# mrvollger/rustybam

Measured on AMD Instinct MI355X. Metric: CIGAR-ops/s, liftover over 100 kb sliding windows (whole pass, inputs resident in HBM), higher is better.
Workload: dtype u32

## Files before the change

### include/rustybam_amd.h

```cpp
#ifndef RUSTYBAM_AMD_H
#define RUSTYBAM_AMD_H

#include <stddef.h>
#include <stdint.h>

#ifdef __cplusplus
extern "C" {
#endif

#define RB_ABI_VERSION 1

enum rb_op { RB_OP_M = 0, RB_OP_I = 1, RB_OP_D = 2, RB_OP_N = 3, RB_OP_S = 4, RB_OP_H = 5, RB_OP_P = 6, RB_OP_EQ = 7, RB_OP_X = 8,
             RB_OP_CONT = 14  };

typedef enum rb_error {
    RB_OK = 0,
    RB_E_INVALID = -1,
    RB_E_NO_DEVICE = -2,
    RB_E_HIP = -3,
    RB_E_CAPACITY = -4,
    RB_E_NOMEM = -5
} rb_error;

typedef enum rb_status {
    RB_ST_OK = 0,
    RB_ST_NONE_INDEL = 1,
    RB_ST_NONE_NOMATCH = 2,
    RB_ST_NONE_EMPTY = 3,
    RB_ST_NONE_INVERTED = 4,
    RB_ST_NONE_INTEGRITY = 5,
    RB_ST_PANIC_NOTFOUND = 16,
    RB_ST_PANIC_EMPTY_CIGAR = 17,
    RB_ST_PANIC_INTEGRITY_T = 18,
    RB_ST_PANIC_INTEGRITY_Q = 19,
    RB_ST_PANIC_ALL_INDEL = 20,
    RB_ST_PANIC_ASSERT = 21,
    RB_ST_PANIC_OVERFLOW = 22
} rb_status;

enum { RB_BSEARCH_MODERN = 0 , RB_BSEARCH_LEGACY = 1 , RB_LIFT_EARLY_EXIT = 16,
       RB_LIFT_DESCRIPTORS = 32,
       RB_LIFT_FUSED_SCAN = 64,
       RB_BREAK_ONE_WALK = 128,
       RB_LIFT_OP_STARTS = 1 << 20,
       RB_LIFT_QBED = 1 << 21 };

enum {
    RB_F_REGULAR = 1u << 0,
    RB_F_STRIPPED = 1u << 1,
    RB_F_HAS_M = 1u << 2,
    RB_F_PROVISIONAL = 1u << 3,
    RB_F_ENDS_NOT_MATCH = 1u << 4
};
enum {
    RB_HIT_INSIDE = 1u << 0,
    RB_HIT_GENERIC = 1u << 1,
    RB_HIT_DESCRIPTOR = 1u << 2
};

typedef struct rb_reduce_row {
    uint64_t t_bases, q_bases;
    uint32_t nmatch, aln_len;
    uint32_t equal, diff, ins, del, matches;
    uint32_t ins_events, del_events;
    float id_by_all, id_by_events, id_by_matches;
    uint32_t status;
    uint32_t flags;
} rb_reduce_row;

typedef struct rb_norm_row {
    uint64_t t_st, t_en, q_st, q_en;
    uint32_t first_op, n_ops;
    uint32_t lead_ops, trail_ops;
    uint32_t nmatch, aln_len;
    uint32_t status;
    uint32_t flags;
} rb_norm_row;

typedef struct rb_hit_row {
    uint32_t rec, win;
    uint16_t status, flags;
    uint32_t out_n;
    uint64_t t_st, t_en, q_st, q_en;
    uint32_t nmatch, aln_len;
    uint64_t out_off;
} rb_hit_row;

typedef struct rb_pair_row {
    uint64_t split_idx;
    int32_t split_score;
    uint32_t status;
    uint64_t t_st[2], t_en[2], q_st[2], q_en[2];
    uint32_t nmatch[2], aln_len[2];
    uint64_t out_off[2];
    uint32_t out_n[2];
    uint64_t _pad;
} rb_pair_row;

typedef struct rb_counters {
    uint64_t n_hits;
    uint64_t out_ops_needed;
    uint64_t out_ops_used;
    uint64_t n_generic;
    uint32_t overflow;
    uint32_t phase[5];
    uint32_t brk_scratch_short;
    uint32_t redo_two_walk;
} rb_counters;

enum { RB_TEXT_OK = 0, RB_TEXT_BAD = 1 , RB_TEXT_TOO_LONG = 2 ,
       RB_TEXT_UNUSUAL = 3  };

typedef struct rb_batch_view {
    uint64_t n_rec, n_ops;
    const uint32_t *ops;
    const uint64_t *op_off;
    const uint64_t *t_st, *t_en, *q_st, *q_en;
    const uint8_t *strand;
    const uint32_t *contig;
} rb_batch_view;

typedef struct rb_windows_view {
    uint64_t n_win;
    const uint32_t *contig;
    const uint64_t *st, *en;
} rb_windows_view;

typedef struct rb_ctx rb_ctx;
typedef struct rb_plan rb_plan;

int rb_abi_version(void);
int rb_device_count(void);
int rb_ctx_create(int device, void *hip_stream, rb_ctx **out);
void rb_ctx_destroy(rb_ctx *ctx);
const char *rb_ctx_last_error(const rb_ctx *ctx);
int rb_ctx_sync(rb_ctx *ctx);
void *rb_ctx_stream(rb_ctx *ctx);
int rb_ctx_set_timing(rb_ctx *ctx, int enabled);
int rb_ctx_get_timing(rb_ctx *ctx, double *ms_out, int cap, int *n_out);

int rb_dev_alloc(rb_ctx *ctx, size_t bytes, void **dev_ptr);
int rb_dev_free(rb_ctx *ctx, void *dev_ptr);
int rb_dev_alloc_mode(rb_ctx *ctx, const void *dev_ptr);
int rb_dev_release(rb_ctx *ctx, void *dev_ptr);
int rb_dev_cache_trim(rb_ctx *ctx, uint64_t keep_bytes);
int rb_dev_alloc_stats(rb_ctx *ctx, uint64_t out[5]);
int rb_dev_upload(rb_ctx *ctx, void *dev_dst, const void *host_src, size_t bytes);
int rb_dev_download(rb_ctx *ctx, void *host_dst, const void *dev_src, size_t bytes);
int rb_dev_memset(rb_ctx *ctx, void *dev_dst, int value, size_t bytes);

int rb_dev_scan_records(rb_ctx *ctx, const rb_batch_view *batch, rb_reduce_row *reduce_rows, rb_norm_row *norm_rows);
int rb_ctx_scan_route(rb_ctx *ctx, uint64_t out[2]);

int rb_plan_create(rb_ctx *ctx, uint64_t n_rec, const uint64_t *op_off_host, const uint32_t *contig_host,
                   uint64_t n_win, const uint32_t *w_contig_host, const uint64_t *w_st_host, const uint64_t *w_en_host,
                   rb_plan **out);
void rb_plan_destroy(rb_plan *plan);
int64_t rb_plan_tiles_host(uint64_t n_rec, const uint64_t *op_off_host, uint64_t short_max, uint32_t *sched_out, uint32_t *tiles_out,
                           uint64_t tiles_cap, uint64_t *n_long_out);
size_t rb_plan_workspace_bytes(const rb_plan *plan, uint64_t rows_cap);
size_t rb_plan_diag_stamps_offset(const rb_plan *plan, uint64_t rows_cap);
uint64_t rb_plan_out_capacity(const rb_plan *plan, int for_break);

int rb_dev_liftover(rb_ctx *ctx, const rb_plan *plan, const rb_batch_view *batch, const rb_norm_row *norm_rows,
                    int bsearch_policy, void *workspace, rb_hit_row *rows, uint64_t rows_cap, uint32_t *out_ops,
                    uint64_t out_cap, rb_counters *counters);

size_t rb_largest_scratch_bytes(uint64_t n_keys);
int rb_dev_largest(rb_ctx *ctx, const rb_hit_row *rows, uint64_t n_rows, const uint32_t *win_key, const uint32_t *rec_key,
                   uint64_t n_keys, uint64_t *sel, uint64_t *out, void *scratch);

int rb_dev_stats_rows(rb_ctx *ctx, const rb_batch_view *batch, const rb_hit_row *rows, uint64_t n_rows, const uint32_t *out_ops,
                      rb_reduce_row *stats );

typedef struct rb_pieces_info {
    uint64_t n_pieces, n_ops;
    uint32_t overflow;
    uint32_t declined;
    uint64_t _reserved[5];
} rb_pieces_info;
size_t rb_rows_to_batch_scratch_bytes(uint64_t n_rows);
void rb_rows_to_batch_shape(uint32_t out[3]);
int rb_dev_rows_to_batch(rb_ctx *ctx, const rb_batch_view *src, const rb_hit_row *rows, uint64_t n_rows, const uint32_t *out_ops,
                         uint64_t pieces_cap, uint64_t ops_cap, uint32_t *new_ops, uint64_t *new_op_off ,
                         uint64_t *t_st, uint64_t *t_en, uint64_t *q_st, uint64_t *q_en, uint8_t *strand, uint32_t *contig,
                         uint32_t *parent , rb_pieces_info *info, void *scratch);

enum { RB_PAIRS_ORIENT = 1, RB_PAIRS_FILTER = 2 };
enum { RB_PAIRS_DECL_PANIC = 1, RB_PAIRS_DECL_KEY = 2, RB_PAIRS_DECL_WRAP = 4, RB_PAIRS_DECL_ZERO_SPAN = 8 };
typedef struct rb_pairs_info {
    uint64_t n_kept, n_flipped_rows;
    uint32_t overflow;
    uint32_t declined;
    uint64_t _reserved[5];
} rb_pairs_info;
size_t rb_pairs_scratch_bytes(uint64_t n_keys, uint64_t n_rows);
void rb_pairs_shape(uint32_t out[2]);
int rb_dev_pairs_rows(rb_ctx *ctx, const rb_hit_row *rows, uint64_t n_rows, const uint32_t *rec_key, const uint64_t *rec_q_len,
                      const uint8_t *strand , uint64_t n_rec, uint64_t n_keys, uint32_t mode, uint64_t paired_len,
                      uint64_t min_aln, uint64_t min_query, rb_hit_row *rows_out, uint64_t rows_cap, uint8_t *key_flip ,
                      rb_pairs_info *info, void *scratch);
int rb_host_pairs_rows(const rb_hit_row *rows, uint64_t n_rows, const uint32_t *rec_key, const uint64_t *rec_q_len, const uint8_t *strand,
                       uint64_t n_rec, uint64_t n_keys, uint32_t mode, uint64_t paired_len, uint64_t min_aln, uint64_t min_query,
                       rb_hit_row *rows_out, uint64_t rows_cap, uint8_t *key_flip, rb_pairs_info *info);

size_t rb_pairs_records_scratch_bytes(uint64_t n_keys, uint64_t n_rec);
void rb_pairs_records_shape(uint32_t out[2]);
int rb_dev_pairs_records(rb_ctx *ctx, const uint64_t *t_st, const uint64_t *t_en, const uint64_t *q_st, const uint64_t *q_en,
                         const uint8_t *strand, const uint32_t *rec_key, const uint64_t *rec_q_len ,
                         uint64_t n_rec, uint64_t n_keys, uint32_t mode ,
                         uint64_t paired_len, uint64_t min_aln, uint64_t min_query,
                         uint32_t *kept , uint64_t kept_cap, uint64_t *q_st_out, uint64_t *q_en_out ,
                         uint8_t *key_flip , uint64_t *key_order , rb_pairs_info *info, void *scratch);
int rb_host_pairs_records(const uint64_t *t_st, const uint64_t *t_en, const uint64_t *q_st, const uint64_t *q_en, const uint8_t *strand,
                          const uint32_t *rec_key, const uint64_t *rec_q_len, uint64_t n_rec, uint64_t n_keys, uint32_t mode, uint64_t paired_len,
                          uint64_t min_aln, uint64_t min_query, uint32_t *kept, uint64_t kept_cap, uint64_t *q_st_out, uint64_t *q_en_out,
                          uint8_t *key_flip, uint64_t *key_order, rb_pairs_info *info);

int rb_dev_break(rb_ctx *ctx, const rb_plan *plan, const rb_batch_view *batch, const rb_norm_row *norm_rows,
                 uint32_t max_size, int bsearch_policy, void *workspace, rb_hit_row *rows, uint64_t rows_cap,
                 uint32_t *out_ops, uint64_t out_cap, rb_counters *counters);

int rb_dev_swap(rb_ctx *ctx, const rb_batch_view *batch, uint32_t *out_ops);

enum { RB_TRIM_IN_PLACE = 256 };
int rb_dev_overlap_split(rb_ctx *ctx, const rb_batch_view *batch, const rb_norm_row *norm_rows, uint64_t n_pairs,
                         const uint32_t *left, const uint32_t *right, const uint64_t *pair_out_off, int match_score,
                         int diff_score, int indel_score, int bsearch_policy, rb_pair_row *rows, uint32_t *out_ops);

int rb_dev_trim_reserve(rb_ctx *ctx, uint64_t n_pairs);

int rb_dev_apply_pairs(rb_ctx *ctx, uint64_t n_pairs, const uint32_t *left, const uint32_t *right, const rb_pair_row *rows,
                       uint64_t *op_off, rb_norm_row *norm_rows);

typedef struct rb_trim_pass {
    uint64_t n_pairs, n_deferred, ops_end;
    uint32_t bad_status, _pad;
    uint64_t _reserved[4];
} rb_trim_pass;
size_t rb_trim_select_scratch_bytes(uint64_t n_groups);
int rb_dev_trim_select(rb_ctx *ctx, uint64_t n_rec, uint64_t n_groups, const uint32_t *order, const uint64_t *grp_off,
                       const rb_norm_row *norm_rows, uint64_t out_base, uint8_t *contained, uint32_t *left, uint32_t *right,
                       uint64_t *pair_out_off, rb_trim_pass *pass, void *scratch);
int rb_dev_trim_check(rb_ctx *ctx, uint64_t n_pairs, const rb_pair_row *rows, rb_trim_pass *pass);
int rb_dev_gather_records(rb_ctx *ctx, uint64_t n_rec, const uint32_t *ops, const uint64_t *op_off, const rb_norm_row *norm_rows,
                          uint64_t *new_op_off, uint32_t *new_ops, void *scratch);

int rb_host_scan_records(rb_ctx *ctx, uint64_t n_rec, const uint32_t *ops, const uint64_t *op_off,
                         const uint64_t *t_st, const uint64_t *t_en, const uint64_t *q_st, const uint64_t *q_en,
                         const uint8_t *strand, rb_reduce_row *reduce_rows, rb_norm_row *norm_rows);
int rb_host_liftover(rb_ctx *ctx, uint64_t n_rec, const uint32_t *ops, const uint64_t *op_off, const uint64_t *t_st,
                     const uint64_t *t_en, const uint64_t *q_st, const uint64_t *q_en, const uint8_t *strand,
                     const uint32_t *contig, uint64_t n_win, const uint32_t *w_contig, const uint64_t *w_st,
                     const uint64_t *w_en, int bsearch_policy, rb_norm_row *norm_rows_out ,
                     rb_hit_row **rows, uint64_t *n_rows, uint32_t **out_ops, uint64_t *n_out, rb_counters *counters);
int rb_host_break(rb_ctx *ctx, uint64_t n_rec, const uint32_t *ops, const uint64_t *op_off, const uint64_t *t_st,
                  const uint64_t *t_en, const uint64_t *q_st, const uint64_t *q_en, const uint8_t *strand,
                  uint32_t max_size, int bsearch_policy, rb_norm_row *norm_rows_out, rb_hit_row **rows,
                  uint64_t *n_rows, uint32_t **out_ops, uint64_t *n_out, rb_counters *counters);
int rb_host_swap(rb_ctx *ctx, uint64_t n_rec, const uint32_t *ops, const uint64_t *op_off, const uint8_t *strand,
                 uint32_t *out_ops);
int rb_host_overlap_split(rb_ctx *ctx, uint64_t n_rec, const uint32_t *ops, const uint64_t *op_off, const uint64_t *t_st,
                          const uint64_t *t_en, const uint64_t *q_st, const uint64_t *q_en, const uint8_t *strand,
                          uint64_t n_pairs, const uint32_t *left, const uint32_t *right, int match_score, int diff_score,
                          int indel_score, int bsearch_policy, rb_pair_row *rows, uint32_t **out_ops, uint64_t *n_out);
void rb_host_free(void *p);

size_t rb_text_scratch_bytes(uint64_t n);
int rb_dev_parse_cigars(rb_ctx *ctx, const uint8_t *text, const uint64_t *text_off, const uint64_t *text_end, uint64_t n_rec,
                        uint64_t *op_off, uint32_t *ops, uint64_t ops_cap, uint8_t *status, void *scratch);
int rb_dev_format_cigars(rb_ctx *ctx, const uint32_t *ops, const uint32_t *ops_alt, uint64_t n_items, const uint64_t *first,
                         const uint32_t *count, const uint32_t *first_len, const uint32_t *last_len, uint64_t *text_off, uint8_t *text,
                         uint64_t text_cap, void *scratch);
int rb_host_parse_cigars(rb_ctx *ctx, const uint8_t *text, const uint64_t *text_off, const uint64_t *text_end, uint64_t n_rec,
                         uint64_t *op_off, uint32_t **ops, uint8_t *status);
int rb_host_format_cigars(rb_ctx *ctx, const uint32_t *ops, uint64_t n_ops, uint64_t n_items, const uint64_t *first, const uint32_t *count,
                          const uint32_t *first_len, const uint32_t *last_len, uint64_t *text_off, uint8_t **text);
int rb_host_liftover_text(rb_ctx *ctx, uint64_t n_rec, const uint8_t *text, uint64_t text_bytes, const uint64_t *cig_off,
                          const uint64_t *cig_end, const uint64_t *t_st, const uint64_t *t_en, const uint64_t *q_st, const uint64_t *q_en,
                          const uint8_t *strand, const uint32_t *contig, uint64_t n_win, const uint32_t *w_contig, const uint64_t *w_st,
                          const uint64_t *w_en, int bsearch_policy, uint8_t *cig_status, rb_reduce_row *reduce_out, rb_norm_row *norm_out,
                          rb_hit_row **rows, uint64_t *n_rows, uint64_t **row_text_off, uint8_t **row_text, rb_counters *counters);
int rb_host_liftover_largest_text(rb_ctx *ctx, uint64_t n_rec, const uint8_t *text, uint64_t text_bytes, const uint64_t *cig_off,
                                  const uint64_t *cig_end, const uint64_t *t_st, const uint64_t *t_en, const uint64_t *q_st, const uint64_t *q_en,
                                  const uint8_t *strand, const uint32_t *contig, uint64_t n_win, const uint32_t *w_contig, const uint64_t *w_st,
                                  const uint64_t *w_en, int bsearch_policy, uint8_t *cig_status, rb_reduce_row *reduce_out, rb_norm_row *norm_out,
                                  rb_hit_row **rows, uint64_t *n_rows, uint64_t **row_text_off, uint8_t **row_text, rb_counters *counters,
                                  const uint32_t *win_key, uint64_t n_keys, uint32_t inside_key, int *declined);
int rb_host_break_text(rb_ctx *ctx, uint64_t n_rec, const uint8_t *text, uint64_t text_bytes, const uint64_t *cig_off,
                       const uint64_t *cig_end, const uint64_t *t_st, const uint64_t *t_en, const uint64_t *q_st, const uint64_t *q_en,
                       const uint8_t *strand, uint32_t max_size, int bsearch_policy, uint8_t *cig_status, rb_reduce_row *reduce_out,
                       rb_norm_row *norm_out, rb_hit_row **rows, uint64_t *n_rows, uint64_t **row_text_off, uint8_t **row_text,
                       rb_counters *counters);
int rb_host_liftover_stats_text(rb_ctx *ctx, uint64_t n_rec, const uint8_t *text, uint64_t text_bytes, const uint64_t *cig_off,
                                const uint64_t *cig_end, const uint64_t *t_st, const uint64_t *t_en, const uint64_t *q_st, const uint64_t *q_en,
                                const uint8_t *strand, const uint32_t *contig, uint64_t n_win, const uint32_t *w_contig, const uint64_t *w_st,
                                const uint64_t *w_en, int bsearch_policy, uint8_t *cig_status, rb_reduce_row *reduce_out, rb_norm_row *norm_out,
                                rb_hit_row **rows, uint64_t *n_rows, rb_reduce_row **stats, rb_counters *counters);
int rb_host_break_stats_text(rb_ctx *ctx, uint64_t n_rec, const uint8_t *text, uint64_t text_bytes, const uint64_t *cig_off,
                             const uint64_t *cig_end, const uint64_t *t_st, const uint64_t *t_en, const uint64_t *q_st, const uint64_t *q_en,
                             const uint8_t *strand, uint32_t max_size, int bsearch_policy, uint8_t *cig_status, rb_reduce_row *reduce_out,
                             rb_norm_row *norm_out, rb_hit_row **rows, uint64_t *n_rows, rb_reduce_row **stats, rb_counters *counters);
int rb_host_break_pairs_text(rb_ctx *ctx, uint64_t n_rec, const uint8_t *text, uint64_t text_bytes, const uint64_t *cig_off,
                             const uint64_t *cig_end, const uint64_t *t_st, const uint64_t *t_en, const uint64_t *q_st, const uint64_t *q_en,
                             const uint8_t *strand, uint32_t max_size, int bsearch_policy, uint8_t *cig_status, rb_reduce_row *reduce_out,
                             rb_norm_row *norm_out, rb_hit_row **rows, uint64_t *n_rows, uint64_t **row_text_off, uint8_t **row_text,
                             rb_counters *counters, const uint32_t *rec_key, const uint64_t *rec_q_len, uint64_t n_keys, uint32_t mode,
                             uint64_t paired_len, uint64_t min_aln, uint64_t min_query, uint8_t *key_flip, int *declined);
int rb_host_break_pairs_stats_text(rb_ctx *ctx, uint64_t n_rec, const uint8_t *text, uint64_t text_bytes, const uint64_t *cig_off,
                                   const uint64_t *cig_end, const uint64_t *t_st, const uint64_t *t_en, const uint64_t *q_st, const uint64_t *q_en,
                                   const uint8_t *strand, uint32_t max_size, int bsearch_policy, uint8_t *cig_status, rb_reduce_row *reduce_out,
                                   rb_norm_row *norm_out, rb_hit_row **rows, uint64_t *n_rows, rb_reduce_row **stats, rb_counters *counters,
// ... 90 lines not shown
```

### rustybam_amd/csrc/capi.hip

```cpp
#include <hip/hip_runtime.h>
#include <sys/mman.h>

#include <algorithm>
#include <cstdarg>
#include <cstdio>
#include <cstdlib>
#include <cstring>
#include <ctime>
#include <numeric>
#include <string>
#include <thread>
#include <vector>
#include <chrono>
#include <map>
#include <mutex>

#include "../../include/rustybam_amd.h"
#include "rb_lift.h"
#include "rb_trim.h"
#include "rb_launch.h"

#ifndef RB_SCAN_ROWS_MEAN_MAX
#define RB_SCAN_ROWS_MEAN_MAX 1536
#endif
#ifndef RB_SHORT_MAX_DEFAULT
#define RB_SHORT_MAX_DEFAULT 2048
#endif

#define RB_MAX_ARENA 256

#define RB_TIMING_RING 256
__global__ __launch_bounds__(256) void rb_k_fill_bytes(uint8_t *dst, uint32_t v4, size_t n) {
    const uintptr_t a = (uintptr_t)dst;
    const size_t head = n < 16 ? n : (size_t)((16 - (a & 15)) & 15);
    const size_t body = (n - head) / 16;
    const size_t tail0 = head + body * 16;
    const size_t i = (size_t)blockIdx.x * blockDim.x + threadIdx.x, stride = (size_t)gridDim.x * blockDim.x;
    for (size_t k = i; k < body; k += stride) *reinterpret_cast<uint4 *>(dst + head + k * 16) = make_uint4(v4, v4, v4, v4);
    if (i < head) dst[i] = (uint8_t)v4;
    if (i < n - tail0) dst[tail0 + i] = (uint8_t)v4;
}
extern "C" hipError_t rb_fill_async(void *dst, int value, size_t bytes, hipStream_t stream) {
    if (!bytes) return hipSuccess;
    const uint32_t b = (uint32_t)value & 255u, v4 = b | (b << 8) | (b << 16) | (b << 24);
    const size_t groups = bytes / 16 + 1;
    const unsigned blocks = (unsigned)std::min<size_t>((groups + 255) / 256, 65536);
    hipLaunchKernelGGL(rb_k_fill_bytes, dim3(blocks ? blocks : 1), dim3(256), 0, stream, (uint8_t *)dst, v4, bytes);
    return hipGetLastError();
}

struct rb_ctx {
    int device = -1;
    hipStream_t stream = nullptr;
    bool own_stream = false;
    std::string err;
    bool timing = false;
    std::vector<hipEvent_t> ev_a, ev_b;
    uint64_t timed_calls = 0;
    hipStream_t side = nullptr;
    hipEvent_t ev_fork = nullptr, ev_join = nullptr;
    void *trim_scratch = nullptr;
    uint32_t trim_scratch_blocks = 0;
    void *trim_pend = nullptr;
    uint64_t trim_pend_cap = 0;
    void *scan_list = nullptr;
    uint64_t scan_list_cap = 0;
    uint64_t scan_rows_n = 0;
    void *pin[2] = {nullptr, nullptr};
    hipEvent_t pin_ev[2] = {nullptr, nullptr};
    bool pin_busy[2] = {false, false};
    unsigned pin_next = 0;
    uint64_t alloc_fallbacks = 0;
    struct cached_buf { void *p; size_t bytes; bool placed; };
    std::vector<cached_buf> cache;
    size_t cache_bytes = 0;
};
#define RB_PIN_CHUNK ((size_t)32 << 20)
#define RB_PIN_MIN ((size_t)8 << 20)

struct rb_plan {
    rb_ctx *ctx = nullptr;
    uint64_t n_rec = 0, n_win = 0, n_ops = 0;
    uint32_t n_contig = 0;
    uint32_t depth = 0;
    uint32_t *sched = nullptr, *slot_of = nullptr, *canon_pos = nullptr, *w_orig = nullptr, *ident = nullptr;
    uint64_t *w_st = nullptr, *w_en = nullptr, *wo_st = nullptr, *wo_en = nullptr, *cw_off = nullptr;
    uint8_t *cw_mono = nullptr;
    uint32_t *tiles = nullptr;
    uint32_t n_tiles = 0, stream_end = 0;
};

static int fail(rb_ctx *ctx, int code, const char *fmt, ...) {
    if (ctx) {
        char buf[512];
        va_list ap;
        va_start(ap, fmt);
        vsnprintf(buf, sizeof buf, fmt, ap);
        va_end(ap);
        ctx->err = buf;
    }
    return code;
}
#define HIPCHK(ctx, call)                                                                             \
    do {                                                                                              \
        hipError_t e_ = (call);                                                                       \
        if (e_ != hipSuccess) return fail((ctx), RB_E_HIP, "%s: %s", #call, hipGetErrorString(e_)); \
    } while (0)

extern "C" int rb_abi_version(void) { return RB_ABI_VERSION; }

extern "C" int rb_device_count(void) {
    int n = 0;
    if (hipGetDeviceCount(&n) != hipSuccess) return 0;
    return n;
}

extern "C" int rb_ctx_create(int device, void *hip_stream, rb_ctx **out) {
    if (!out) return RB_E_INVALID;
    *out = nullptr;
    int n = 0;
    if (hipGetDeviceCount(&n) != hipSuccess || n <= 0 || device < 0 || device >= n) return RB_E_NO_DEVICE;
    hipDeviceProp_t prop;
    if (hipGetDeviceProperties(&prop, device) != hipSuccess) return RB_E_NO_DEVICE;
    if (strncmp(prop.gcnArchName, "gfx950", 6) != 0) {
        fprintf(stderr, "rustybam_amd: device %d is %s; this library only carries gfx950 (MI355X) code objects\n", device, prop.gcnArchName);
        return RB_E_NO_DEVICE;
    }
    if (hipSetDevice(device) != hipSuccess) return RB_E_NO_DEVICE;
    rb_ctx *c = new rb_ctx();
    c->device = device;
    if (hip_stream) {
        c->stream = (hipStream_t)hip_stream;
    } else {
        if (hipStreamCreateWithFlags(&c->stream, hipStreamNonBlocking) != hipSuccess) {
            delete c;
            return RB_E_HIP;
        }
        c->own_stream = true;
    }
    int prio_least = 0, prio_greatest = 0;
    if (hipDeviceGetStreamPriorityRange(&prio_least, &prio_greatest) != hipSuccess ||
        hipStreamCreateWithPriority(&c->side, hipStreamNonBlocking, prio_least) != hipSuccess ||
        hipEventCreateWithFlags(&c->ev_fork, hipEventDisableTiming) != hipSuccess ||
        hipEventCreateWithFlags(&c->ev_join, hipEventDisableTiming) != hipSuccess) {
        (void)hipGetLastError();
        rb_ctx_destroy(c);
        return RB_E_HIP;
    }
    *out = c;
    return RB_OK;
}
extern "C" void rb_ctx_destroy(rb_ctx *ctx) {
    if (!ctx) return;
    if (ctx->side) {
        (void)hipStreamSynchronize(ctx->side);
        hipStreamDestroy(ctx->side);
    }
    if (ctx->ev_fork) hipEventDestroy(ctx->ev_fork);
    if (ctx->ev_join) hipEventDestroy(ctx->ev_join);
    for (auto e : ctx->ev_a) hipEventDestroy(e);
    for (auto e : ctx->ev_b) hipEventDestroy(e);
    for (int k = 0; k < 2; k++) {
        if (ctx->pin[k]) hipHostFree(ctx->pin[k]);
        if (ctx->pin_ev[k]) hipEventDestroy(ctx->pin_ev[k]);
    }
    if (ctx->trim_scratch) hipFree(ctx->trim_scratch);
    if (ctx->trim_pend) hipFree(ctx->trim_pend);
    if (ctx->scan_list) hipFree(ctx->scan_list);
    (void)rb_dev_cache_trim(ctx, 0);
    if (ctx->own_stream) hipStreamDestroy(ctx->stream);
    delete ctx;
}
extern "C" const char *rb_ctx_last_error(const rb_ctx *ctx) { return ctx ? ctx->err.c_str() : "no context"; }
extern "C" int rb_ctx_sync(rb_ctx *ctx) {
    if (!ctx) return RB_E_INVALID;
    HIPCHK(ctx, hipStreamSynchronize(ctx->stream));
    return RB_OK;
}
extern "C" void *rb_ctx_stream(rb_ctx *ctx) { return ctx ? (void *)ctx->stream : nullptr; }

extern "C" int rb_ctx_set_timing(rb_ctx *ctx, int enabled) {
    if (!ctx) return RB_E_INVALID;
    if (enabled && ctx->ev_a.empty()) {
        ctx->ev_a.resize(RB_TIMING_RING);
        ctx->ev_b.resize(RB_TIMING_RING);
        for (int i = 0; i < RB_TIMING_RING; i++) {
            HIPCHK(ctx, hipEventCreate(&ctx->ev_a[i]));
            HIPCHK(ctx, hipEventCreate(&ctx->ev_b[i]));
        }
    }
    ctx->timing = enabled != 0;
    ctx->timed_calls = 0;
    return RB_OK;
}
extern "C" int rb_ctx_get_timing(rb_ctx *ctx, double *ms_out, int cap, int *n_out) {
    if (!ctx || !ms_out || !n_out) return RB_E_INVALID;
    HIPCHK(ctx, hipStreamSynchronize(ctx->stream));
    const uint64_t have = ctx->timed_calls < RB_TIMING_RING ? ctx->timed_calls : RB_TIMING_RING;
    int n = 0;
    for (uint64_t k = 0; k < have && n < cap; k++) {
        const uint64_t call = ctx->timed_calls - have + k;
        const size_t slot = (size_t)(call % RB_TIMING_RING);
        float ms = 0;
        HIPCHK(ctx, hipEventElapsedTime(&ms, ctx->ev_a[slot], ctx->ev_b[slot]));
        ms_out[n++] = ms;
    }
    *n_out = n;
    return RB_OK;
}

struct rb_vmm_alloc {
    size_t bytes, chunk;
    std::vector<hipMemGenericAllocationHandle_t> handles;
    bool placed = false;
};
static std::map<void *, rb_vmm_alloc> g_vmm;
static std::mutex g_vmm_mu;
static size_t g_va_live = 0, g_va_retired = 0;
static std::map<void *, size_t> g_asked;
static size_t rb_va_cap() {
    const char *e = getenv("RB_ALLOC_VA_CAP_GB");
    return (size_t)(e ? strtoull(e, nullptr, 10) : 32768ull) << 30;
}
static int rb_free_vmm(void *p, int device, hipError_t *err) {
    std::lock_guard<std::mutex> lk(g_vmm_mu);
    auto it = g_vmm.find(p);
    if (it == g_vmm.end()) return 0;
    hipError_t first = hipSuccess;
    auto note = [&](hipError_t e) {
        if (e != hipSuccess && first == hipSuccess) first = e;
    };
    note(hipSetDevice(device));
    note(hipDeviceSynchronize());
    const size_t chunk = it->second.chunk, n = it->second.handles.size();
    for (size_t k = 0; k < n; k++) note(hipMemUnmap((char *)p + k * chunk, chunk));
    for (auto &h : it->second.handles) note(hipMemRelease(h));
    g_va_live -= it->second.bytes;
    g_va_retired += it->second.bytes;
// ... 236 lines not shown
    if (!pin_ready(ctx)) {
        HIPCHK(ctx, hipStreamSynchronize(ctx->stream));
        HIPCHK(ctx, hipMemcpy(host_dst, dev_src, bytes, hipMemcpyDeviceToHost));
        return RB_OK;
    }
    size_t prev_off = 0, prev_n = 0;
    int prev_slot = -1;
    for (size_t off = 0, k = 0; off < bytes; off += RB_PIN_CHUNK, k++) {
        const int slot = (int)(k & 1);
        const size_t n = std::min(RB_PIN_CHUNK, bytes - off);
        if (ctx->pin_busy[slot]) HIPCHK(ctx, hipEventSynchronize(ctx->pin_ev[slot]));
        HIPCHK(ctx, hipMemcpyAsync(ctx->pin[slot], (const char *)dev_src + off, n, hipMemcpyDeviceToHost, ctx->stream));
        HIPCHK(ctx, hipEventRecord(ctx->pin_ev[slot], ctx->stream));
        ctx->pin_busy[slot] = true;
        if (prev_slot >= 0) {
            HIPCHK(ctx, hipEventSynchronize(ctx->pin_ev[prev_slot]));
            par_memcpy((char *)host_dst + prev_off, ctx->pin[prev_slot], prev_n);
            ctx->pin_busy[prev_slot] = false;
        }
        prev_off = off, prev_n = n, prev_slot = slot;
    }
    if (prev_slot >= 0) {
        HIPCHK(ctx, hipEventSynchronize(ctx->pin_ev[prev_slot]));
        par_memcpy((char *)host_dst + prev_off, ctx->pin[prev_slot], prev_n);
        ctx->pin_busy[prev_slot] = false;
    }
    HIPCHK(ctx, hipStreamSynchronize(ctx->stream));
    return RB_OK;
}
extern "C" int rb_dev_memset(rb_ctx *ctx, void *dev_dst, int value, size_t bytes) {
    if (!ctx) return RB_E_INVALID;
    if (bytes) HIPCHK(ctx, rb_fill_async(dev_dst, value, bytes, ctx->stream));
    return RB_OK;
}

extern "C" int rb_dev_scan_records(rb_ctx *ctx, const rb_batch_view *b, rb_reduce_row *reduce_rows, rb_norm_row *norm_rows) {
    if (!ctx || !b) return RB_E_INVALID;
    if (((uintptr_t)b->ops & 15u) != 0) return fail(ctx, RB_E_INVALID, "ops must be 16-byte aligned");
    rb_scan_params p;
    p.n_rec = b->n_rec;
    p.ops = b->ops;
    p.op_off = b->op_off;
    p.t_st = b->t_st;
    p.t_en = b->t_en;
    p.q_st = b->q_st;
    p.q_en = b->q_en;
    p.strand = b->strand;
    p.reduce_rows = reduce_rows;
    p.norm_rows = norm_rows;
    p.list = nullptr;
    p.n_list = nullptr;
    ctx->scan_rows_n = 0;
    if (b->n_rec >= 64 && b->n_ops / b->n_rec <= RB_SCAN_ROWS_MEAN_MAX) {
        if (ctx->scan_list_cap < b->n_rec) {
            HIPCHK(ctx, hipStreamSynchronize(ctx->stream));
            if (ctx->scan_list) hipFree(ctx->scan_list);
            ctx->scan_list = nullptr, ctx->scan_list_cap = 0;
            const uint64_t cap = b->n_rec + b->n_rec / 4 + 1024;
            if (hipMalloc(&ctx->scan_list, 256 + cap * 4) == hipSuccess) ctx->scan_list_cap = cap;
            else (void)hipGetLastError();
        }
        if (ctx->scan_list) {
            HIPCHK(ctx, rb_fill_async(ctx->scan_list, 0, 8, ctx->stream));
            HIPCHK(ctx, rb_launch_scan_rows(&p, ctx->scan_list, ctx->stream));
            ctx->scan_rows_n = b->n_rec;
            return RB_OK;
        }
    }
    HIPCHK(ctx, rb_launch_scan_records(&p, ctx->stream));
    return RB_OK;
}

extern "C" int rb_ctx_scan_route(rb_ctx *ctx, uint64_t out[2]) {
    if (!ctx || !out) return RB_E_INVALID;
    out[0] = out[1] = 0;
    if (!ctx->scan_rows_n) return RB_OK;
    unsigned long long n_listed = 0;
    HIPCHK(ctx, hipSetDevice(ctx->device));
    HIPCHK(ctx, hipMemcpyAsync(&n_listed, ctx->scan_list, sizeof n_listed, hipMemcpyDeviceToHost, ctx->stream));
    HIPCHK(ctx, hipStreamSynchronize(ctx->stream));
    out[0] = ctx->scan_rows_n - n_listed;
    out[1] = n_listed;
    return RB_OK;
}

template <typename T>
static int upload_vec(rb_ctx *ctx, const std::vector<T> &v, T **dev) {
    int rc = rb_dev_alloc(ctx, v.size() * sizeof(T) + 16, (void **)dev);
    if (rc) return rc;
    if (!v.empty()) {
        rc = rb_dev_upload(ctx, *dev, v.data(), v.size() * sizeof(T));
        if (rc) return rc;
    }
    return RB_OK;
}

static void rb_cut_tiles(uint64_t n_rec, const uint64_t *op_off, uint64_t short_max, std::vector<uint32_t> &sched, std::vector<uint32_t> &tiles,
                         uint64_t *n_long_out) {
    tiles.clear();
    *n_long_out = 0;
    short_max = std::min<uint64_t>(short_max, rb_tile_max_ops());
    if (short_max < 8 || !n_rec) return;
    const uint64_t max_ops = rb_tile_max_ops(), max_rec = rb_tile_max_records();
    std::vector<uint32_t> t2;
    uint64_t first = 0, cnt = 0, ops = 0, n_long = 0, n_tiled = 0;
    bool tiny = false;
    auto close = [&]() {
        if (cnt) t2.push_back((uint32_t)first | (tiny ? 0x80000000u : 0u)), t2.push_back((uint32_t)cnt), n_tiled += tiny ? 0 : cnt;
        cnt = 0, ops = 0;
    };
    for (uint64_t r = 0; r < n_rec; r++) {
        const uint64_t n = op_off[r + 1] - op_off[r];
        if (n > short_max) {
            close();
            n_long++;
            continue;
        }
        const bool t = n < 8;
        if (cnt && (t != tiny || cnt >= max_rec || (!t && ops + n > max_ops))) close();
        if (!cnt) first = r, tiny = t;
        cnt++, ops += n;
    }
    close();
    if (n_tiled == 0) return;
    std::vector<uint32_t> s2(n_rec);
    uint64_t a = 0, b = n_long;
    for (uint64_t w = 0; w < n_rec; w++)
        if (op_off[(uint64_t)sched[w] + 1] - op_off[sched[w]] > short_max) s2[a++] = sched[w];
    std::vector<uint32_t> slot_short(n_rec, 0);
    for (uint64_t r = 0; r < n_rec; r++)
        if (op_off[r + 1] - op_off[r] <= short_max) slot_short[r] = (uint32_t)b, s2[b++] = (uint32_t)r;
    sched.swap(s2);
    tiles.reserve(t2.size() / 2 * 3);
    for (size_t t = 0; t + 1 < t2.size(); t += 2) tiles.push_back(t2[t]), tiles.push_back(t2[t + 1]), tiles.push_back(slot_short[t2[t] & 0x7FFFFFFFu]);
    *n_long_out = n_long;
}
extern "C" int64_t rb_plan_tiles_host(uint64_t n_rec, const uint64_t *op_off, uint64_t short_max, uint32_t *sched_out, uint32_t *tiles_out,
                                      uint64_t tiles_cap, uint64_t *n_long_out) {
    if (n_rec && (!op_off || !sched_out)) return -1;
    if (n_rec >= 0xFFFFFFFFull) return -1;
    std::vector<uint32_t> sched(n_rec), tiles;
    std::iota(sched.begin(), sched.end(), 0u);
    std::stable_sort(sched.begin(), sched.end(), [&](uint32_t x, uint32_t y) { return op_off[(uint64_t)x + 1] - op_off[x] > op_off[(uint64_t)y + 1] - op_off[y]; });
    uint64_t n_long = 0;
    rb_cut_tiles(n_rec, op_off, short_max ? short_max : RB_SHORT_MAX_DEFAULT, sched, tiles, &n_long);
    for (uint64_t i = 0; i < n_rec; i++) sched_out[i] = sched[i];
    const uint64_t nt = tiles.size() / 3;
    for (uint64_t t = 0; t < nt && t < tiles_cap && tiles_out; t++)
        for (int k = 0; k < 3; k++) tiles_out[3 * t + k] = tiles[3 * t + k];
    if (n_long_out) *n_long_out = tiles.empty() ? n_rec : n_long;
    return (int64_t)nt;
}

extern "C" int rb_plan_create(rb_ctx *ctx, uint64_t n_rec, const uint64_t *op_off, const uint32_t *contig, uint64_t n_win,
                              const uint32_t *w_contig, const uint64_t *w_st, const uint64_t *w_en, rb_plan **out) {
    if (!ctx || !out || (n_rec && (!op_off || !contig))) return RB_E_INVALID;
    if (n_rec >= 0xFFFFFFFFull || n_win >= 0xFFFFFFFFull) return fail(ctx, RB_E_INVALID, "too many records/windows for one batch");
    HIPCHK(ctx, hipSetDevice(ctx->device));
    rb_plan *pl = new rb_plan();
    pl->ctx = ctx;
    pl->n_rec = n_rec;
    pl->n_win = n_win;
    uint32_t maxc = 0;
    for (uint64_t i = 0; i < n_rec; i++) maxc = std::max(maxc, contig[i]);
    for (uint64_t i = 0; i < n_win; i++) maxc = std::max(maxc, w_contig[i]);
    const uint32_t n_contig = (n_rec || n_win) ? maxc + 1 : 0;
    pl->n_contig = n_contig;
    std::vector<uint32_t> canon_pos(n_rec);
    {
        std::vector<uint64_t> rank(n_contig, UINT64_MAX);
        uint64_t nr = 0;
        for (uint64_t i = 0; i < n_rec; i++)
            if (rank[contig[i]] == UINT64_MAX) rank[contig[i]] = nr++;
        std::vector<uint64_t> start(nr + 1, 0);
        for (uint64_t i = 0; i < n_rec; i++) start[rank[contig[i]] + 1]++;
        for (uint64_t k = 0; k < nr; k++) start[k + 1] += start[k];
        for (uint64_t i = 0; i < n_rec; i++) canon_pos[i] = (uint32_t)start[rank[contig[i]]]++;
    }
    std::vector<uint32_t> sched(n_rec), ident(n_rec);
    std::iota(ident.begin(), ident.end(), 0u);
    {
        uint64_t max_len = 0;
        std::vector<uint64_t> key(n_rec);
        for (uint64_t i = 0; i < n_rec; i++) key[i] = op_off[i + 1] - op_off[i], max_len = std::max(max_len, key[i]);
        int passes = 0;
        while (passes < 4 && (max_len >> (16 * passes)) != 0) passes++;
        std::vector<uint32_t> a(ident), b(n_rec);
        std::vector<uint64_t> cnt(65537);
        for (int ps = 0; ps < passes; ps++) {
            std::fill(cnt.begin(), cnt.end(), 0);
            const int sh = 16 * ps;
            for (uint64_t i = 0; i < n_rec; i++) cnt[(0xFFFFu - (uint32_t)((key[i] >> sh) & 0xFFFFu)) + 1]++;
            for (int k = 0; k < 65536; k++) cnt[k + 1] += cnt[k];
            for (uint64_t i = 0; i < n_rec; i++) {
                const uint32_t r = a[i];
                b[cnt[0xFFFFu - (uint32_t)((key[r] >> sh) & 0xFFFFu)]++] = r;
            }
            a.swap(b);
        }
        sched = a;
    }
    std::vector<uint64_t> cw_off(n_contig + 1, 0), g_st(n_win), g_en(n_win), o_st(n_win), o_en(n_win);
    std::vector<uint32_t> g_orig(n_win);
    std::vector<uint8_t> mono(n_contig ? n_contig : 1, 1);
    for (uint64_t i = 0; i < n_win; i++) cw_off[w_contig[i] + 1]++;
    for (uint32_t c = 0; c < n_contig; c++) cw_off[c + 1] += cw_off[c];
    {
        std::vector<uint64_t> cur(cw_off.begin(), cw_off.end() - (n_contig ? 1 : 0));
        for (uint64_t i = 0; i < n_win; i++) {
            const uint64_t d = cur[w_contig[i]]++;
            g_st[d] = w_st[i];
            g_en[d] = w_en[i];
            g_orig[d] = (uint32_t)i;
            o_st[i] = w_st[i];
            o_en[i] = w_en[i];
        }
    }
    for (uint32_t c = 0; c < n_contig; c++)
        for (uint64_t i = cw_off[c] + 1; i < cw_off[c + 1]; i++)
            if (g_st[i] < g_st[i - 1] || g_en[i] < g_en[i - 1]) mono[c] = 0;
    pl->n_ops = n_rec ? op_off[n_rec] : 0;
    for (uint32_t c = 0; c < n_contig; c++) {
        if (!mono[c]) continue;
        uint64_t lo = cw_off[c];
        for (uint64_t i = cw_off[c]; i < cw_off[c + 1]; i++) {
            while (lo < i && g_en[lo] < g_st[i]) lo++;
            pl->depth = std::max<uint32_t>(pl->depth, (uint32_t)std::min<uint64_t>(i - lo + 1, 1u << 20));
        }
    }
    std::vector<uint32_t> tiles;
    pl->stream_end = (uint32_t)n_rec;
    {
        const char *e = getenv("RB_TILE");
        const bool on = !(e && !strcmp(e, "0"));
        uint64_t short_max = RB_SHORT_MAX_DEFAULT;
        if (const char *m = getenv("RB_SHORT_MAX")) short_max = strtoull(m, nullptr, 10);
        if (on && n_rec) {
            uint64_t n_long = 0;
            rb_cut_tiles(n_rec, op_off, short_max, sched, tiles, &n_long);
            if (!tiles.empty()) pl->stream_end = (uint32_t)n_long;
        }
        pl->n_tiles = (uint32_t)(tiles.size() / 3);
    }
    int rc = RB_OK;
    std::vector<uint32_t> slot_of(n_rec);
    for (uint64_t w = 0; w < n_rec; w++) slot_of[sched[w]] = (uint32_t)w;
    if (!rc) rc = upload_vec(ctx, sched, &pl->sched);
    if (!rc) rc = upload_vec(ctx, slot_of, &pl->slot_of);
    if (!rc) rc = upload_vec(ctx, ident, &pl->ident);
    if (!rc) rc = upload_vec(ctx, canon_pos, &pl->canon_pos);
    if (!rc) rc = upload_vec(ctx, g_st, &pl->w_st);
    if (!rc) rc = upload_vec(ctx, g_en, &pl->w_en);
    if (!rc) rc = upload_vec(ctx, g_orig, &pl->w_orig);
    if (!rc) rc = upload_vec(ctx, o_st, &pl->wo_st);
    if (!rc) rc = upload_vec(ctx, o_en, &pl->wo_en);
    if (!rc) rc = upload_vec(ctx, cw_off, &pl->cw_off);
    if (!rc) rc = upload_vec(ctx, mono, &pl->cw_mono);
    if (!rc && pl->n_tiles) rc = upload_vec(ctx, tiles, &pl->tiles);
    if (!rc && hipStreamSynchronize(ctx->stream) != hipSuccess) rc = fail(ctx, RB_E_HIP, "plan upload: %s", hipGetErrorString(hipGetLastError()));
    if (rc) {
        rb_plan_destroy(pl);
        return rc;
    }
    *out = pl;
    return RB_OK;
}
extern "C" void rb_plan_destroy(rb_plan *pl) {
    if (!pl) return;
    void *ptrs[] = {pl->sched, pl->slot_of, pl->ident, pl->canon_pos, pl->w_st, pl->w_en, pl->w_orig, pl->wo_st, pl->wo_en, pl->cw_off, pl->cw_mono, pl->tiles};
    for (void *q : ptrs)
        if (q) (void)rb_dev_free(pl->ctx, q);
    delete pl;
}

struct ws_layout {
    size_t hit_off, win_lo, block_sums, arena, pend_count, pend_list, jobs, gen_list, x_st, x_en, bp_tmp, bp_off, bp_cur, brk_rows, copy_count, copy_list, decl_count, decl_list, gen_cp, diag_stamps, fb_count, fb_list, starts_bad, total;
};
static bool rb_no_gen_cp() {
    static const bool v = getenv("RB_DEBUG_NO_GEN_CP") != nullptr;
    return v;
}
static ws_layout ws_of(uint64_t n_rec, uint64_t rows_cap, uint64_t n_ops) {
    ws_layout w;
    size_t o = 0;
    auto take = [&](size_t bytes) {
        size_t at = o;
        o += (bytes + 255) & ~(size_t)255;
        return at;
    };
    w.hit_off = take((n_rec + 2) * 8);
    w.win_lo = take((n_rec + 2) * 4);
    w.block_sums = take(rb_scan_block_sums_count(n_rec) * 8);
    w.arena = take((size_t)RB_MAX_ARENA * RB_ARENA_STRIDE * 8);
    w.pend_count = take(256);
    w.pend_list = take((n_rec + 1) * 4);
    w.jobs = take((n_rec + 1) * sizeof(rb_job));
    w.gen_list = take((rows_cap + 1) * 4);
    w.x_st = take((rows_cap + 1) * 8);
    w.x_en = take((rows_cap + 1) * 8);
    w.bp_tmp = take((rows_cap + 1) * 8);
    w.bp_off = take((n_rec + 1) * 8);
    w.bp_cur = take((size_t)RB_MAX_ARENA * 128);
    w.brk_rows = take((rows_cap + 1) * sizeof(rb_hit_row));
    w.copy_count = take(256);
    w.copy_list = take((rows_cap + 1) * 16);
    w.decl_count = take(256);
    w.decl_list = take((n_rec + 1) * 4);
    w.gen_cp = take(rb_no_gen_cp() ? 256 : (size_t)(n_ops / RB_GCP + n_rec + 2) * sizeof(uint4));
    w.diag_stamps = take((n_rec + 1) * 4);
    w.fb_count = take(256);
    w.fb_list = take((n_rec + 1) * 4);
    w.starts_bad = take(256);
    w.total = o;
    return w;
}
extern "C" size_t rb_plan_workspace_bytes(const rb_plan *plan, uint64_t rows_cap) {
    if (!plan) return 0;
    return ws_of(plan->n_rec, rows_cap, plan->n_ops).total;
}
extern "C" size_t rb_plan_diag_stamps_offset(const rb_plan *plan, uint64_t rows_cap) {
    if (!plan) return 0;
    return ws_of(plan->n_rec, rows_cap, plan->n_ops).diag_stamps;
}

static uint64_t slot_stride_of(uint64_t n_ops, uint64_t n_rec) { return ((n_ops + 31) & ~(uint64_t)31) + 32 * n_rec + 64; }
extern "C" uint64_t rb_plan_out_capacity(const rb_plan *plan, int for_break) {
    if (!plan) return 0;
    const uint64_t slots = for_break ? std::min<uint32_t>(2u, RB_MS) : std::min<uint32_t>(plan->depth, RB_MS);
    return slots * slot_stride_of(plan->n_ops, plan->n_rec) + plan->n_ops / 16 + 32 * plan->n_rec + (1u << 20);
}

static uint32_t pick_arenas(uint64_t n_rec) {
    uint64_t a = n_rec / 256;
    if (a < 1) a = 1;
    if (a > RB_MAX_ARENA) a = RB_MAX_ARENA;
    return (uint32_t)a;
}

static int lift_common(rb_ctx *ctx, const rb_plan *plan, const rb_batch_view *b, const rb_norm_row *norm, int policy,
                       void *workspace, rb_hit_row *rows, uint64_t rows_cap, uint32_t *out_ops, uint64_t out_cap,
                       rb_counters *counters, bool is_break, uint32_t max_size) {
    if (!ctx || !plan || !b || !norm || !workspace || !counters) return RB_E_INVALID;
    if (b->n_rec != plan->n_rec) return fail(ctx, RB_E_INVALID, "plan was built for %llu records, batch has %llu", (unsigned long long)plan->n_rec, (unsigned long long)b->n_rec);
    if (((uintptr_t)b->ops & 15u) || ((uintptr_t)out_ops & 15u)) return fail(ctx, RB_E_INVALID, "ops/out_ops must be 16-byte aligned");
    if (rows_cap >= 0xFFFFFFFFull) return fail(ctx, RB_E_INVALID, "rows_cap too large");
    if ((uintptr_t)workspace & 255u) return fail(ctx, RB_E_INVALID, "workspace must be 256-byte aligned");
    const ws_layout w = ws_of(plan->n_rec, rows_cap, plan->n_ops);
    char *ws = (char *)workspace;
    rb_lift_params p;
    memset(&p, 0, sizeof p);
    p.n_rec = b->n_rec;
    p.ops = b->ops;
    p.op_off = b->op_off;
    p.contig = b->contig;
    p.strand = b->strand;
    p.norm = norm;
    p.sched = plan->sched;
    p.slot_of = plan->slot_of;
    p.canon_pos = is_break ? plan->ident : plan->canon_pos;
    p.w_st = plan->w_st;
    p.w_en = plan->w_en;
    p.w_orig = plan->w_orig;
    p.wo_st = plan->wo_st;
    p.wo_en = plan->wo_en;
    p.cw_off = plan->cw_off;
    p.cw_mono = plan->cw_mono;
    p.n_contig = plan->n_contig;
    p.hit_off = (uint64_t *)(ws + w.hit_off);
    p.win_lo = (uint32_t *)(ws + w.win_lo);
    p.rows = rows;
    p.rows_cap = rows_cap;
    p.out_ops = out_ops;
    p.out_cap = out_cap;
    p.arena_cur = (unsigned long long *)(ws + w.arena);
    p.n_arena = pick_arenas(b->n_rec);
    p.desc_mode = (policy & RB_LIFT_DESCRIPTORS) ? 1 : 0;
    p.slot_stride = slot_stride_of(b->n_ops, b->n_rec);
    const uint32_t want = p.desc_mode ? 0u : std::min<uint32_t>(is_break ? 2u : plan->depth, RB_MS);
    const uint64_t min_arena = 1024ull * p.n_arena;
    uint32_t n_slots = want;
    while (n_slots && (uint64_t)n_slots * p.slot_stride + min_arena > out_cap) n_slots--;
    if (getenv("RB_DEBUG_SLOTS")) n_slots = std::min<uint32_t>(n_slots, (uint32_t)atoi(getenv("RB_DEBUG_SLOTS")));
    p.n_slots = n_slots;
    p.needed_base = p.desc_mode ? 4 * rows_cap : (uint64_t)want * p.slot_stride;
    p.arena_origin = p.desc_mode ? 4 * rows_cap : (uint64_t)n_slots * p.slot_stride;
    if (p.desc_mode && out_cap < p.arena_origin + 1024) return fail(ctx, RB_E_CAPACITY, "descriptor mode needs out_cap >= 4 * rows_cap + 1024");
    p.arena_size = out_cap > p.arena_origin ? ((out_cap - p.arena_origin) / p.n_arena) & ~(uint64_t)3 : 0;
    p.copy_list = (uint4 *)(ws + w.copy_list);
    p.gj_a = (rb_gja *)(ws + w.brk_rows), p.gj_b = (uint4 *)(ws + w.copy_list), p.gj_c = (uint2 *)(ws + w.bp_tmp);
    p.copy_count = (unsigned long long *)(ws + w.copy_count);
    p.gen_list = (uint32_t *)(ws + w.gen_list);
    p.gen_cp = rb_no_gen_cp() ? nullptr : (uint4 *)(ws + w.gen_cp);
    p.diag_stamps = (uint32_t *)(ws + w.diag_stamps);
    p.jobs = (rb_job *)(ws + w.jobs);
    p.fused = (policy & RB_LIFT_FUSED_SCAN) ? 1 : 0;
    p.op_starts = (policy & RB_LIFT_OP_STARTS) ? 1 : 0;
    if (p.op_starts && p.fused) return fail(ctx, RB_E_INVALID, "RB_LIFT_OP_STARTS takes finished norm_rows: not together with RB_LIFT_FUSED_SCAN");
    if (p.op_starts && (policy & RB_LIFT_DESCRIPTORS)) return fail(ctx, RB_E_INVALID, "RB_LIFT_OP_STARTS with RB_LIFT_DESCRIPTORS: a descriptor indexes the record's ORIGINAL cigar, which a batch cut in place no longer is");
    if (p.op_starts && b->n_ops > plan->n_ops) return fail(ctx, RB_E_INVALID, "RB_LIFT_OP_STARTS: batch->n_ops exceeds the plan's op count (gather the batch first)");
    if (p.op_starts && b->n_rec) {
        unsigned long long *bad = (unsigned long long *)(ws + w.starts_bad), first_bad = 0;
        HIPCHK(ctx, rb_fill_async(bad, 0xFF, 8, ctx->stream));
        HIPCHK(ctx, rb_launch_starts_check(b->op_off, norm, b->n_rec, b->n_ops, bad, ctx->stream));
        HIPCHK(ctx, hipMemcpyAsync(&first_bad, bad, 8, hipMemcpyDeviceToHost, ctx->stream));
        HIPCHK(ctx, hipStreamSynchronize(ctx->stream));
        if (first_bad != ~0ull)
            return fail(ctx, RB_E_INVALID, "RB_LIFT_OP_STARTS: record %llu lies outside the batch's %llu ops (a pass moved it: gather the batch first)",
                        first_bad, (unsigned long long)b->n_ops);
    }
    p.norm_w = const_cast<rb_norm_row *>(norm);
    p.pend_list = (uint32_t *)(ws + w.pend_list);
    p.pend_count = (unsigned long long *)(ws + w.pend_count);
    const bool use_tiles = plan->n_tiles != 0 && ((policy >> 8) & 0xFFF) == 0;
    p.tile_first = use_tiles ? plan->tiles : nullptr;
    p.n_tiles = use_tiles ? plan->n_tiles : 0;
    p.fb_list = (uint32_t *)(ws + w.fb_list);
    p.fb_count = (unsigned long long *)(ws + w.fb_count);
    const uint32_t stream_end = use_tiles ? plan->stream_end : (uint32_t)b->n_rec;
    rb_scan_params sp;
    memset(&sp, 0, sizeof sp);
    if (p.fused) {
        sp.n_rec = b->n_rec;
        sp.ops = b->ops;
        sp.op_off = b->op_off;
        sp.t_st = b->t_st, sp.t_en = b->t_en, sp.q_st = b->q_st, sp.q_en = b->q_en;
        sp.strand = b->strand;
        sp.norm_rows = p.norm_w;
        HIPCHK(ctx, rb_fill_async(p.pend_count, 0, 8, ctx->stream));
        HIPCHK(ctx, rb_launch_peek_norm(&sp, ctx->stream));
    }
    p.counters = counters;
    p.policy = policy & 1;
    p.early_exit = (policy & RB_LIFT_EARLY_EXIT) ? 1 : 0;
    p.debug_skip = (policy >> 8) & 0xFFF;
    uint64_t *block_sums = (uint64_t *)(ws + w.block_sums);
    HIPCHK(ctx, rb_fill_async(counters, 0, sizeof(rb_counters), ctx->stream));
    HIPCHK(ctx, rb_fill_async(p.copy_count, 0, 8, ctx->stream));
    HIPCHK(ctx, rb_fill_async(p.arena_cur, 0, (size_t)RB_MAX_ARENA * RB_ARENA_STRIDE * 8, ctx->stream));
    if (b->n_rec == 0) return RB_OK;
    const bool one_walk = is_break && (policy & RB_BREAK_ONE_WALK) && !p.desc_mode;
    if (one_walk) {
        p.brk_mode = 1, p.brk_max = max_size;
        p.rows_final = rows;
        p.rows = (rb_hit_row *)(ws + w.brk_rows);
        p.brk_off = (uint64_t *)(ws + w.bp_off);
        p.brk_cursor = (unsigned long long *)(ws + w.bp_cur);
        p.brk_n_arena = pick_arenas(b->n_rec);
        p.brk_arena_cap = rows_cap / p.brk_n_arena;
        p.brk_decl_list = (uint32_t *)(ws + w.decl_list);
        p.brk_decl_count = (unsigned long long *)(ws + w.decl_count);
        HIPCHK(ctx, rb_fill_async(p.brk_decl_count, 0, 8, ctx->stream));
        HIPCHK(ctx, rb_fill_async(p.brk_cursor, 0, (size_t)RB_MAX_ARENA * 128, ctx->stream));
        HIPCHK(ctx, rb_fill_async(p.hit_off, 0, (size_t)(b->n_rec + 2) * 8, ctx->stream));
        HIPCHK(ctx, rb_fill_async(p.brk_off, 0xFF, (size_t)(b->n_rec + 1) * 8, ctx->stream));
        HIPCHK(ctx, rb_launch_make_jobs(&p, ctx->stream));
        const size_t slot1 = (size_t)(ctx->timed_calls % RB_TIMING_RING);
        if (ctx->timing) HIPCHK(ctx, hipEventRecord(ctx->ev_a[slot1], ctx->stream));
        p.wave0 = 0;
        p.wave_end = stream_end;
        HIPCHK(ctx, rb_launch_liftover_stream(&p, ctx->stream));
        if (use_tiles) {
            HIPCHK(ctx, rb_fill_async(p.fb_count, 0, 8, ctx->stream));
            HIPCHK(ctx, rb_launch_liftover_tiles(&p, ctx->stream));
            HIPCHK(ctx, rb_launch_liftover_stream_list(&p, ctx->stream));
        }
        if (p.fused) {
            sp.list = p.pend_list;
            sp.n_list = (const uint64_t *)p.pend_count;
            HIPCHK(ctx, rb_launch_scan_records(&sp, ctx->stream));
        }
        if (ctx->timing) {
            HIPCHK(ctx, hipEventRecord(ctx->ev_b[slot1], ctx->stream));
            ctx->timed_calls++;
        }
        rb_break_params bp;
        memset(&bp, 0, sizeof bp);
        bp.n_rec = b->n_rec, bp.ops = b->ops, bp.op_off = b->op_off, bp.norm = norm, bp.sched = plan->sched, bp.hit_off = p.hit_off;
        bp.x_st = (uint64_t *)(ws + w.x_st), bp.x_en = (uint64_t *)(ws + w.x_en);
        bp.rows_cap = rows_cap, bp.max_size = max_size;
        bp.list = p.brk_decl_list, bp.n_list = p.brk_decl_count;
        bp.fill = 0;
        HIPCHK(ctx, rb_launch_break_list_declined(&p, ctx->stream));
        HIPCHK(ctx, rb_launch_break_pieces(&bp, ctx->stream));
        HIPCHK(ctx, rb_launch_count_and_scan(&p, block_sums, false, ctx->stream));
        bp.fill = 1;
        HIPCHK(ctx, rb_launch_break_pieces(&bp, ctx->stream));
        HIPCHK(ctx, rb_launch_break_gather(&p, ctx->stream));
        rb_lift_params pg = p;
        pg.rows = rows, pg.x_st = bp.x_st, pg.x_en = bp.x_en;
        HIPCHK(ctx, rb_launch_break_declined(&pg, ctx->stream));
        return RB_OK;
    }
    if (is_break) {
        rb_break_params bp;
        memset(&bp, 0, sizeof bp);
        bp.n_rec = b->n_rec;
        bp.ops = b->ops;
        bp.op_off = b->op_off;
        bp.norm = norm;
        bp.sched = plan->sched;
        bp.hit_off = p.hit_off;
        bp.x_st = (uint64_t *)(ws + w.x_st);
        bp.x_en = (uint64_t *)(ws + w.x_en);
        bp.rows_cap = rows_cap;
        bp.max_size = max_size;
        bp.tmp = (uint2 *)(ws + w.bp_tmp);
        bp.tmp_off = (uint64_t *)(ws + w.bp_off);
        bp.tmp_cursor = (unsigned long long *)(ws + w.bp_cur);
        bp.n_arena = pick_arenas(b->n_rec);
        bp.arena_cap = rows_cap / bp.n_arena;
        HIPCHK(ctx, rb_fill_async(bp.tmp_cursor, 0, (size_t)RB_MAX_ARENA * 128, ctx->stream));
        bp.fill = 2, bp.redo_only = 0;
        HIPCHK(ctx, rb_launch_break_pieces(&bp, ctx->stream));
        HIPCHK(ctx, rb_launch_count_and_scan(&p, block_sums, false, ctx->stream));
        HIPCHK(ctx, rb_launch_break_place(&bp, ctx->stream));
        bp.fill = 1, bp.redo_only = 1;
        HIPCHK(ctx, rb_launch_break_pieces(&bp, ctx->stream));
        p.x_st = bp.x_st;
        p.x_en = bp.x_en;
    } else {
        HIPCHK(ctx, rb_launch_count_and_scan(&p, block_sums, true, ctx->stream));
    }
    const char *tb = getenv("RB_TILE_BESIDE");
    const bool beside = use_tiles && !is_break && stream_end != 0 && !(tb && atoi(tb) == 0);
    if (use_tiles && !is_break) HIPCHK(ctx, rb_fill_async(p.fb_count, 0, 8, ctx->stream));
    HIPCHK(ctx, rb_launch_make_jobs(&p, ctx->stream));
    const size_t slot = (size_t)(ctx->timed_calls % RB_TIMING_RING);
    if (beside) HIPCHK(ctx, hipEventRecord(ctx->ev_fork, ctx->stream));
    if (ctx->timing) HIPCHK(ctx, hipEventRecord(ctx->ev_a[slot], ctx->stream));
    p.wave0 = 0;
    p.wave_end = stream_end;
    if (beside) {
        hipError_t e = hipStreamWaitEvent(ctx->side, ctx->ev_fork, 0);
        const char *what = "hipStreamWaitEvent(fork)";
        if (e == hipSuccess) e = rb_launch_liftover_tiles(&p, ctx->side), what = "rb_launch_liftover_tiles";
        if (e == hipSuccess) e = rb_launch_liftover_stream_list(&p, ctx->side), what = "rb_launch_liftover_stream_list";
        if (e == hipSuccess) e = hipEventRecord(ctx->ev_join, ctx->side), what = "hipEventRecord(join)";
        if (e == hipSuccess) e = rb_launch_liftover_stream(&p, ctx->stream), what = "rb_launch_liftover_stream";
        if (e == hipSuccess) e = hipStreamWaitEvent(ctx->stream, ctx->ev_join, 0), what = "hipStreamWaitEvent(join)";
        if (e != hipSuccess) {
            (void)hipStreamSynchronize(ctx->side);
            return fail(ctx, RB_E_HIP, "%s: %s", what, hipGetErrorString(e));
        }
    } else {
        HIPCHK(ctx, rb_launch_liftover_stream(&p, ctx->stream));
        if (use_tiles) {
            if (is_break) HIPCHK(ctx, rb_fill_async(p.fb_count, 0, 8, ctx->stream));
            HIPCHK(ctx, rb_launch_liftover_tiles(&p, ctx->stream));
            HIPCHK(ctx, rb_launch_liftover_stream_list(&p, ctx->stream));
        }
    }
    if (p.fused) {
        sp.list = p.pend_list;
        sp.n_list = (const uint64_t *)p.pend_count;
        HIPCHK(ctx, rb_launch_scan_records(&sp, ctx->stream));
    }
    if (ctx->timing) {
        HIPCHK(ctx, hipEventRecord(ctx->ev_b[slot], ctx->stream));
        ctx->timed_calls++;
    }
    HIPCHK(ctx, rb_launch_liftover_tail(&p, ctx->stream));
    return RB_OK;
}

extern "C" int rb_dev_liftover(rb_ctx *ctx, const rb_plan *plan, const rb_batch_view *batch, const rb_norm_row *norm_rows,
                               int bsearch_policy, void *workspace, rb_hit_row *rows, uint64_t rows_cap, uint32_t *out_ops,
                               uint64_t out_cap, rb_counters *counters) {
    return lift_common(ctx, plan, batch, norm_rows, bsearch_policy, workspace, rows, rows_cap, out_ops, out_cap, counters, false, 0);
}
extern "C" int rb_dev_break(rb_ctx *ctx, const rb_plan *plan, const rb_batch_view *batch, const rb_norm_row *norm_rows,
                            uint32_t max_size, int bsearch_policy, void *workspace, rb_hit_row *rows, uint64_t rows_cap,
                            uint32_t *out_ops, uint64_t out_cap, rb_counters *counters) {
    return lift_common(ctx, plan, batch, norm_rows, bsearch_policy, workspace, rows, rows_cap, out_ops, out_cap, counters, true, max_size);
}

extern "C" int rb_dev_swap(rb_ctx *ctx, const rb_batch_view *b, uint32_t *out_ops) {
    if (!ctx || !b || !out_ops) return RB_E_INVALID;
    rb_swap_params p;
    p.n_rec = b->n_rec;
    p.ops = b->ops;
    p.op_off = b->op_off;
    p.strand = b->strand;
    p.out_ops = out_ops;
    if (out_ops == b->ops) {
        HIPCHK(ctx, rb_launch_swap_inplace(&p, ctx->stream));
        return RB_OK;
    }
    if (out_ops < b->ops + b->n_ops && b->ops < out_ops + b->n_ops)
        return fail(ctx, RB_E_INVALID, "rb_dev_swap: out_ops overlaps the batch's ops without being equal to them (in place: out_ops == batch->ops)");
    HIPCHK(ctx, rb_launch_swap(&p, ctx->stream));
    return RB_OK;
}

static int trim_pend_reserve(rb_ctx *ctx, uint64_t n_pairs) {
    if (ctx->trim_pend && ctx->trim_pend_cap >= n_pairs) return RB_OK;
    HIPCHK(ctx, hipStreamSynchronize(ctx->stream));
    if (ctx->trim_pend) hipFree(ctx->trim_pend);
    ctx->trim_pend = nullptr, ctx->trim_pend_cap = 0;
    const uint64_t cap = n_pairs + n_pairs / 4 + 1024;
    const hipError_t e = hipMalloc(&ctx->trim_pend, 256 + cap * 4);
    if (e != hipSuccess) {
        ctx->trim_pend = nullptr, (void)hipGetLastError();
        return fail(ctx, RB_E_NOMEM, "hipMalloc(list of %llu pending pairs): %s", (unsigned long long)cap, hipGetErrorString(e));
    }
    ctx->trim_pend_cap = cap;
    return RB_OK;
}
extern "C" int rb_dev_trim_reserve(rb_ctx *ctx, uint64_t n_pairs) {
    if (!ctx) return RB_E_INVALID;
    HIPCHK(ctx, hipSetDevice(ctx->device));
    return trim_pend_reserve(ctx, n_pairs);
}

extern "C" int rb_dev_overlap_split(rb_ctx *ctx, const rb_batch_view *b, const rb_norm_row *norm, uint64_t n_pairs, const uint32_t *left,
                                    const uint32_t *right, const uint64_t *pair_out_off, int match_score, int diff_score,
                                    int indel_score, int policy, rb_pair_row *rows, uint32_t *out_ops) {
    if (!ctx || !b || !norm || (n_pairs && (!left || !right || !pair_out_off || !rows || !out_ops))) return RB_E_INVALID;
    rb_trim_params p;
    p.n_pairs = n_pairs;
    p.ops = b->ops;
    p.op_off = b->op_off;
    p.strand = b->strand;
    p.norm = norm;
    p.left = left;
    p.right = right;
    p.pair_out_off = pair_out_off;
    p.match_score = match_score;
    p.diff_score = diff_score;
    p.indel_score = indel_score;
    p.policy = policy & 1;
    p.rows = rows;
    p.out_ops = out_ops;
    p.list_declined = 0;
    p.in_place = (policy & RB_TRIM_IN_PLACE) ? 1 : 0;
    if (p.in_place && out_ops != b->ops) return fail(ctx, RB_E_INVALID, "RB_TRIM_IN_PLACE: out_ops must be the batch's own ops array");
    if (!ctx->trim_scratch) {
        const uint32_t blocks = 48;
        if (hipMalloc(&ctx->trim_scratch, rb_trim_scratch_bytes(blocks)) == hipSuccess) ctx->trim_scratch_blocks = blocks;
        else ctx->trim_scratch = nullptr, (void)hipGetLastError();
    }
    p.scratch = (uint32_t *)ctx->trim_scratch;
    p.scratch_blocks = ctx->trim_scratch_blocks;
    {
        const int rc = trim_pend_reserve(ctx, n_pairs);
        if (rc) return rc;
    }
    p.pend = (unsigned long long *)ctx->trim_pend;
    p.pend_list = (uint32_t *)((char *)ctx->trim_pend + 256);
    HIPCHK(ctx, rb_fill_async(p.pend, 0, 8, ctx->stream));
    HIPCHK(ctx, rb_launch_overlap_split(&p, ctx->stream));
    return RB_OK;
}

extern "C" size_t rb_trim_select_scratch_bytes(uint64_t n_groups) {
    return 2 * (((n_groups + 2) * 8 + 255) & ~(size_t)255) + ((2 * n_groups * 4 + 255) & ~(size_t)255) + (rb_scan_block_sums_count(n_groups) + 4) * 8 + 256;
}
extern "C" int rb_dev_trim_select(rb_ctx *ctx, uint64_t n_rec, uint64_t n_groups, const uint32_t *order, const uint64_t *grp_off,
                                  const rb_norm_row *norm_rows, uint64_t out_base, uint8_t *contained, uint32_t *left, uint32_t *right,
                                  uint64_t *pair_out_off, rb_trim_pass *pass, void *scratch) {
    if (!ctx || !pass || (n_groups && (!order || !grp_off || !norm_rows || !contained || !left || !right || !pair_out_off || !scratch))) return RB_E_INVALID;
    (void)n_rec;
    HIPCHK(ctx, hipSetDevice(ctx->device));
    rb_tsel_params p;
    memset(&p, 0, sizeof p);
    char *sc = (char *)scratch;
    p.n_groups = n_groups, p.order = order, p.grp_off = grp_off, p.norm = norm_rows, p.contained = contained;
    p.slot = (uint64_t *)sc;
    sc += ((n_groups + 2) * 8 + 255) & ~(size_t)255;
    p.has = (uint64_t *)sc;
    sc += ((n_groups + 2) * 8 + 255) & ~(size_t)255;
    p.cand = (uint32_t *)sc;
    sc += (2 * n_groups * 4 + 255) & ~(size_t)255;
    p.out_base = out_base, p.left = left, p.right = right, p.pair_out_off = pair_out_off, p.pass = pass;
    HIPCHK(ctx, rb_launch_trim_select(&p, (uint64_t *)sc, ctx->stream));
    return RB_OK;
}
extern "C" int rb_dev_trim_check(rb_ctx *ctx, uint64_t n_pairs, const rb_pair_row *rows, rb_trim_pass *pass) {
    if (!ctx || !pass || (n_pairs && !rows)) return RB_E_INVALID;
    HIPCHK(ctx, hipSetDevice(ctx->device));
    HIPCHK(ctx, rb_launch_trim_check(rows, n_pairs, pass, ctx->stream));
    return RB_OK;
}
extern "C" int rb_dev_apply_pairs(rb_ctx *ctx, uint64_t n_pairs, const uint32_t *left, const uint32_t *right, const rb_pair_row *rows,
                                  uint64_t *op_off, rb_norm_row *norm_rows) {
    if (!ctx || (n_pairs && (!left || !right || !rows || !op_off || !norm_rows))) return RB_E_INVALID;
    rb_apply_params p{n_pairs, left, right, rows, op_off, norm_rows};
    HIPCHK(ctx, rb_launch_apply_pairs(&p, ctx->stream));
    return RB_OK;
}
extern "C" int rb_dev_gather_records(rb_ctx *ctx, uint64_t n_rec, const uint32_t *ops, const uint64_t *op_off, const rb_norm_row *norm_rows,
                                     uint64_t *new_op_off, uint32_t *new_ops, void *scratch) {
    if (!ctx || !new_op_off || !scratch || (n_rec && (!ops || !op_off || !norm_rows))) return RB_E_INVALID;
    rb_gather_params p{n_rec, ops, op_off, norm_rows, new_op_off, new_ops, 0};
    HIPCHK(ctx, rb_fill_async(new_op_off + n_rec, 0, 8, ctx->stream));
    if (n_rec == 0) return RB_OK;
    HIPCHK(ctx, rb_launch_gather_records(&p, ctx->stream));
    HIPCHK(ctx, rb_launch_exclusive_scan(new_op_off, n_rec, (uint64_t *)scratch, nullptr, ctx->stream));
    if (new_ops) {
        p.fill = 1;
        HIPCHK(ctx, rb_launch_gather_records(&p, ctx->stream));
// ... 1732 lines not shown
```

### rustybam_amd/csrc/k_liftover.hip

```cpp
#include "rb_lift.h"
#include "rb_launch.h"
#include <type_traits>
#include <algorithm>

__global__ __launch_bounds__(256) void rb_k_count_hits(rb_lift_params p) {
    const uint64_t r = (uint64_t)blockIdx.x * blockDim.x + threadIdx.x;
    if (r >= p.n_rec) return;
    uint64_t cnt = 0;
    const rb_norm_row *nr = &p.norm[r];
    const uint32_t c = p.contig[r];
    if (nr->status == RB_ST_OK && c < p.n_contig) {
        const uint64_t ws = p.cw_off[c], we = p.cw_off[c + 1];
        const uint64_t t_st = nr->t_st, t_en = nr->t_en;
        if (p.cw_mono[c]) {
            const uint64_t lo = rb_lower_en_gt(p.w_en, ws, we, t_st);
            const uint64_t hi = rb_lower_st_ge(p.w_st, ws, we, t_en);
            cnt = hi > lo ? hi - lo : 0;
            p.win_lo[r] = (uint32_t)lo;
        } else {
            for (uint64_t i = ws; i < we; i++) cnt += (t_en > p.w_st[i] && t_st < p.w_en[i]) ? 1 : 0;
        }
    }
    p.hit_off[p.canon_pos[r]] = cnt;
}

#define RB_SCAN_PER_BLOCK 2048
__global__ __launch_bounds__(256) void rb_k_scan_partial(const uint64_t *v, uint64_t n, uint64_t *block_sums) {
    __shared__ uint64_t sh[4];
    const uint64_t base = (uint64_t)blockIdx.x * RB_SCAN_PER_BLOCK;
    uint64_t s = 0;
    for (int k = 0; k < RB_SCAN_PER_BLOCK / 256; k++) {
        uint64_t i = base + (uint64_t)k * 256 + threadIdx.x;
        if (i < n) s += v[i];
    }
    s = rb_wave_sum_u64(s);
    if ((threadIdx.x & 63) == 0) sh[threadIdx.x >> 6] = s;
    __syncthreads();
    if (threadIdx.x == 0) block_sums[blockIdx.x] = sh[0] + sh[1] + sh[2] + sh[3];
}
__global__ __launch_bounds__(256) void rb_k_scan_top(uint64_t *block_sums, uint64_t n_blocks) {
    __shared__ uint64_t sh[256];
    __shared__ uint64_t carry;
    if (threadIdx.x == 0) carry = 0;
    __syncthreads();
    for (uint64_t b = 0; b < n_blocks; b += 256) {
        uint64_t i = b + threadIdx.x;
        uint64_t x = i < n_blocks ? block_sums[i] : 0;
        sh[threadIdx.x] = x;
        __syncthreads();
        for (int off = 1; off < 256; off <<= 1) {
            uint64_t y = threadIdx.x >= (unsigned)off ? sh[threadIdx.x - off] : 0;
            __syncthreads();
            sh[threadIdx.x] += y;
            __syncthreads();
        }
        uint64_t incl = sh[threadIdx.x];
        if (i < n_blocks) block_sums[i] = carry + incl - x;
        __syncthreads();
        if (threadIdx.x == 255) carry += incl;
        __syncthreads();
    }
    if (threadIdx.x == 0) block_sums[n_blocks] = carry;
}
__global__ __launch_bounds__(256) void rb_k_scan_apply(uint64_t *v, uint64_t n, const uint64_t *block_sums, uint64_t *total_out) {
    __shared__ uint64_t sh[256];
    const uint64_t base = (uint64_t)blockIdx.x * RB_SCAN_PER_BLOCK;
    uint64_t x[RB_SCAN_PER_BLOCK / 256];
    uint64_t s = 0;
    const uint64_t i0 = base + (uint64_t)threadIdx.x * (RB_SCAN_PER_BLOCK / 256);
#pragma unroll
    for (int k = 0; k < RB_SCAN_PER_BLOCK / 256; k++) {
        x[k] = (i0 + k < n) ? v[i0 + k] : 0;
        s += x[k];
    }
    sh[threadIdx.x] = s;
    __syncthreads();
    for (int off = 1; off < 256; off <<= 1) {
        uint64_t y = threadIdx.x >= (unsigned)off ? sh[threadIdx.x - off] : 0;
        __syncthreads();
        sh[threadIdx.x] += y;
        __syncthreads();
    }
    uint64_t run = block_sums[blockIdx.x] + sh[threadIdx.x] - s;
#pragma unroll
    for (int k = 0; k < RB_SCAN_PER_BLOCK / 256; k++) {
        if (i0 + k < n) v[i0 + k] = run;
        run += x[k];
    }
    if (blockIdx.x == gridDim.x - 1 && threadIdx.x == 255) {
        const uint64_t total = block_sums[gridDim.x];
        v[n] = total;
        if (total_out) *total_out = total;
    }
}

__global__ __launch_bounds__(256) void rb_k_make_jobs(rb_lift_params p) {
    const uint64_t r64 = (uint64_t)blockIdx.x * blockDim.x + threadIdx.x;
    if (r64 >= p.n_rec) return;
    const uint32_t r = (uint32_t)r64;
    const uint64_t w = p.slot_of[r];
    const rb_norm_row *nr = &p.norm[r];
    rb_job j;
    j.r = r;
    j.n = nr->n_ops;
    j.rec0 = p.op_off[r] + nr->first_op;
    j.t_st = nr->t_st, j.t_en = nr->t_en, j.q_st = nr->q_st, j.q_en = nr->q_en;
    const uint64_t k = p.canon_pos[r];
    const bool brk = p.brk_mode != 0;
    const uint64_t h0 = brk ? 0ull : p.hit_off[k], nh = brk ? 1ull : p.hit_off[k + 1] - h0;
    const bool explicit_w = brk || p.x_st != nullptr;
    const uint32_t cg = p.contig[r];
    const bool mono = explicit_w || (cg < p.n_contig && p.cw_mono[cg] != 0);
    uint32_t f = 0;
    const bool provisional = (nr->flags & RB_F_PROVISIONAL) != 0;
    if (nr->status == RB_ST_OK && (nh != 0 || provisional)) {
        if (h0 + nh > p.rows_cap) f |= RB_JOB_ROWS_OVERFLOW;
        else f |= RB_JOB_VALID;
    }
    if ((nr->flags & RB_F_REGULAR) || (provisional && !(nr->flags & RB_F_ENDS_NOT_MATCH))) f |= RB_JOB_REGULAR;
    if (p.strand[r] == (uint8_t)'-') f |= RB_JOB_MINUS;
    if (mono) f |= RB_JOB_MONO;
    j.flags = f;
    j.h0 = (uint32_t)h0;
    j.nh = (uint32_t)nh;
    j.lo = (explicit_w || !mono || !(f & RB_JOB_VALID) || nh == 0) ? 0u : p.win_lo[r];
    p.jobs[w] = j;
}

#define RB_RING_BASE 88
#define RB_RING_TOP_N 103
#define RB_SPILL_ROOM 4
#define RB_WPE 4, 5
#include "rb_stream.h"
#define RB_STREAM_KERNEL(NAME, BRK, DIAG, ROOM)                                                                                   \
    __global__ __launch_bounds__(256) __attribute__((amdgpu_waves_per_eu(RB_WPE), amdgpu_num_vgpr(RB_RING_BASE - (ROOM)))) void NAME(rb_lift_params p_) { \
        (void)p_;                                 \
        rb_stream_record<BRK, DIAG>();                                                                                            \
    }
RB_STREAM_KERNEL(rb_k_liftover_stream, false, false, RB_SPILL_ROOM)
RB_STREAM_KERNEL(rb_k_liftover_stream_diag, false, true, 5)

__global__ __launch_bounds__(256) void rb_k_copy_clips(rb_lift_params p) {
    const uint64_t n_copy = *p.copy_count;
    const int lane = rb_lane();
    for (uint64_t e = (uint64_t)blockIdx.x * 4u + (threadIdx.x >> 6); e < n_copy; e += (uint64_t)gridDim.x * 4u) {
        const uint4 d = p.copy_list[e];
        rb_hit_row *row = &p.rows[d.x];
        const uint32_t rec = row->rec, n = row->out_n;
        const uint32_t *src = p.ops + p.op_off[rec] + p.norm[rec].first_op + d.y;
        const uint32_t padded = (n + 3u) & ~3u;
        const uint32_t arena = (uint32_t)(e % p.n_arena);
        unsigned long long b0 = 0;
        if (lane == 0) b0 = atomicAdd(&p.arena_cur[(uint64_t)arena * RB_ARENA_STRIDE], (unsigned long long)padded);
        b0 = rb_first64(b0);
        if (b0 + padded > p.arena_size) {
            if (lane == 0) p.counters->overflow = 1;
            continue;
        }
        const uint64_t off = p.arena_origin + (uint64_t)arena * p.arena_size + b0;
        uint32_t *dst = p.out_ops + off;
        for (uint32_t k = (uint32_t)lane; k < n; k += 64u) {
            uint32_t w = src[k];
            const uint32_t len0 = rb_len(w);
            uint32_t len = len0;
            if (n == 1u && d.z && d.w) len = d.z + d.w - len0;
            else {
                if (k == 0 && d.z) len = d.z;
                if (k == n - 1u && d.w) len = d.w;
            }
            dst[k] = (len << 4) | rb_opc(w);
        }
        if (lane == 0) row->out_off = off;
    }
}

struct rb_gwalk {
    const uint32_t *ops;
    uint32_t n;
};

__device__ uint64_t rb_legacy_probe(uint64_t N, uint64_t klo, uint64_t khi) {
    uint64_t size = N, left = 0, right = N;
    while (left < right) {
        const uint64_t mid = left + size / 2;
        if (mid < klo)
            left = mid + 1;
        else if (mid > khi)
            right = mid;
        else
            return mid;
        size = right - left;
    }
    return klo;
}

__device__ uint64_t rb_unit_tpos(const uint32_t *ops, uint32_t n, uint64_t t_st, uint64_t unit) {
    int64_t tpos = (int64_t)t_st - 1;
    uint64_t U = 0;
    for (uint32_t i = 0; i < n; i++) {
        const uint32_t opc = rb_wopc(ops, i), len = rb_wlen(ops, i);
        const bool isref = opc <= 8 && rb_in(RB_REF_MASK, opc);
        if (unit < U + len) return (uint64_t)(isref ? tpos + (int64_t)(unit - U) + 1 : tpos);
        U += len;
        if (isref) tpos += len;
    }
    return ~0ull;
}
__device__ bool rb_bsearch_units(const uint32_t *ops, uint32_t n, uint64_t t_st, uint64_t N, uint64_t key, int policy, uint64_t *idx) {
    auto cmp = [&](uint64_t mid) -> int {
        const uint64_t v = rb_unit_tpos(ops, n, t_st, mid);
        return v < key ? -1 : (v > key ? 1 : 0);
    };
    if (policy != RB_BSEARCH_LEGACY) {
        uint64_t size = N;
        if (size == 0) return false;
        uint64_t base = 0;
        while (size > 1) {
            const uint64_t half = size / 2, mid = base + half;
            base = cmp(mid) > 0 ? base : mid;
            size -= half;
        }
        *idx = base;
        return cmp(base) == 0;
    }
    uint64_t size = N, left = 0, right = N;
    while (left < right) {
        const uint64_t mid = left + size / 2;
        const int c = cmp(mid);
        if (c < 0) left = mid + 1;
        else if (c > 0) right = mid;
        else {
            *idx = mid;
            return true;
        }
        size = right - left;
    }
    return false;
}

__device__ void rb_generic_serial_hit(const rb_lift_params &p, const uint64_t g) {
    for (int once = 0; once < 1; once++) {
        const uint64_t hrow = p.gen_list[g];
        rb_hit_row *row = &p.rows[hrow];
        const uint32_t r = row->rec, win = row->win;
        const rb_norm_row *nr = &p.norm[r];
        if (nr->status != RB_ST_OK) {
            row->status = (uint16_t)nr->status;
            row->out_n = 0;
            row->out_off = 0;
            row->t_st = row->t_en = row->q_st = row->q_en = 0;
            row->nmatch = row->aln_len = 0;
            continue;
        }
        const uint64_t t_st = nr->t_st, t_en = nr->t_en, q_st = nr->q_st, q_en = nr->q_en;
        const bool minus = p.strand[r] == (uint8_t)'-';
        const uint32_t n = nr->n_ops;
        const uint32_t *ops = p.ops + p.op_off[r] + nr->first_op;
        const uint64_t wst = p.x_st ? p.x_st[hrow] : p.wo_st[win];
        const uint64_t wen = p.x_en ? p.x_en[hrow] : p.wo_en[win];
        rb_hit_row w;
        w.rec = r;
        w.win = win;
        w.flags = RB_HIT_GENERIC;
        w.status = RB_ST_OK;
        w.out_n = 0;
        w.out_off = 0;
        w.t_st = w.t_en = w.q_st = w.q_en = 0;
        w.nmatch = w.aln_len = 0;
        const uint32_t arena = (uint32_t)(g % p.n_arena);

        if (t_st > wst && t_en < wen) {
            w.flags |= RB_HIT_INSIDE;
            w.t_st = t_st;
            w.t_en = t_en;
            w.q_st = q_st;
            w.q_en = q_en;
            w.nmatch = nr->nmatch;
            w.aln_len = nr->aln_len;
            w.out_n = n;
            const uint32_t padded = (n + 3u) & ~3u;
            const unsigned long long b0 = atomicAdd(&p.arena_cur[(uint64_t)arena * RB_ARENA_STRIDE], (unsigned long long)padded);
            if (b0 + padded <= p.arena_size) {
                w.out_off = p.arena_origin + (uint64_t)arena * p.arena_size + b0;
                for (uint32_t i = 0; i < n; i++) p.out_ops[w.out_off + i] = ops[i];
            } else {
                p.counters->overflow = 1;
            }
            *row = w;
            continue;
        }
        const int64_t ps = (int64_t)(wst > t_st ? wst : t_st);
        const int64_t pe = (int64_t)(wen < t_en ? wen : t_en) - 1;
        uint64_t N = 0;
        uint64_t s_lo = 0, s_hi = 0, e_lo = 0, e_hi = 0;
        bool s_found = false, e_found = false;
        {
            int64_t tpos = (int64_t)t_st - 1;
            for (uint32_t i = 0; i < n; i++) {
                const uint32_t opc = rb_wopc(ops, i), len = rb_wlen(ops, i);
                if (len == 0) continue;
                if (opc <= 8 && rb_in(RB_REF_MASK, opc)) {
                    if (ps > tpos && ps <= tpos + (int64_t)len) {
                        const uint64_t u = N + (uint64_t)(ps - tpos - 1);
                        if (!s_found) { s_found = true; s_lo = u; }
                        s_hi = u;
                    }
                    if (pe > tpos && pe <= tpos + (int64_t)len) {
                        const uint64_t u = N + (uint64_t)(pe - tpos - 1);
                        if (!e_found) { e_found = true; e_lo = u; }
                        e_hi = u;
                    }
                    tpos += len;
                } else {
                    if (ps == tpos && tpos >= 0) {
                        if (!s_found) { s_found = true; s_lo = N; }
                        s_hi = N + len - 1;
                    }
                    if (pe == tpos && tpos >= 0) {
                        if (!e_found) { e_found = true; e_lo = N; }
                        e_hi = N + len - 1;
                    }
                }
                N += len;
            }
        }
        bool wrapped = false;
        if (t_st == 0)
            for (uint32_t i = 0; i < n; i++) {
                if (rb_wlen(ops, i) == 0) continue;
                const uint32_t opc = rb_wopc(ops, i);
                wrapped = !(opc <= 8 && rb_in(RB_REF_MASK, opc));
                break;
            }
        uint64_t ks, ke;
        if (wrapped) {
            if (!rb_bsearch_units(ops, n, t_st, N, (uint64_t)ps, p.policy, &ks) || !rb_bsearch_units(ops, n, t_st, N, (uint64_t)pe, p.policy, &ke)) {
                w.status = RB_ST_PANIC_NOTFOUND;
                *row = w;
                continue;
            }
        } else {
            if (!s_found || !e_found) {
                w.status = RB_ST_PANIC_NOTFOUND;
                *row = w;
                continue;
            }
            ks = p.policy == RB_BSEARCH_LEGACY ? rb_legacy_probe(N, s_lo, s_hi) : s_hi;
            ke = p.policy == RB_BSEARCH_LEGACY ? rb_legacy_probe(N, e_lo, e_hi) : e_hi;
        }
        uint64_t a = N, b = 0;
        uint64_t Ra = 0, Qa = 0, Ma = 0, nRb = 0, nQb = 0, nMb = 0;
        {
            uint64_t U = 0, R = 0, Q = 0, M = 0;
            bool a_set = false;
            for (uint32_t i = 0; i < n; i++) {
                const uint32_t opc = rb_wopc(ops, i), len = rb_wlen(ops, i);
                if (len == 0) continue;
                const bool isref = opc <= 8 && rb_in(RB_REF_MASK, opc), isq = opc <= 8 && rb_in(RB_QRY_MASK, opc);
                const bool ism = opc <= 8 && rb_in(RB_MATCH_MASK, opc);
                if (ism) {
                    if (!a_set && U + len > ks) {
                        a = ks > U ? ks : U;
                        const uint64_t off = a - U;
                        Ra = R + off;
                        Qa = Q + off;
                        Ma = M + off;
                        a_set = true;
                    }
                    if (U <= ke) {
                        b = (U + len - 1) < ke ? (U + len - 1) : ke;
                        const uint64_t off = b - U;
                        nRb = R + off + 1;
                        nQb = Q + off + 1;
                        nMb = M + off + 1;
                    }
                }
                U += len;
                if (isref) R += len;
                if (isq) Q += len;
                if (ism) M += len;
            }
        }
        if (a > b || a >= N) {
            w.status = RB_ST_NONE_INDEL;
            *row = w;
            continue;
        }
        uint32_t out_n = 0;
        {
            uint64_t U = 0;
            uint32_t prev = RB_NULL_OP, run = 0;
            for (uint32_t i = 0; i < n; i++) {
                const uint32_t opc = rb_wopc(ops, i), len = rb_wlen(ops, i);
                if (len == 0) continue;
                const uint64_t u0 = U, u1 = U + len - 1;
                U += len;
                if (u1 < a) continue;
                if (u0 > b) break;
                const uint64_t c0 = u0 > a ? u0 : a, c1 = u1 < b ? u1 : b;
                if (opc != prev) {
                    if (prev != RB_NULL_OP) out_n += 1u + ((run >> RB_LEN_BITS_WORD) ? 1u : 0u);
                    run = 0;
                }
                run += (uint32_t)(c1 - c0 + 1);
                prev = opc;
            }
            if (prev != RB_NULL_OP) out_n += 1u + ((run >> RB_LEN_BITS_WORD) ? 1u : 0u);
        }
        w.t_st = t_st + Ra;
        w.t_en = t_st + nRb;
        if (!minus) {
            w.q_st = q_st + Qa;
            w.q_en = q_st + nQb;
        } else {
            w.q_st = q_en - nQb;
            w.q_en = q_en - Qa;
        }
        w.nmatch = (uint32_t)(nMb - Ma);
        w.aln_len = (uint32_t)(b - a + 1);
        w.out_n = out_n;
        const uint32_t padded = (out_n + 3u) & ~3u;
        const unsigned long long b0 = atomicAdd(&p.arena_cur[(uint64_t)arena * RB_ARENA_STRIDE], (unsigned long long)padded);
        if (b0 + padded > p.arena_size) {
            p.counters->overflow = 1;
            *row = w;
            continue;
        }
        w.out_off = p.arena_origin + (uint64_t)arena * p.arena_size + b0;
        {
            uint64_t U = 0;
            uint32_t prev = RB_NULL_OP, run = 0;
            uint64_t o = w.out_off;
            for (uint32_t i = 0; i < n; i++) {
                const uint32_t opc = rb_wopc(ops, i), len = rb_wlen(ops, i);
                if (len == 0) continue;
                const uint64_t u0 = U, u1 = U + len - 1;
                U += len;
                if (u1 < a) continue;
                if (u0 > b) break;
                const uint64_t c0 = u0 > a ? u0 : a, c1 = u1 < b ? u1 : b;
                const uint32_t piece = (uint32_t)(c1 - c0 + 1);
                if (opc != prev) {
                    if (prev != RB_NULL_OP) o += rb_emit_run(p.out_ops + o, run, prev);
                    prev = opc;
                    run = piece;
                } else {
                    run += piece;
                }
            }
            if (prev != RB_NULL_OP) o += rb_emit_run(p.out_ops + o, run, prev);
        }
        *row = w;
    }
}

__device__ __forceinline__ uint4 *rb_gen_cp_of(const rb_lift_params &p, uint32_t r, uint32_t first_op) {
    return p.gen_cp + ((p.op_off[r] + first_op) / RB_GCP + r);
}
__global__ __launch_bounds__(256) void rb_k_generic_checkpoints(rb_lift_params p) {
    static_assert(RB_GCP == 64u, "one 16-byte load per lane covers four checkpoint intervals: lanes 0, 16, 32, 48 stand at their starts");
    const uint32_t wib = threadIdx.x >> 6;
    const int lane = rb_lane();
    const uint64_t n_gen = p.counters->n_generic;
    for (uint64_t g = (uint64_t)blockIdx.x * 4u + wib; g < n_gen; g += (uint64_t)gridDim.x * 4u) {
        const uint32_t r = p.rows[p.gen_list[g]].rec;
        if (g > 0 && p.rows[p.gen_list[g - 1]].rec == r) continue;
        const rb_norm_row *nr = &p.norm[r];
        if (nr->status != RB_ST_OK) continue;
        const uint32_t n = nr->n_ops;
        if (n <= RB_GCP) continue;
        const uint32_t *ops = p.ops + p.op_off[r] + nr->first_op;
        uint4 *cp = rb_gen_cp_of(p, r, nr->first_op);
        auto load = [&](uint32_t c0) -> uint4 {
            const uint32_t i = c0 + 4u * (uint32_t)lane;
            if (i + 3u < n) return rb_load4_unaligned(ops + i);
            return make_uint4(i < n ? ops[i] : 0u, i + 1u < n ? ops[i + 1u] : 0u, i + 2u < n ? ops[i + 2u] : 0u, 0u);
        };
        uint64_t U = 0;
        uint32_t R = 0, Q = 0, M = 0;
        uint4 nxt = load(0u);
        for (uint32_t c0 = 0; c0 < n; c0 += 256u) {
            const uint4 cur = nxt;
            if (c0 + 256u < n) nxt = load(c0 + 256u);
            const uint32_t w4[4] = {cur.x, cur.y, cur.z, cur.w};
            uint64_t u = 0;
            uint32_t rr = 0, q = 0, m = 0;
#pragma unroll
            for (int k = 0; k < 4; k++) {
                const uint32_t i = c0 + 4u * (uint32_t)lane + (uint32_t)k;
                uint32_t opc = rb_opc(w4[k]), len = rb_len(w4[k]);
                if (opc == RB_OP_CONT && i < n) opc = rb_wopc(ops, i), len = rb_wlen(ops, i);
                const bool okc = opc <= 8u;
                u += len;
                rr += okc && rb_in(RB_REF_MASK, opc) ? len : 0u;
                q += okc && rb_in(RB_QRY_MASK, opc) ? len : 0u;
                m += okc && rb_in(RB_MATCH_MASK, opc) ? len : 0u;
            }
            const uint64_t iu = (uint64_t)rb_wave_scan_incl((uint32_t)u & 0xFFFFFFu) + ((uint64_t)rb_wave_scan_incl((uint32_t)(u >> 24)) << 24);
            const uint32_t ir = rb_wave_scan_incl(rr), iq = rb_wave_scan_incl(q), im = rb_wave_scan_incl(m);
            const bool mine = (lane & 15) == 0 && c0 + 4u * (uint32_t)lane < n;
            const uint64_t Uv = U + iu - u;
            if (__ballot(mine && (Uv >> 32)) != 0ull) {
                if (lane == 0) cp[0] = make_uint4(0xFFFFFFFFu, 0xFFFFFFFFu, 0xFFFFFFFFu, 0xFFFFFFFFu);
                break;
            }
            if (mine) cp[c0 / RB_GCP + ((uint32_t)lane >> 4)] = make_uint4((uint32_t)Uv, R + ir - rr, Q + iq - q, M + im - m);
            U += rb_readlane<uint64_t>(iu, 63), R += rb_readlane<uint32_t>(ir, 63), Q += rb_readlane<uint32_t>(iq, 63), M += rb_readlane<uint32_t>(im, 63);
        }
    }
}
__device__ __forceinline__ uint64_t rb_wave_min_u64(uint64_t v) {
#pragma unroll
    for (int off = 32; off > 0; off >>= 1) {
        const uint64_t o = __shfl_xor(v, off, 64);
        v = o < v ? o : v;
    }
    return v;
}
__device__ __forceinline__ uint64_t rb_wave_max_u64(uint64_t v) {
#pragma unroll
    for (int off = 32; off > 0; off >>= 1) {
        const uint64_t o = __shfl_xor(v, off, 64);
        v = o > v ? o : v;
    }
    return v;
}
__global__ __launch_bounds__(256) void rb_k_generic_jobs(rb_lift_params p) {
    const uint64_t n_gen = p.counters->n_generic;
    for (uint64_t g = (uint64_t)blockIdx.x * 256u + threadIdx.x; g < n_gen; g += (uint64_t)gridDim.x * 256u) {
        const uint32_t hrow = p.gen_list[g];
        const rb_hit_row *row = &p.rows[hrow];
        const uint32_t r = row->rec, win = row->win;
        const rb_norm_row *nr = &p.norm[r];
        rb_gja A;
        A.t_st = nr->t_st, A.t_en = nr->t_en, A.q_st = nr->q_st, A.q_en = nr->q_en;
        A.n = nr->n_ops;
        A.ops_off = p.op_off[r] + nr->first_op;
        A.wst = p.x_st ? p.x_st[hrow] : p.wo_st[win];
        A.wen = p.x_en ? p.x_en[hrow] : p.wo_en[win];
        A.k2 = 0;
        uint32_t k1 = 0, has_cp = 0;
        const uint32_t status = nr->status;
        if (status == RB_ST_OK && !(A.t_st > A.wst && A.t_en < A.wen)) {
            const uint4 *gcp = (p.gen_cp && A.n > RB_GCP) ? rb_gen_cp_of(p, r, nr->first_op) : nullptr;
            if (gcp && gcp[0].x == 0xFFFFFFFFu) gcp = nullptr;
            if (gcp) {
                has_cp = 1;
                const uint32_t ncp = (A.n + RB_GCP - 1u) / RB_GCP;
                auto last_le = [&](uint64_t target) -> uint32_t {
                    uint32_t lo = 0, hi = ncp;
                    while (hi - lo > 1u) {
                        const uint32_t mid = (lo + hi) >> 1;
                        if ((uint64_t)gcp[mid].y <= target) lo = mid; else hi = mid;
                    }
                    return lo;
                };
                const int64_t ps = (int64_t)(A.wst > A.t_st ? A.wst : A.t_st), pe = (int64_t)(A.wen < A.t_en ? A.wen : A.t_en) - 1;
                k1 = last_le((uint64_t)ps - A.t_st);
                const uint32_t k2 = pe >= ps ? last_le((uint64_t)pe - A.t_st) : 0u;
                if (k2 > k1 + 1u) A.k2 = k2;
            }
        }
        p.gj_a[g] = A;
        p.gj_b[g] = make_uint4(hrow, r, win, (status << 16) | (((uint32_t)row->flags & 0xFFu) << 8) | (has_cp << 1) | (p.strand[r] == (uint8_t)'-' ? 1u : 0u));
        p.gj_c[g] = make_uint2(nr->aln_len, k1);
    }
}
#define RB_GW_WPE 4
__global__ __launch_bounds__(256) __attribute__((amdgpu_waves_per_eu(RB_GW_WPE))) void rb_k_liftover_generic_wave(rb_lift_params p) {
    __shared__ uint32_t run_tot_all[4][64], run_opc_all[4][64];
    const uint32_t wib = threadIdx.x >> 6;
    uint32_t *run_tot = run_tot_all[wib], *run_opc = run_opc_all[wib];
    const int lane = rb_lane();
    const uint64_t n_gen = p.counters->n_generic;
    for (uint64_t g = (uint64_t)blockIdx.x * 4u + wib; g < n_gen; g += (uint64_t)gridDim.x * 4u) {
        const rb_gja A_ = p.gj_a[g];
        const uint4 B_ = p.gj_b[g];
        const uint2 C_ = p.gj_c[g];
        const uint64_t hrow = rb_first(B_.x);
        const uint32_t r = rb_first(B_.y), win = rb_first(B_.z), gfl = rb_first(B_.w);
        rb_hit_row *row = &p.rows[hrow];
        rb_hit_row w;
        w.rec = r;
        w.win = win;
        w.flags = RB_HIT_GENERIC;
        w.status = RB_ST_OK;
        w.out_n = 0;
        w.out_off = 0;
        w.t_st = w.t_en = w.q_st = w.q_en = 0;
        w.nmatch = w.aln_len = 0;
        if ((gfl >> 16) != RB_ST_OK) {
            w.status = (uint16_t)(gfl >> 16);
            w.flags = (uint16_t)((gfl >> 8) & 0xFFu);
            if (lane == 0) *row = w;
            continue;
        }
        const uint64_t t_st = rb_first64(A_.t_st), t_en = rb_first64(A_.t_en), q_st = rb_first64(A_.q_st), q_en = rb_first64(A_.q_en);
        const bool minus = (gfl & 1u) != 0u;
        const uint32_t n = rb_first(A_.n);
        const uint64_t ops_off = rb_first64(A_.ops_off);
        const uint32_t *ops = p.ops + ops_off;
        const uint64_t wst = rb_first64(A_.wst), wen = rb_first64(A_.wen);
        const uint32_t rec_units = rb_first(C_.x);
        const uint32_t arena = (uint32_t)(g % p.n_arena);
        auto reserve = [&](uint32_t padded, uint64_t *off) -> bool {
            unsigned long long b0 = 0;
            if (lane == 0) b0 = atomicAdd(&p.arena_cur[(uint64_t)arena * RB_ARENA_STRIDE], (unsigned long long)padded);
            b0 = rb_first64(b0);
            if (b0 + padded > p.arena_size) {
                if (lane == 0) p.counters->overflow = 1;
                return false;
            }
            *off = p.arena_origin + (uint64_t)arena * p.arena_size + b0;
            return true;
        };
        if (t_st > wst && t_en < wen) {
            w.flags |= RB_HIT_INSIDE;
            w.t_st = t_st, w.t_en = t_en, w.q_st = q_st, w.q_en = q_en;
            w.nmatch = p.norm[r].nmatch, w.aln_len = rec_units;
            w.out_n = n;
            uint64_t off;
            if (reserve((n + 3u) & ~3u, &off)) {
                w.out_off = off;
                for (uint32_t i = (uint32_t)lane; i < n; i += 64u) p.out_ops[off + i] = ops[i];
            }
            if (lane == 0) *row = w;
            continue;
        }
        const int64_t ps = (int64_t)(wst > t_st ? wst : t_st);
        const int64_t pe = (int64_t)(wen < t_en ? wen : t_en) - 1;
        uint32_t c_start = 0, c_end1 = 0;
        uint4 cp0 = make_uint4(0u, 0u, 0u, 0u), cp_e1 = cp0;
        bool first_seen = false, wrapped = false;
        const uint4 *gcp = (gfl & 2u) ? p.gen_cp + (ops_off / RB_GCP + r) : nullptr;
        const uint32_t ncp = (n + RB_GCP - 1u) / RB_GCP;
        auto cp_search = [&](int field, uint64_t target) -> uint32_t {
            uint32_t k1 = 0;
            for (uint32_t kb = 0; kb < ncp; kb += 64u) {
                const uint32_t k = kb + (uint32_t)lane;
                const uint4 c = gcp[k < ncp ? k : 0u];
                const uint64_t m = __ballot(k < ncp && (uint64_t)(field ? c.y : c.x) <= target);
                if (!m) break;
                k1 = kb + (uint32_t)__builtin_popcountll(m) - 1u;
                if (m != ~0ull) break;
            }
            return k1;
        };
        if (gcp) {
            const uint32_t k1 = rb_first(C_.y), k2 = rb_first(A_.k2);
            if (k2) c_end1 = k2 * RB_GCP, cp_e1 = gcp[k2];
            if (k1) {
                c_start = k1 * RB_GCP;
                cp0 = gcp[k1];
                if (t_st == 0) {
                    for (uint32_t c0 = 0; c0 < n && !first_seen; c0 += 64u) {
                        const uint32_t i = c0 + (uint32_t)lane;
                        uint32_t opc = RB_NULL_OP, len = 0u;
                        if (i < n) opc = rb_wopc(ops, i), len = rb_wlen(ops, i);
                        const uint64_t m = __ballot(len != 0u);
                        if (m) {
                            first_seen = true;
                            wrapped = !((__ballot(opc <= 8u && rb_in(RB_REF_MASK, opc)) >> __builtin_ctzll(m)) & 1ull);
                        }
                    }
                }
                first_seen = true;
            }
        }
        uint64_t s_lo = ~0ull, s_hi = 0, e_lo = ~0ull, e_hi = 0;
        uint64_t Ub = cp0.x, Rb = cp0.y;
        auto ld = [&](uint32_t c0_) -> uint32_t { return c0_ + (uint32_t)lane < n ? ops[c0_ + (uint32_t)lane] : 0u; };
#define RB_GW_GROUP 1
#define RB_GW_GROUP3 2
        constexpr int RB_GW_GMAX = RB_GW_GROUP > RB_GW_GROUP3 ? RB_GW_GROUP : RB_GW_GROUP3;
        using rb_g12 = std::integral_constant<int, RB_GW_GROUP>;
        using rb_g3 = std::integral_constant<int, RB_GW_GROUP3>;
        uint32_t wc[RB_GW_GMAX], wx[RB_GW_GMAX];
        uint32_t wcb = 0xFFFFFFFFu, wxb = 0xFFFFFFFFu;
        auto win_fill = [&](auto G_, uint32_t base, uint32_t (&dst)[RB_GW_GMAX], auto &&ldf) {
            constexpr int G = decltype(G_)::value;
#pragma unroll
            for (int k = 0; k < G; k++) dst[k] = ldf(base + 64u * (uint32_t)k);
        };
        auto win_take = [&](auto G_, uint32_t c0_, auto &&ldf) -> uint32_t {
            constexpr int G = decltype(G_)::value;
            const uint32_t d = c0_ - wcb;
            if (wcb == 0xFFFFFFFFu || d >= 64u * G || (d & 63u)) {
                if (c0_ == wxb) {
#pragma unroll
                    for (int k = 0; k < G; k++) wc[k] = wx[k];
                } else {
                    win_fill(G_, c0_, wc, ldf);
                }
                wcb = c0_, wxb = c0_ + 64u * G;
                win_fill(G_, wxb, wx, ldf);
            }
            const uint32_t k = (c0_ - wcb) >> 6;
            uint32_t v = wc[0];
#pragma unroll
            for (int q = 1; q < G; q++) v = k == (uint32_t)q ? wc[q] : v;
            return v;
        };
        auto win_reset = [&]() { wcb = wxb = 0xFFFFFFFFu; };
        for (uint32_t c0 = c_start; c0 < n; c0 += 64u) {
            const uint32_t i = c0 + (uint32_t)lane;
            const uint32_t wv = win_take(rb_g12{}, c0, ld);
            uint32_t opc = rb_opc(wv), len = i < n ? rb_len(wv) : 0u;
            if (opc == RB_OP_CONT) opc = rb_wopc(ops, i), len = rb_wlen(ops, i);
            const bool isref = opc <= 8u && rb_in(RB_REF_MASK, opc);
            const uint32_t iu = rb_wave_scan_incl(len), ir = rb_wave_scan_incl(isref ? len : 0u);
            if (!first_seen) {
                const uint64_t m = __ballot(len != 0u);
                if (m) {
                    first_seen = true;
                    wrapped = t_st == 0 && !((__ballot(isref) >> __builtin_ctzll(m)) & 1ull);
                }
            }
            if (len) {
                const uint64_t U = Ub + iu - len;
                const int64_t tpos = (int64_t)t_st - 1 + (int64_t)(Rb + ir - (isref ? len : 0u));
                if (isref) {
                    if (ps > tpos && ps <= tpos + (int64_t)len) {
                        const uint64_t u = U + (uint64_t)(ps - tpos - 1);
// ... 34 lines not shown
        uint32_t ia = 0, ib = 0, len_a = 0, len_b = 0;
        bool a_set = false, b_set = false;
        {
            uint64_t U0 = cp0.x, R0 = cp0.y, Q0 = cp0.z, M0 = cp0.w;
            uint32_t c_end2 = 0;
            uint4 cp_e2 = cp0;
            if (gcp && ke >= ks) {
                const uint32_t k3 = cp_search(0, ke);
                if (k3 * RB_GCP > c_start + RB_GCP) c_end2 = k3 * RB_GCP, cp_e2 = gcp[k3];
            }
          for (int attempt = 0; attempt < 2; attempt++) {
            bool jumped = false;
            if (attempt) U0 = cp0.x, R0 = cp0.y, Q0 = cp0.z, M0 = cp0.w, a_set = false, b_set = false, a = N, b = 0, c_end2 = 0;
            win_reset();
            for (uint32_t c0 = c_start; c0 < n; c0 += 64u) {
                if (a_set && U0 > ke) break;
                const uint32_t i = c0 + (uint32_t)lane;
                const uint32_t wv = win_take(rb_g12{}, c0, ld);
                uint32_t opc = rb_opc(wv), len = i < n ? rb_len(wv) : 0u;
                if (opc == RB_OP_CONT) opc = rb_wopc(ops, i), len = rb_wlen(ops, i);
                const bool okc = opc <= 8u;
                const bool isref = okc && rb_in(RB_REF_MASK, opc), isq = okc && rb_in(RB_QRY_MASK, opc), ism = okc && rb_in(RB_MATCH_MASK, opc);
                const uint32_t iu = rb_wave_scan_incl(len), ir = rb_wave_scan_incl(isref ? len : 0u), iq = rb_wave_scan_incl(isq ? len : 0u),
                               im = rb_wave_scan_incl(ism ? len : 0u);
                const uint64_t U = U0 + iu - len, R = R0 + ir - (isref ? len : 0u), Q = Q0 + iq - (isq ? len : 0u), M = M0 + im - (ism ? len : 0u);
                if (!a_set) {
                    const uint64_t m = __ballot(ism && len != 0u && U + len > ks);
                    if (m) {
                        const int l = __builtin_ctzll(m);
                        const uint64_t Ul = rb_readlane<uint64_t>(U, l);
                        a = ks > Ul ? ks : Ul;
                        const uint64_t off = a - Ul;
                        Ra = rb_readlane<uint64_t>(R, l) + off, Qa = rb_readlane<uint64_t>(Q, l) + off, Ma = rb_readlane<uint64_t>(M, l) + off;
                        Ua_op = Ul, ia = c0 + (uint32_t)l, len_a = rb_readlane<uint32_t>(len, l);
                        a_set = true;
                    }
                }
                {
                    const uint64_t m = __ballot(ism && len != 0u && U <= ke);
                    if (m) {
                        const int l = 63 - __builtin_clzll(m);
                        const uint64_t Ul = rb_readlane<uint64_t>(U, l);
                        const uint32_t ll = rb_readlane<uint32_t>(len, l);
                        b = Ul + ll - 1 < ke ? Ul + ll - 1 : ke;
                        const uint64_t off = b - Ul;
                        nRb = rb_readlane<uint64_t>(R, l) + off + 1, nQb = rb_readlane<uint64_t>(Q, l) + off + 1, nMb = rb_readlane<uint64_t>(M, l) + off + 1;
                        Ub_op = Ul, ib = c0 + (uint32_t)l, len_b = ll;
                        b_set = true;
                    }
                }
                U0 += rb_readlane<uint32_t>(iu, 63), R0 += rb_readlane<uint32_t>(ir, 63), Q0 += rb_readlane<uint32_t>(iq, 63), M0 += rb_readlane<uint32_t>(im, 63);
                if (a_set && c_end2 > c0 + 64u) {
                    c0 = c_end2 - 64u;
                    U0 = cp_e2.x, R0 = cp_e2.y, Q0 = cp_e2.z, M0 = cp_e2.w;
                    c_end2 = 0, jumped = true, b_set = false;
                }
            }
            if (!jumped || b_set) break;
          }
        }
        if (a > b || a >= N || !a_set || !b_set) {
            w.status = RB_ST_NONE_INDEL;
            if (lane == 0) *row = w;
            continue;
        }
        w.t_st = t_st + Ra;
        w.t_en = t_st + nRb;
        if (!minus) w.q_st = q_st + Qa, w.q_en = q_st + nQb;
        else w.q_st = q_en - nQb, w.q_en = q_en - Qa;
        w.nmatch = (uint32_t)(nMb - Ma);
        w.aln_len = (uint32_t)(b - a + 1);
        uint64_t off;
        if (!reserve((ib - ia + 2u + 3u) & ~3u, &off)) {
            if (lane == 0) *row = w;
            continue;
        }
        uint32_t out_pos = 0, c_tot = 0, c_opc = 0;
        bool has_carry = false;
        auto ld3 = [&](uint32_t c0_) -> uint32_t {
            const uint32_t i_ = c0_ + (uint32_t)lane;
            return (i_ >= ia && i_ <= ib) ? ops[i_] : 0u;
        };
        win_reset();
        for (uint32_t c0 = ia & ~63u; c0 <= ib; c0 += 64u) {
            const uint32_t i = c0 + (uint32_t)lane;
            const uint32_t wv = win_take(rb_g3{}, c0, ld3);
            uint32_t opc = rb_opc(wv), len = rb_len(wv);
            if (opc == RB_OP_CONT) opc = rb_wopc(ops, i), len = rb_wlen(ops, i);
            const bool in = i >= ia && i <= ib && len != 0u;
            uint32_t piece = len;
            if (i == ia) piece = ia == ib ? (uint32_t)(b - a + 1) : (uint32_t)(Ua_op + len_a - a);
            else if (i == ib) piece = (uint32_t)(b - Ub_op + 1);
            {
                const bool inr = i >= ia && i <= ib;
                const uint32_t ptype = rb_prev_lane(opc, has_carry ? c_opc : 0xFFu);
                const bool odd = inr && (len == 0u || rb_opc(wv) == RB_OP_CONT || (piece >> RB_LEN_BITS_WORD) != 0u || (ptype == opc && (lane == 0 || i > ia)));
                if (!__ballot(odd)) {
                    if (has_carry) {
                        if (lane == 0) rb_emit_run(p.out_ops + off + out_pos, c_tot, c_opc);
                        out_pos += 1u + ((c_tot >> RB_LEN_BITS_WORD) ? 1u : 0u);
                    }
                    const uint64_t im = __ballot(inr);
                    const uint32_t cnt = (uint32_t)__builtin_popcountll(im), rank = (uint32_t)__builtin_popcountll(im & ((1ull << lane) - 1ull));
                    if (inr && rank + 1u < cnt) p.out_ops[off + out_pos + rank] = (piece << 4) | opc;
                    out_pos += cnt - 1u;
                    const int last = 63 - __builtin_clzll(im);
                    c_tot = rb_readlane<uint32_t>(piece, last), c_opc = rb_readlane<uint32_t>(opc, last);
                    has_carry = true;
                    continue;
                }
            }
            const uint32_t key = in ? ((uint32_t)lane << 5) | 16u | opc : 0u;
            const uint32_t incl = rb_wave_scan_incl_max_u32(key);
            const uint32_t ckey = has_carry ? 16u | c_opc : 0u;
            uint32_t prev = rb_prev_lane(incl, ckey);
            prev = (prev & 16u) ? prev : ckey;
            const bool start = in && !((prev & 16u) && (prev & 15u) == opc);
            const uint64_t sm = __ballot(start);
            const uint32_t nstarts = (uint32_t)__builtin_popcountll(sm);
            const int32_t ridx = (int32_t)__builtin_popcountll(sm & ((2ull << lane) - 1ull)) - 1;
            run_tot[lane] = 0u;
            __builtin_amdgcn_fence(__ATOMIC_RELEASE, "wavefront");
            __builtin_amdgcn_wave_barrier();
            if (in && ridx >= 0) atomicAdd(&run_tot[ridx], piece);
            if (start) run_opc[ridx] = opc;
            c_tot += rb_wave_sum_u32((in && ridx < 0) ? piece : 0u);
            __builtin_amdgcn_fence(__ATOMIC_ACQ_REL, "wavefront");
            __builtin_amdgcn_wave_barrier();
            if (nstarts) {
                if (has_carry) {
                    const uint32_t cw = 1u + ((c_tot >> RB_LEN_BITS_WORD) ? 1u : 0u);
                    if (lane == 0) rb_emit_run(p.out_ops + off + out_pos, c_tot, c_opc);
                    out_pos += cw;
                }
                const bool mine_out = (uint32_t)lane + 1u < nstarts;
                const uint32_t my_tot = mine_out ? run_tot[lane] : 0u;
                const uint32_t my_words = mine_out ? 1u + ((my_tot >> RB_LEN_BITS_WORD) ? 1u : 0u) : 0u;
                const uint32_t wincl = rb_wave_scan_incl(my_words);
                if (mine_out) rb_emit_run(p.out_ops + off + out_pos + (wincl - my_words), my_tot, run_opc[lane]);
                out_pos += rb_readlane<uint32_t>(wincl, 63);
                c_tot = run_tot[nstarts - 1u], c_opc = run_opc[nstarts - 1u];
                has_carry = true;
            }
            __builtin_amdgcn_wave_barrier();
        }
        if (has_carry) {
            if (lane == 0) rb_emit_run(p.out_ops + off + out_pos, c_tot, c_opc);
            out_pos += 1u + ((c_tot >> RB_LEN_BITS_WORD) ? 1u : 0u);
        }
        w.out_n = out_pos;
        w.out_off = off;
        if (lane == 0) *row = w;
    }
}

__global__ __launch_bounds__(64) void rb_k_finish(rb_lift_params p) {
    unsigned long long mx = 0, sum = 0;
    for (uint32_t a = threadIdx.x; a < p.n_arena; a += 64) {
        const unsigned long long c = p.arena_cur[(uint64_t)a * RB_ARENA_STRIDE];
        mx = c > mx ? c : mx;
        sum += c;
    }
    for (int off = 32; off > 0; off >>= 1) {
        const unsigned long long o = __shfl_xor(mx, off, 64);
        mx = o > mx ? o : mx;
        sum += __shfl_xor(sum, off, 64);
    }
    if (threadIdx.x != 0) return;
    p.counters->out_ops_used = p.arena_origin + sum;
    p.counters->out_ops_needed = p.needed_base + (mx + 3ull) / 4ull * 4ull * p.n_arena + 1024ull * p.n_arena;
    if (p.counters->n_hits > p.rows_cap) p.counters->overflow = 1;
    if (p.n_tiles && !p.debug_skip) {
        p.counters->phase[3] = p.n_tiles;
        p.counters->phase[4] = (uint32_t)*p.fb_count;
    }
    if (p.brk_mode && p.counters->brk_scratch_short) {
        p.counters->overflow = 1;
        const uint64_t have = p.counters->n_hits > p.rows_cap ? p.counters->n_hits : p.rows_cap;
        p.counters->n_hits = have + have / 4u + 1024u;
    }
}

__global__ __launch_bounds__(256) void rb_k_break_gather(rb_lift_params p) {
    const uint64_t t = (uint64_t)blockIdx.x * 256u + threadIdx.x;
    const uint64_t r = t >> 2;
    if (r >= p.n_rec) return;
    const uint64_t h0 = p.hit_off[r], n = p.hit_off[r + 1] - h0, src = p.brk_off[r];
    if (src == ~0ull) return;
    const uint32_t part = (uint32_t)(t & 3u);
    const uint4 *from = reinterpret_cast<const uint4 *>(p.rows + src);
    uint4 *to = reinterpret_cast<uint4 *>(p.rows_final + h0);
    for (uint64_t j = 0; j < n; j++)
        if (h0 + j < p.rows_cap) to[4 * j + part] = from[4 * j + part];
}
extern "C" hipError_t rb_launch_break_gather(const rb_lift_params *p, hipStream_t stream) {
    if (p->n_rec == 0) return hipSuccess;
    hipLaunchKernelGGL(rb_k_copy_clips, dim3(2048), dim3(256), 0, stream, *p);
    hipLaunchKernelGGL(rb_k_break_gather, dim3((unsigned)((p->n_rec * 4 + 255) / 256)), dim3(256), 0, stream, *p);
    return hipGetLastError();
}
__global__ __launch_bounds__(256) void rb_k_break_list_declined(rb_lift_params p) {
    const uint64_t r = (uint64_t)blockIdx.x * 256u + threadIdx.x;
    if (r >= p.n_rec || p.brk_off[r] != ~1ull) return;
    p.brk_off[r] = ~0ull;
    p.hit_off[r] = 0;
    p.brk_decl_list[atomicAdd(p.brk_decl_count, 1ull)] = (uint32_t)r;
}
extern "C" hipError_t rb_launch_break_list_declined(const rb_lift_params *p, hipStream_t stream) {
    if (p->n_rec == 0) return hipSuccess;
    hipLaunchKernelGGL(rb_k_break_list_declined, dim3((unsigned)((p->n_rec + 255) / 256)), dim3(256), 0, stream, *p);
    return hipGetLastError();
}
__global__ __launch_bounds__(256) void rb_k_break_declined_rows(rb_lift_params p) {
    const uint64_t n_list = *p.brk_decl_count;
    for (uint64_t i = (uint64_t)blockIdx.x * 256u + threadIdx.x; i < n_list; i += (uint64_t)gridDim.x * 256u) {
        const uint32_t r = p.brk_decl_list[i];
        const uint64_t h0 = p.hit_off[r], n = p.hit_off[r + 1] - h0;
        for (uint64_t j = 0; j < n; j++) {
            const uint64_t h = h0 + j;
            if (h >= p.rows_cap) break;
            rb_hit_row *row = &p.rows[h];
            row->rec = r;
            row->win = (uint32_t)j;
            row->flags = RB_HIT_GENERIC;
            const unsigned long long g = atomicAdd((unsigned long long *)&p.counters->n_generic, 1ull);
            p.gen_list[g] = (uint32_t)h;
        }
    }
}
extern "C" hipError_t rb_launch_break_declined(const rb_lift_params *p, hipStream_t stream) {
    if (p->n_rec == 0) return hipSuccess;
    hipLaunchKernelGGL(rb_k_break_declined_rows, dim3((unsigned)std::min<uint64_t>((p->n_rec + 255) / 256, 256)), dim3(256), 0, stream, *p);
    if (p->gen_cp) hipLaunchKernelGGL(rb_k_generic_checkpoints, dim3(2048), dim3(256), 0, stream, *p);
    hipLaunchKernelGGL(rb_k_generic_jobs, dim3(1024), dim3(256), 0, stream, *p);
    hipLaunchKernelGGL(rb_k_liftover_generic_wave, dim3(2048), dim3(256), 0, stream, *p);
    hipLaunchKernelGGL(rb_k_finish, dim3(1), dim3(64), 0, stream, *p);
    return hipGetLastError();
}
extern "C" hipError_t rb_launch_count_and_scan(const rb_lift_params *p, uint64_t *block_sums, bool do_count, hipStream_t stream) {
    if (p->n_rec == 0) return hipSuccess;
    if (do_count) {
        const unsigned blocks = (unsigned)((p->n_rec + 255) / 256);
        hipLaunchKernelGGL(rb_k_count_hits, dim3(blocks), dim3(256), 0, stream, *p);
    }
    return rb_launch_exclusive_scan(p->hit_off, p->n_rec, block_sums, &p->counters->n_hits, stream);
}
extern "C" hipError_t rb_launch_exclusive_scan(uint64_t *v, uint64_t n, uint64_t *block_sums, uint64_t *total_out, hipStream_t stream) {
    if (n == 0) return hipSuccess;
    const uint64_t nb = (n + RB_SCAN_PER_BLOCK - 1) / RB_SCAN_PER_BLOCK;
    hipLaunchKernelGGL(rb_k_scan_partial, dim3((unsigned)nb), dim3(256), 0, stream, (const uint64_t *)v, n, block_sums);
    hipLaunchKernelGGL(rb_k_scan_top, dim3(1), dim3(256), 0, stream, block_sums, nb);
    hipLaunchKernelGGL(rb_k_scan_apply, dim3((unsigned)nb), dim3(256), 0, stream, v, n, (const uint64_t *)block_sums, total_out);
    return hipGetLastError();
}
extern "C" hipError_t rb_launch_make_jobs(const rb_lift_params *p, hipStream_t stream) {
    if (p->n_rec == 0) return hipSuccess;
    hipLaunchKernelGGL(rb_k_make_jobs, dim3((unsigned)((p->n_rec + 255) / 256)), dim3(256), 0, stream, *p);
    return hipGetLastError();
}

extern "C" hipError_t rb_launch_liftover_stream(const rb_lift_params *p, hipStream_t stream) {
    if (p->n_rec == 0 || p->wave_end <= p->wave0) return hipSuccess;
    const unsigned blocks = (unsigned)(((uint64_t)(p->wave_end - p->wave0) + 3) / 4);
    if (p->debug_skip) {
        if (!p->brk_mode) {
            hipLaunchKernelGGL(rb_k_liftover_stream_diag, dim3(blocks), dim3(256), 0, stream, *p);
            return hipGetLastError();
        }
    }
    if (p->brk_mode) return rb_launch_liftover_stream_brk(p, blocks, stream);
    hipLaunchKernelGGL(rb_k_liftover_stream, dim3(blocks), dim3(256), 0, stream, *p);
    return hipGetLastError();
}
extern "C" hipError_t rb_launch_liftover_tail(const rb_lift_params *p, hipStream_t stream) {
    if (p->n_rec == 0) return hipSuccess;
    hipLaunchKernelGGL(rb_k_copy_clips, dim3(2048), dim3(256), 0, stream, *p);
    if (p->gen_cp) hipLaunchKernelGGL(rb_k_generic_checkpoints, dim3(2048), dim3(256), 0, stream, *p);
    hipLaunchKernelGGL(rb_k_generic_jobs, dim3(1024), dim3(256), 0, stream, *p);
    hipLaunchKernelGGL(rb_k_liftover_generic_wave, dim3(2048), dim3(256), 0, stream, *p);
    hipLaunchKernelGGL(rb_k_finish, dim3(1), dim3(64), 0, stream, *p);
    return hipGetLastError();
}

extern "C" size_t rb_scan_block_sums_count(uint64_t n_rec) { return (size_t)((n_rec + RB_SCAN_PER_BLOCK - 1) / RB_SCAN_PER_BLOCK + 2); }
```

### rustybam_amd/csrc/k_records.hip

```cpp
#include "rb_device.h"
#include "rb_launch.h"
#include "rb_ratio.h"
#include <algorithm>
#include <type_traits>

struct rb_strip {
    uint32_t lead, trail;
    uint64_t dR, dQ;
    uint64_t t_st, t_en, q_st, q_en;
};
__device__ __forceinline__ rb_strip rb_strip_ends(const uint32_t *ops, uint64_t n, uint64_t t_st, uint64_t t_en, uint64_t q_st, uint64_t q_en,
                                                  bool minus) {
    rb_strip o;
    uint64_t lead = 0, rm_st_t = 0, rm_st_q = 0;
    uint32_t prev = RB_NULL_OP;
    o.dR = o.dQ = 0;
    while (lead < n) {
        uint32_t opc, len;
        const uint32_t words = rb_op_fwd(ops, n, lead, &opc, &len);
        if (!rb_in(RB_INDEL_MASK, opc)) break;
        if (opc == RB_OP_D) {
            rm_st_t += len;
            rm_st_q += 1;
            o.dR += len;
        } else {
            rm_st_q += len;
            o.dQ += len;
        }
        if (prev != RB_NULL_OP && prev != opc) {
            rm_st_t += 1;
            rm_st_q -= 1;
        }
        prev = opc;
        lead += words;
    }
    uint64_t trail = 0, rm_en_t = 0, rm_en_q = 0;
    while (trail < n) {
        uint32_t opc, len;
        const uint32_t words = rb_op_bwd(ops, n - 1 - trail, &opc, &len);
        if (!rb_in(RB_INDEL_MASK, opc)) break;
        if (opc == RB_OP_D) {
            rm_en_t += len;
            if (lead + trail < n) o.dR += len;
        } else {
            rm_en_q += len;
            if (lead + trail < n) o.dQ += len;
        }
        trail += words;
    }
    o.lead = (uint32_t)lead;
    o.trail = (uint32_t)trail;
    o.t_st = t_st + rm_st_t, o.t_en = t_en - rm_en_t;
    if (minus) {
        const uint64_t t = rm_st_q;
        rm_st_q = rm_en_q;
        rm_en_q = t;
    }
    o.q_st = q_st + rm_st_q, o.q_en = q_en - rm_en_q;
    return o;
}

__global__ __launch_bounds__(256) void rb_k_peek_norm(rb_scan_params p) {
    const uint64_t r = (uint64_t)blockIdx.x * blockDim.x + threadIdx.x;
    if (r >= p.n_rec) return;
    const uint64_t o0 = p.op_off[r], n = p.op_off[r + 1] - o0;
    rb_norm_row w;
    w.t_st = w.t_en = w.q_st = w.q_en = 0;
    w.first_op = w.n_ops = w.lead_ops = w.trail_ops = w.nmatch = w.aln_len = 0;
    w.flags = RB_F_PROVISIONAL;
    uint32_t st = RB_ST_OK;
    if (n == 0) {
        st = RB_ST_PANIC_EMPTY_CIGAR;
    } else {
        const bool minus = p.strand && p.strand[r] == (uint8_t)'-';
        const rb_strip sp = rb_strip_ends(p.ops + o0, n, p.t_st[r], p.t_en[r], p.q_st[r], p.q_en[r], minus);
        w.lead_ops = sp.lead;
        w.trail_ops = sp.trail;
        if (sp.lead || sp.trail) w.flags |= RB_F_STRIPPED;
        if ((uint64_t)sp.lead + sp.trail > n) {
            st = RB_ST_PANIC_ALL_INDEL;
        } else {
            w.t_st = sp.t_st, w.t_en = sp.t_en, w.q_st = sp.q_st, w.q_en = sp.q_en;
            w.first_op = sp.lead;
            w.n_ops = (uint32_t)(n - sp.lead - sp.trail);
            const uint32_t fo = rb_opc(p.ops[o0 + sp.lead]), lo_ = rb_opc(p.ops[o0 + n - 1 - sp.trail]);
            if (fo > 8u || lo_ > 8u || !rb_in(RB_MATCH_MASK, fo) || !rb_in(RB_MATCH_MASK, lo_)) w.flags |= RB_F_ENDS_NOT_MATCH;
        }
    }
    if (st != RB_ST_OK) w.flags &= ~(uint32_t)RB_F_PROVISIONAL;
    w.status = st;
    p.norm_rows[r] = w;
}

__device__ __forceinline__ void rb_scan_finish(const rb_scan_params &p, const uint64_t r, const uint64_t (&L)[9], const uint32_t ins_events,
                                               const uint32_t del_events, const uint32_t bad, const uint64_t o0, const uint64_t o1, const uint64_t t_st,
                                               const uint64_t t_en, const uint64_t q_st, const uint64_t q_en, const bool minus) {
    const uint64_t n = o1 - o0;
    const uint64_t R = L[RB_OP_M] + L[RB_OP_D] + L[RB_OP_N] + L[RB_OP_EQ] + L[RB_OP_X];
    const uint64_t Q = L[RB_OP_M] + L[RB_OP_I] + L[RB_OP_S] + L[RB_OP_EQ] + L[RB_OP_X];
    const uint64_t M = L[RB_OP_M] + L[RB_OP_EQ] + L[RB_OP_X];
    uint64_t U = 0;
#pragma unroll
    for (int t = 0; t < 9; t++) U += L[t];
    uint32_t flags = 0;
    if (bad == 0 && U <= 0xFFFFFFFFull) flags |= RB_F_REGULAR;
    if (L[RB_OP_M] != 0) flags |= RB_F_HAS_M;

    if (p.reduce_rows) {
        rb_reduce_row w;
        w.t_bases = R;
        w.q_bases = Q;
        w.nmatch = (uint32_t)M;
        w.aln_len = (uint32_t)U;
        w.equal = (uint32_t)L[RB_OP_EQ];
        w.diff = (uint32_t)(L[RB_OP_X] + L[RB_OP_M]);
        w.ins = (uint32_t)L[RB_OP_I];
        w.del = (uint32_t)L[RB_OP_D];
        w.matches = (uint32_t)L[RB_OP_M];
        w.ins_events = ins_events;
        w.del_events = del_events;
        rb_identity_ratios(w);
        uint32_t st = RB_ST_OK;
        if (U > 0xFFFFFFFFull)
            st = RB_ST_PANIC_OVERFLOW;
        else if (t_en < t_st || t_en - t_st != R)
            st = RB_ST_PANIC_INTEGRITY_T;
        else if (q_en < q_st || q_en - q_st != Q)
            st = RB_ST_PANIC_INTEGRITY_Q;
        w.status = st;
        w.flags = flags;
        p.reduce_rows[r] = w;
    }

    if (p.norm_rows) {
        rb_norm_row w;
        w.t_st = w.t_en = w.q_st = w.q_en = 0;
        w.first_op = w.n_ops = w.lead_ops = w.trail_ops = w.nmatch = w.aln_len = 0;
        w.flags = flags;
        uint32_t st = RB_ST_OK;
        if (n == 0) {
            st = RB_ST_PANIC_EMPTY_CIGAR;
        } else {
            const rb_strip sp = rb_strip_ends(p.ops + o0, n, t_st, t_en, q_st, q_en, minus);
            w.lead_ops = sp.lead;
            w.trail_ops = sp.trail;
            if (sp.lead || sp.trail) w.flags |= RB_F_STRIPPED;
            if ((uint64_t)sp.lead + sp.trail > n) {
                st = RB_ST_PANIC_ALL_INDEL;
            } else {
                const uint64_t Rn = R - sp.dR, Qn = Q - sp.dQ, Un = U - sp.dR - sp.dQ;
                if (Un > 0xFFFFFFFFull)
                    st = RB_ST_PANIC_OVERFLOW;
                else if (sp.t_en < sp.t_st || sp.t_en - sp.t_st != Rn)
                    st = RB_ST_PANIC_INTEGRITY_T;
                else if (sp.q_en < sp.q_st || sp.q_en - sp.q_st != Qn)
                    st = RB_ST_PANIC_INTEGRITY_Q;
                if (st == RB_ST_OK) {
                    w.t_st = sp.t_st;
                    w.t_en = sp.t_en;
                    w.q_st = sp.q_st;
                    w.q_en = sp.q_en;
                    w.first_op = sp.lead;
                    w.n_ops = (uint32_t)(n - sp.lead - sp.trail);
                    w.nmatch = (uint32_t)M;
                    w.aln_len = (uint32_t)Un;
                    const uint32_t fo = rb_opc(p.ops[o0 + sp.lead]), lo_ = rb_opc(p.ops[o1 - 1 - sp.trail]);
                    if (!rb_in(RB_MATCH_MASK, fo) || !rb_in(RB_MATCH_MASK, lo_)) w.flags &= ~(uint32_t)RB_F_REGULAR;
                }
            }
        }
        w.status = st;
        p.norm_rows[r] = w;
    }
}

#define RB_LEN_BITS 40

__global__ __launch_bounds__(256) void rb_k_scan_records(rb_scan_params p) {
    __shared__ unsigned long long hist_all[4][9][64];
    const uint64_t wave0 = (uint64_t)blockIdx.x * 4u + (threadIdx.x >> 6);
    const int lane = rb_lane();
    unsigned long long(*hist)[64] = hist_all[threadIdx.x >> 6];
    const uint64_t n_work = p.list ? rb_first64(*p.n_list) : p.n_rec;
    const uint64_t stride = p.list ? (uint64_t)gridDim.x * 4u : n_work + 1;
  for (uint64_t wave = wave0; wave < n_work; wave += stride) {
    const uint64_t r = p.list ? (uint64_t)rb_first(p.list[wave]) : rb_first64(wave);
    const uint64_t o0 = p.op_off[r], o1 = p.op_off[r + 1];
    const uint64_t n = o1 - o0;
#pragma unroll
    for (int t = 0; t < 9; t++) hist[t][lane] = 0ull;
    uint32_t bad = 0;

    const uint64_t g0 = o0 & ~3ull;
    const int32_t head = (int32_t)(o0 - g0);
    const uint32_t n32 = (uint32_t)n;
    const uint32_t n_steps = n ? (uint32_t)((o1 - g0 + 511u) >> 9) : 0u;
    const uint32_t *__restrict__ gbase = p.ops + g0;
    const uint32_t last_off = n ? (uint32_t)(((o1 - 1u) & ~3ull) - g0) : 0u;
    auto load_half = [&](uint32_t stp, uint32_t half) -> uint4 {
        uint32_t off = (stp << 9) + half * 4u + (uint32_t)lane * 8u;
        off = off < last_off ? off : last_off;
        return *reinterpret_cast<const uint4 *>(gbase + off);
    };
    uint32_t carry_w = 0xFu;
    uint32_t v_reg = 0xFFFFFFFFu, v_minlen = 0xFFFFFFFFu, v_adj = 0xFFFFFFFFu, v_big = 0u;
    uint4 pf[2][2];
    if (n_steps) {
#pragma unroll
        for (int q = 0; q < 2; q++) {
            pf[q][0] = load_half((uint32_t)q, 0u);
            pf[q][1] = load_half((uint32_t)q, 1u);
            __builtin_amdgcn_sched_barrier(0);
        }
    }
    const uint32_t my_hist = (uint32_t)lane;
    for (uint32_t st0 = 0; st0 < n_steps; st0 += 2) {
#pragma unroll
        for (int ring = 0; ring < 2; ring++) {
            const uint32_t st = st0 + (uint32_t)ring;
            if (st < n_steps) {
                const uint32_t raw[8] = {pf[ring][0].x, pf[ring][0].y, pf[ring][0].z, pf[ring][0].w,
                                         pf[ring][1].x, pf[ring][1].y, pf[ring][1].z, pf[ring][1].w};
                const int32_t idx0 = (int32_t)(st << 9) + lane * 8 - head;
                auto step = [&](auto edge_c) {
                    constexpr bool edge = decltype(edge_c)::value;
                    uint32_t mylast = raw[7];
                    if (edge && (uint32_t)(idx0 + 7) >= n32) mylast = 0xFu;
                    uint32_t prevw = rb_prev_lane(mylast, carry_w);
                    carry_w = rb_readlane<uint32_t>(mylast, 63);
#pragma unroll
                    for (int q = 0; q < 8; q++) {
                        const bool ok = !edge || (uint32_t)(idx0 + q) < n32;
                        const uint32_t w = raw[q], opc = w & 15u, len = w >> 4;
                        if (ok) {
                            if (opc <= 8u) {
                                __hip_atomic_fetch_add(&hist[opc][my_hist], (unsigned long long)len | (1ull << RB_LEN_BITS), __ATOMIC_RELAXED,
                                                       __HIP_MEMORY_SCOPE_WORKGROUP);
                            } else {
                                v_big |= 8u;
                                const bool cont = opc == RB_OP_CONT && (prevw & 15u) <= 8u;
                                __hip_atomic_fetch_add(&hist[cont ? (prevw & 15u) : (uint32_t)RB_OP_P][my_hist],
                                                       cont ? (unsigned long long)(len & 15u) << RB_LEN_BITS_WORD : (unsigned long long)len, __ATOMIC_RELAXED,
                                                       __HIP_MEMORY_SCOPE_WORKGROUP);
                            }
// ... 169 lines not shown
```

### rustybam_amd/csrc/rb_launch.h

```cpp
#pragma once
#include <hip/hip_runtime.h>
#include <stdint.h>

#include "../../include/rustybam_amd.h"

struct rb_lift_params;
struct rb_trim_params;
struct nf_read;
struct nf_tdesc;

struct rb_scan_params {
    uint64_t n_rec;
    const uint32_t *ops;
    const uint64_t *op_off;
    const uint64_t *t_st, *t_en, *q_st, *q_en;
    const uint8_t *strand;
    rb_reduce_row *reduce_rows;
    rb_norm_row *norm_rows;
    const uint32_t *list;
    const uint64_t *n_list;
};
extern "C" hipError_t rb_launch_scan_records(const rb_scan_params *p, hipStream_t stream);
extern "C" hipError_t rb_launch_scan_rows(const rb_scan_params *p, void *long_buf, hipStream_t stream);
extern "C" hipError_t rb_launch_peek_norm(const rb_scan_params *p, hipStream_t stream);

extern "C" hipError_t rb_launch_count_and_scan(const rb_lift_params *p, uint64_t *block_sums, bool do_count, hipStream_t stream);
extern "C" hipError_t rb_launch_exclusive_scan(uint64_t *v, uint64_t n, uint64_t *block_sums, uint64_t *total_out, hipStream_t stream);
extern "C" size_t rb_scan_block_sums_count(uint64_t n_rec);
extern "C" hipError_t rb_launch_make_jobs(const rb_lift_params *p, hipStream_t stream);
extern "C" hipError_t rb_launch_liftover_stream(const rb_lift_params *p, hipStream_t stream);
extern "C" hipError_t rb_launch_liftover_tail(const rb_lift_params *p, hipStream_t stream);
extern "C" hipError_t rb_launch_liftover_stream_list(const rb_lift_params *p, hipStream_t stream);
extern "C" hipError_t rb_launch_liftover_stream_brk(const rb_lift_params *p, unsigned blocks, hipStream_t stream);
extern "C" hipError_t rb_launch_liftover_tiles(const rb_lift_params *p, hipStream_t stream);
extern "C" uint32_t rb_tile_max_ops(void);
extern "C" uint32_t rb_tile_max_records(void);
extern "C" hipError_t rb_launch_break_gather(const rb_lift_params *p, hipStream_t stream);
extern "C" hipError_t rb_launch_break_declined(const rb_lift_params *p, hipStream_t stream);
extern "C" hipError_t rb_launch_break_list_declined(const rb_lift_params *p, hipStream_t stream);

struct rb_break_params {
    uint64_t n_rec;
    const uint32_t *ops;
    const uint64_t *op_off;
    const rb_norm_row *norm;
    const uint32_t *sched;
    uint64_t *hit_off;
    uint64_t *x_st, *x_en;
    uint64_t rows_cap;
    uint32_t max_size;
    int fill;
    int redo_only;
    uint2 *tmp;
    uint64_t *tmp_off;
    unsigned long long *tmp_cursor;
    uint32_t n_arena;
    uint64_t arena_cap;
    const uint32_t *list;
    const unsigned long long *n_list;
};
struct rb_swap_params {
    uint64_t n_rec;
    const uint32_t *ops;
    const uint64_t *op_off;
    const uint8_t *strand;
    uint32_t *out_ops;
};
struct rb_digest_params {
    const uint32_t *ops;
    const uint64_t *op_off;
    const rb_hit_row *rows;
    uint64_t n_rows;
    const uint32_t *out_ops;
    uint64_t row_base, rec_base;
    unsigned long long *digest;
};
struct rb_compact_params {
    uint64_t n_rows;
    rb_hit_row *rows;
    const uint32_t *src;
    uint64_t *off;
    uint32_t *dst;
    int fill;
};
extern "C" hipError_t rb_launch_break_pieces(const rb_break_params *p, hipStream_t stream);
extern "C" hipError_t rb_launch_break_place(const rb_break_params *p, hipStream_t stream);
extern "C" hipError_t rb_launch_swap(const rb_swap_params *p, hipStream_t stream);
extern "C" hipError_t rb_launch_swap_inplace(const rb_swap_params *p, hipStream_t stream);
extern "C" hipError_t rb_launch_starts_check(const uint64_t *op_off, const rb_norm_row *norm, uint64_t n_rec, uint64_t n_ops, unsigned long long *bad,
                                             hipStream_t stream);
extern "C" hipError_t rb_launch_synth(uint64_t seed, uint64_t first_record, uint64_t n_rec, const uint64_t *op_off, uint32_t *ops, hipStream_t stream);
extern "C" hipError_t rb_launch_digest_rows(const rb_digest_params *p, hipStream_t stream);
extern "C" hipError_t rb_launch_compact_clips(const rb_compact_params *p, hipStream_t stream);
extern "C" hipError_t rb_launch_box_probe(const void *src, void *d0, void *d1, uint64_t n_stretch, uint32_t *stamps, int scatter, hipStream_t stream);

struct rb_parse_params {
    uint64_t n_rec;
    const uint8_t *text;
    const uint64_t *text_off;
    const uint64_t *text_end;
    uint64_t *op_off;
    uint32_t *ops;
    uint64_t ops_cap;
    uint8_t *status;
};
struct rb_format_params {
    uint64_t n_items;
    const uint32_t *ops;
    const uint32_t *ops_alt;
    const uint64_t *first;
    const uint32_t *count;
    const uint32_t *first_len;
    const uint32_t *last_len;
    uint64_t *text_off;
    uint8_t *text;
    uint64_t text_cap;
    int plain_ops;
};
extern "C" hipError_t rb_launch_parse_cigars(const rb_parse_params *p, bool fill, hipStream_t stream);
extern "C" hipError_t rb_launch_format_cigars(const rb_format_params *p, bool fill, hipStream_t stream);

struct rb_apply_params {
    uint64_t n_pairs;
    const uint32_t *left, *right;
    const rb_pair_row *rows;
    uint64_t *op_off;
    rb_norm_row *norm;
};
struct rb_gather_params {
    uint64_t n_rec;
    const uint32_t *ops;
    const uint64_t *op_off;
    const rb_norm_row *norm;
    uint64_t *new_off;
    uint32_t *new_ops;
    int fill;
};
struct rb_tsel_params {
    uint64_t n_groups;
    const uint32_t *order;
    const uint64_t *grp_off;
    const rb_norm_row *norm;
    uint8_t *contained;
    uint64_t *slot;
    uint64_t *has;
    uint32_t *cand;
    uint64_t out_base;
    uint32_t *left, *right;
    uint64_t *pair_out_off;
    rb_trim_pass *pass;
};
extern "C" hipError_t rb_launch_overlap_split(const rb_trim_params *p, hipStream_t stream);
extern "C" hipError_t rb_launch_overlap_split_quad(const rb_trim_params *p, int t, bool from_list, hipStream_t stream);
extern "C" size_t rb_trim_scratch_bytes(uint32_t blocks);
extern "C" hipError_t rb_launch_apply_pairs(const rb_apply_params *p, hipStream_t stream);
extern "C" hipError_t rb_launch_gather_records(const rb_gather_params *p, hipStream_t stream);
extern "C" hipError_t rb_launch_trim_select(const rb_tsel_params *p, uint64_t *block_sums, hipStream_t stream);
extern "C" hipError_t rb_launch_trim_check(const rb_pair_row *rows, uint64_t n_pairs, rb_trim_pass *pass, hipStream_t stream);

struct rb_largest_params {
    const rb_hit_row *rows;
    uint64_t n_rows;
    const uint32_t *win_key;
    const uint32_t *rec_key;
    uint64_t n_keys;
    unsigned long long *best_span;
    unsigned long long *best_row;
    uint64_t *sel;
    unsigned long long *out;
    uint32_t *worst_status;
};
extern "C" hipError_t rb_launch_largest(const rb_largest_params *p, uint64_t *block_sums, hipStream_t stream);
extern "C" hipError_t rb_launch_largest_rec_keys(const rb_norm_row *norm, uint64_t n_rec, uint32_t inside_key, uint32_t *rec_key, hipStream_t stream);
extern "C" hipError_t rb_launch_largest_gather(const rb_hit_row *rows, const uint32_t *out_ops, const uint64_t *sel, uint64_t n_sel, rb_hit_row *sel_rows,
                                               uint32_t *sel_desc, hipStream_t stream);

struct rb_pairs_params {
    const rb_hit_row *rows;
    uint64_t n_rows;
// ... 131 lines not shown
```

### rustybam_amd/csrc/rb_lift.h

```cpp
#pragma once
#include "rb_device.h"
#include <cstdlib>


#define RB_HMAX 32
#define RB_LDS_PER_HIT 6
#define RB_ARENA_STRIDE 16
#define RB_MS 2

struct __attribute__((aligned(64))) rb_job {
    uint64_t rec0;
    uint32_t n;
    uint32_t r;
    uint32_t h0;
    uint32_t flags;
    uint32_t nh;
    uint32_t lo;
    uint64_t t_st, t_en, q_st, q_en;
};
enum { RB_JOB_VALID = 1, RB_JOB_REGULAR = 2, RB_JOB_MINUS = 4, RB_JOB_MONO = 8, RB_JOB_ROWS_OVERFLOW = 16 };

struct rb_lift_params {
    uint64_t n_rec;
    const uint32_t *ops;
    const uint64_t *op_off;
    const uint32_t *contig;
    const uint8_t *strand;
    const rb_norm_row *norm;
    const uint32_t *sched;
    const uint32_t *slot_of;
    const uint32_t *canon_pos;
    const uint64_t *w_st, *w_en;
    const uint32_t *w_orig;
    const uint64_t *wo_st, *wo_en;
    const uint64_t *cw_off;
    const uint8_t *cw_mono;
    uint32_t n_contig;
    const uint64_t *x_st, *x_en;
    uint64_t *hit_off;
    uint32_t *win_lo;
    rb_hit_row *rows;
    uint64_t rows_cap;
    uint32_t *out_ops;
    uint64_t out_cap;
    unsigned long long *arena_cur;
    uint64_t arena_size;
    uint32_t n_arena;
    uint32_t *gen_list;
    rb_counters *counters;
    int policy;
    int early_exit;
    int desc_mode;
    uint64_t arena_origin;
    int debug_skip;
    uint32_t wave0, wave_end;
    rb_job *jobs;
    int fused;
    rb_norm_row *norm_w;
    uint32_t *pend_list;
    unsigned long long *pend_count;
    uint32_t n_slots;
    uint64_t slot_stride;
    uint64_t needed_base;
    uint4 *copy_list;
    unsigned long long *copy_count;
    int brk_mode;
    uint32_t brk_max;
    uint32_t brk_n_arena;
    uint64_t brk_arena_cap;
    unsigned long long *brk_cursor;
    uint64_t *brk_off;
    rb_hit_row *rows_final;
    uint32_t *brk_decl_list;
    unsigned long long *brk_decl_count;
    uint4 *gen_cp;
    uint32_t *diag_stamps;
    struct rb_gja *gj_a;
    uint4 *gj_b;
    uint2 *gj_c;
    const uint32_t *tile_first;
    uint32_t n_tiles;
    uint32_t *fb_list;
    unsigned long long *fb_count;
    int op_starts;
};
#define RB_GCP 64u
struct __attribute__((aligned(64))) rb_gja {
    uint64_t ops_off;
    uint64_t t_st, t_en, q_st, q_en;
    uint64_t wst, wen;
    uint32_t n;
    uint32_t k2;
};

typedef const __attribute__((address_space(4))) rb_lift_params *rb_kparams;
__device__ __forceinline__ rb_kparams rb_kp_here(rb_kparams q) {
    asm volatile("" : "+s"(q));
    return q;
}

__device__ __forceinline__ uint64_t rb_lower_en_gt(const uint64_t *w_en, uint64_t lo, uint64_t hi, uint64_t t_st) {
    while (lo < hi) {
        uint64_t mid = lo + ((hi - lo) >> 1);
        if (w_en[mid] > t_st) hi = mid; else lo = mid + 1;
    }
    return lo;
}
__device__ __forceinline__ uint64_t rb_lower_st_ge(const uint64_t *w_st, uint64_t lo, uint64_t hi, uint64_t t_en) {
    while (lo < hi) {
        uint64_t mid = lo + ((hi - lo) >> 1);
        if (w_st[mid] >= t_en) hi = mid; else lo = mid + 1;
    }
    return lo;
}

enum { RB_S_UNRES = 0, RB_S_OK = 1, RB_S_NONE = 2, RB_S_DEFER = 3 };

__device__ __forceinline__ int rb_ffs64(unsigned long long m) { return __ffsll((long long)m) - 1; }

__device__ inline void rb_defer_record(rb_kparams kp, uint32_t r, const rb_norm_row *nr, uint64_t h0, uint64_t nh,
                                bool explicit_w, bool mono, uint64_t ws, uint64_t we, int lane) {
    asm volatile("" : "+v"(lane));
    const rb_kparams q_ = rb_kp_here(kp);
    struct { const uint64_t *w_st, *w_en; const uint32_t *w_orig; rb_hit_row *rows; uint64_t rows_cap; uint32_t *gen_list; rb_counters *counters; } p =
        {q_->w_st, q_->w_en, q_->w_orig, q_->rows, q_->rows_cap, q_->gen_list, q_->counters};
    if (explicit_w || mono) {
        uint64_t lo = 0;
        if (!explicit_w) lo = rb_lower_en_gt(p.w_en, ws, we, nr->t_st);
        for (uint64_t j = lane; j < nh; j += 64) {
            const uint64_t h = h0 + j;
            if (h < p.rows_cap) {
                rb_hit_row *row = &p.rows[h];
                row->rec = r;
                row->win = explicit_w ? (uint32_t)j : p.w_orig[lo + j];
                row->flags = RB_HIT_GENERIC;
                const unsigned long long g = atomicAdd((unsigned long long *)&p.counters->n_generic, 1ull);
                p.gen_list[g] = (uint32_t)h;
            }
        }
    } else {
        uint64_t done = 0;
        for (uint64_t b = ws; b < we; b += 64) {
            const uint64_t i = b + lane;
            const bool hit = i < we && nr->t_en > p.w_st[i] && nr->t_st < p.w_en[i];
            const unsigned long long ball = __ballot(hit);
            if (hit) {
                const uint64_t j = done + __popcll(ball & ((1ull << lane) - 1ull));
                const uint64_t h = h0 + j;
                if (h < p.rows_cap) {
                    rb_hit_row *row = &p.rows[h];
                    row->rec = r;
                    row->win = p.w_orig[i];
                    row->flags = RB_HIT_GENERIC;
                    const unsigned long long g = atomicAdd((unsigned long long *)&p.counters->n_generic, 1ull);
                    p.gen_list[g] = (uint32_t)h;
                }
            }
            done += __popcll(ball);
        }
    }
}

struct rb_bres {
    uint32_t st;
    uint32_t op, part;
    uint32_t R, Q, U;
};

__device__ __forceinline__ uint32_t rb_part_pack(uint32_t part, uint32_t op_word) { return part | (op_word << 28); }
__device__ __forceinline__ uint32_t rb_part(uint32_t packed) { return packed & 0x0FFFFFFFu; }
__device__ __forceinline__ uint32_t rb_part_word(uint32_t packed) { return (packed << 4) | (packed >> 28); }

#define RB_WALK_MAX 24

__device__ __forceinline__ uint32_t rb_rl(uint32_t v) { return rb_opc(v) == RB_OP_I ? 0u : rb_len(v); }
__device__ __forceinline__ uint32_t rb_ql(uint32_t v) { return (rb_opc(v) == RB_OP_D || rb_opc(v) == RB_OP_N) ? 0u : rb_len(v); }
__device__ __forceinline__ bool rb_ism(uint32_t v) { return rb_in(RB_MATCH_MASK, rb_opc(v)); }

#define RB_CP_OPS 8
__device__ __forceinline__ rb_bres rb_resolve_group(const uint32_t *__restrict__ ops, uint32_t n, int32_t cidx, const uint32_t (&g)[8],
                                                    uint32_t pv, uint32_t cR, uint32_t cQ, uint32_t cU, uint32_t D, bool is_start, int policy) {
    rb_bres o;
    o.st = RB_S_DEFER;
    o.op = o.part = o.R = o.Q = o.U = 0;
    uint32_t np = 0, fR = cR, fQ = cQ, fU = cU, fv = 0;
    {
        uint32_t R = cR, Q = cQ, U = cU;
        bool before = true;
#pragma unroll
        for (int k = 0; k < RB_CP_OPS; k++) {
            const uint32_t v = (uint32_t)(cidx + k) < n ? g[k] : 0u;
            const uint32_t len = rb_len(v);
            R += len & (uint32_t)__builtin_amdgcn_sbfe((int)0xFFFDFFFDu, v, 1u);
            Q += len & (uint32_t)__builtin_amdgcn_sbfe((int)0xFFF3FFF3u, v, 1u);
            U += len;
            const bool pk = R <= D;
            fv = (before && !pk) ? v : fv;
            np += pk ? 1u : 0u;
            fR = pk ? R : fR;
            fQ = pk ? Q : fQ;
            fU = pk ? U : fU;
            pv = pk ? v : pv;
            before = pk;
        }
    }
    if (np >= (uint32_t)RB_CP_OPS) return o;
    const int32_t fi = cidx + (int32_t)np;
    const uint32_t off = D - fR;
    if (is_start) {
        int32_t X;
        if (off > 0) {
            if (rb_ism(fv)) {
                o.st = RB_S_OK, o.op = (uint32_t)fi, o.part = rb_part_pack(rb_len(fv) - (off - 1), fv), o.R = fR + off - 1, o.Q = fQ + off - 1, o.U = fU + off - 1;
                return o;
            }
            X = fi + 1;
        } else {
            if (fi > 0 && rb_ism(pv)) {
                o.st = RB_S_OK, o.op = (uint32_t)(fi - 1), o.part = rb_part_pack(1u, pv), o.R = fR - 1, o.Q = fQ - 1, o.U = fU - 1;
                return o;
            }
            if (policy == RB_BSEARCH_LEGACY && fi > 0 && rb_opc(pv) == RB_OP_I) return o;
            X = fi;
        }
        uint32_t R = fR, Q = fQ, U = fU;
        uint32_t v = fv;
        int32_t i = fi;
#pragma nounroll
        for (int t = 0; t < RB_WALK_MAX; t++) {
            if (i >= X && rb_ism(v)) {
                o.st = RB_S_OK, o.op = (uint32_t)i, o.part = rb_part_pack(rb_len(v), v), o.R = R, o.Q = Q, o.U = U;
                return o;
            }
            R += rb_rl(v);
            Q += rb_ql(v);
            U += rb_len(v);
            i++;
            if ((uint32_t)i >= n) {
                o.st = RB_S_NONE;
                return o;
            }
            v = ops[i];
        }
        return o;
    } else {
        int32_t Y;
        if (off > 0) {
            if (rb_ism(fv)) {
                o.st = RB_S_OK, o.op = (uint32_t)fi, o.part = rb_part_pack(off, fv), o.R = D, o.Q = fQ + off, o.U = fU + off;
                return o;
            }
            Y = fi - 1;
        } else {
            if (fi > 0 && rb_ism(pv)) {
                o.st = RB_S_OK, o.op = (uint32_t)(fi - 1), o.part = rb_part_pack(rb_len(pv), pv), o.R = fR, o.Q = fQ, o.U = fU;
                return o;
            }
            Y = fi - 2;
        }
        uint32_t R = fR, Q = fQ, U = fU;
        int32_t i = fi - 1;
#pragma nounroll
        for (int t = 0; t < RB_WALK_MAX; t++) {
            if (i < 0) {
                o.st = RB_S_NONE;
                return o;
// ... 104 lines not shown
```

Before: 561.3 billion.

## Fuse liftover setup: zeroing, peek-norm, hit count and job creation in one kernel

Replaces several memset fills, the peek-norm kernel, the count-hits kernel and the separate make-jobs kernel with a single setup kernel that zeroes counters, normalises each record, runs both window binary searches interleaved, writes hit counts and pre-builds jobs. The scan's apply pass then patches h0 into the jobs through a new precomputed slot_of_canon table, so make_jobs is skipped on the non-break path. This cuts launch count and redundant passes over records at the price of a more complex setup kernel, an extra plan table, and job fields being written twice.

New measurement: 561.3 billion. No clear change (-0.0%).

```diff
diff --git a/include/rustybam_amd.h b/include/rustybam_amd.h
--- a/include/rustybam_amd.h
+++ b/include/rustybam_amd.h
@@ -158,6 +158,8 @@
 void rb_plan_destroy(rb_plan *plan);
 int64_t rb_plan_tiles_host(uint64_t n_rec, const uint64_t *op_off_host, uint64_t short_max, uint32_t *sched_out, uint32_t *tiles_out,
                            uint64_t tiles_cap, uint64_t *n_long_out);
+int rb_plan_tables_host(uint64_t n_rec, const uint64_t *op_off_host, const uint32_t *contig_host, int identity, uint32_t *slot_of_out,
+                        uint32_t *canon_pos_out, uint32_t *slot_of_canon_out);
 size_t rb_plan_workspace_bytes(const rb_plan *plan, uint64_t rows_cap);
 size_t rb_plan_diag_stamps_offset(const rb_plan *plan, uint64_t rows_cap);
 uint64_t rb_plan_out_capacity(const rb_plan *plan, int for_break);
diff --git a/rustybam_amd/csrc/capi.hip b/rustybam_amd/csrc/capi.hip
--- a/rustybam_amd/csrc/capi.hip
+++ b/rustybam_amd/csrc/capi.hip
@@ -84,6 +84,7 @@
     uint32_t n_contig = 0;
     uint32_t depth = 0;
     uint32_t *sched = nullptr, *slot_of = nullptr, *canon_pos = nullptr, *w_orig = nullptr, *ident = nullptr;
+    uint32_t *slot_of_canon = nullptr;
     uint64_t *w_st = nullptr, *w_en = nullptr, *wo_st = nullptr, *wo_en = nullptr, *cw_off = nullptr;
     uint8_t *cw_mono = nullptr;
     uint32_t *tiles = nullptr;
@@ -626,6 +627,80 @@
     return (int64_t)nt;
 }
 
+struct rb_plan_orders {
+    std::vector<uint32_t> canon_pos, sched, slot_of, slot_of_canon, tiles;
+    uint32_t stream_end = 0;
+};
+static void rb_plan_order(uint64_t n_rec, const uint64_t *op_off, const uint32_t *contig, uint32_t n_contig, rb_plan_orders &o) {
+    std::vector<uint32_t> &canon_pos = o.canon_pos;
+    canon_pos.assign(n_rec, 0);
+    {
+        std::vector<uint64_t> rank(n_contig, UINT64_MAX);
+        uint64_t nr = 0;
+        for (uint64_t i = 0; i < n_rec; i++)
+            if (rank[contig[i]] == UINT64_MAX) rank[contig[i]] = nr++;
+        std::vector<uint64_t> start(nr + 1, 0);
+        for (uint64_t i = 0; i < n_rec; i++) start[rank[contig[i]] + 1]++;
+        for (uint64_t k = 0; k < nr; k++) start[k + 1] += start[k];
+        for (uint64_t i = 0; i < n_rec; i++) canon_pos[i] = (uint32_t)start[rank[contig[i]]]++;
+    }
+    std::vector<uint32_t> &sched = o.sched;
+    {
+        uint64_t max_len = 0;
+        std::vector<uint64_t> key(n_rec);
+        for (uint64_t i = 0; i < n_rec; i++) key[i] = op_off[i + 1] - op_off[i], max_len = std::max(max_len, key[i]);
+        int passes = 0;
+        while (passes < 4 && (max_len >> (16 * passes)) != 0) passes++;
+        std::vector<uint32_t> a(n_rec), b(n_rec);
+        std::iota(a.begin(), a.end(), 0u);
+        std::vector<uint64_t> cnt(65537);
+        for (int ps = 0; ps < passes; ps++) {
+            std::fill(cnt.begin(), cnt.end(), 0);
+            const int sh = 16 * ps;
+            for (uint64_t i = 0; i < n_rec; i++) cnt[(0xFFFFu - (uint32_t)((key[i] >> sh) & 0xFFFFu)) + 1]++;
+            for (int k = 0; k < 65536; k++) cnt[k + 1] += cnt[k];
+            for (uint64_t i = 0; i < n_rec; i++) {
+                const uint32_t r = a[i];
+                b[cnt[0xFFFFu - (uint32_t)((key[r] >> sh) & 0xFFFFu)]++] = r;
+            }
+            a.swap(b);
+        }
+        sched = a;
+    }
+    o.tiles.clear();
+    o.stream_end = (uint32_t)n_rec;
+    {
+        const char *e = getenv("RB_TILE");
+        const bool on = !(e && !strcmp(e, "0"));
+        uint64_t short_max = RB_SHORT_MAX_DEFAULT;
+        if (const char *m = getenv("RB_SHORT_MAX")) short_max = strtoull(m, nullptr, 10);
+        if (on && n_rec) {
+            uint64_t n_long = 0;
+            rb_cut_tiles(n_rec, op_off, short_max, sched, o.tiles, &n_long);
+            if (!o.tiles.empty()) o.stream_end = (uint32_t)n_long;
+        }
+    }
+    o.slot_of.assign(n_rec, 0);
+    for (uint64_t w = 0; w < n_rec; w++) o.slot_of[sched[w]] = (uint32_t)w;
+    o.slot_of_canon.assign(n_rec, 0);
+    for (uint64_t r = 0; r < n_rec; r++) o.slot_of_canon[canon_pos[r]] = o.slot_of[r];
+}
+extern "C" int rb_plan_tables_host(uint64_t n_rec, const uint64_t *op_off, const uint32_t *contig, int identity, uint32_t *slot_of_out,
+                                   uint32_t *canon_pos_out, uint32_t *slot_of_canon_out) {
+    if (n_rec && (!op_off || !contig || !slot_of_out || !canon_pos_out || !slot_of_canon_out)) return -1;
+    if (n_rec >= 0xFFFFFFFFull) return -1;
+    uint32_t maxc = 0;
+    for (uint64_t i = 0; i < n_rec; i++) maxc = std::max(maxc, contig[i]);
+    rb_plan_orders o;
+    rb_plan_order(n_rec, op_off, contig, n_rec ? maxc + 1 : 0, o);
+    for (uint64_t i = 0; i < n_rec; i++) {
+        slot_of_out[i] = o.slot_of[i];
+        canon_pos_out[i] = identity ? (uint32_t)i : o.canon_pos[i];
+        slot_of_canon_out[i] = identity ? o.slot_of[i] : o.slot_of_canon[i];
+    }
+    return 0;
+}
+
 extern "C" int rb_plan_create(rb_ctx *ctx, uint64_t n_rec, const uint64_t *op_off, const uint32_t *contig, uint64_t n_win,
                               const uint32_t *w_contig, const uint64_t *w_st, const uint64_t *w_en, rb_plan **out) {
     if (!ctx || !out || (n_rec && (!op_off || !contig))) return RB_E_INVALID;
@@ -640,40 +715,10 @@
     for (uint64_t i = 0; i < n_win; i++) maxc = std::max(maxc, w_contig[i]);
     const uint32_t n_contig = (n_rec || n_win) ? maxc + 1 : 0;
     pl->n_contig = n_contig;
-    std::vector<uint32_t> canon_pos(n_rec);
-    {
-        std::vector<uint64_t> rank(n_contig, UINT64_MAX);
-        uint64_t nr = 0;
-        for (uint64_t i = 0; i < n_rec; i++)
-            if (rank[contig[i]] == UINT64_MAX) rank[contig[i]] = nr++;
-        std::vector<uint64_t> start(nr + 1, 0);
-        for (uint64_t i = 0; i < n_rec; i++) start[rank[contig[i]] + 1]++;
-        for (uint64_t k = 0; k < nr; k++) start[k + 1] += start[k];
-        for (uint64_t i = 0; i < n_rec; i++) canon_pos[i] = (uint32_t)start[rank[contig[i]]]++;
-    }
-    std::vector<uint32_t> sched(n_rec), ident(n_rec);
+    rb_plan_orders o;
+    rb_plan_order(n_rec, op_off, contig, n_contig, o);
+    std::vector<uint32_t> ident(n_rec);
     std::iota(ident.begin(), ident.end(), 0u);
-    {
-        uint64_t max_len = 0;
-        std::vector<uint64_t> key(n_rec);
-        for (uint64_t i = 0; i < n_rec; i++) key[i] = op_off[i + 1] - op_off[i], max_len = std::max(max_len, key[i]);
-        int passes = 0;
-        while (passes < 4 && (max_len >> (16 * passes)) != 0) passes++;
-        std::vector<uint32_t> a(ident), b(n_rec);
-        std::vector<uint64_t> cnt(65537);
-        for (int ps = 0; ps < passes; ps++) {
-            std::fill(cnt.begin(), cnt.end(), 0);
-            const int sh = 16 * ps;
-            for (uint64_t i = 0; i < n_rec; i++) cnt[(0xFFFFu - (uint32_t)((key[i] >> sh) & 0xFFFFu)) + 1]++;
-            for (int k = 0; k < 65536; k++) cnt[k + 1] += cnt[k];
-            for (uint64_t i = 0; i < n_rec; i++) {
-                const uint32_t r = a[i];
-                b[cnt[0xFFFFu - (uint32_t)((key[r] >> sh) & 0xFFFFu)]++] = r;
-            }
-            a.swap(b);
-        }
-        sched = a;
-    }
     std::vector<uint64_t> cw_off(n_contig + 1, 0), g_st(n_win), g_en(n_win), o_st(n_win), o_en(n_win);
     std::vector<uint32_t> g_orig(n_win);
     std::vector<uint8_t> mono(n_contig ? n_contig : 1, 1);
@@ -702,27 +747,14 @@
             pl->depth = std::max<uint32_t>(pl->depth, (uint32_t)std::min<uint64_t>(i - lo + 1, 1u << 20));
         }
     }
-    std::vector<uint32_t> tiles;
-    pl->stream_end = (uint32_t)n_rec;
-    {
-        const char *e = getenv("RB_TILE");
-        const bool on = !(e && !strcmp(e, "0"));
-        uint64_t short_max = RB_SHORT_MAX_DEFAULT;
-        if (const char *m = getenv("RB_SHORT_MAX")) short_max = strtoull(m, nullptr, 10);
-        if (on && n_rec) {
-            uint64_t n_long = 0;
-            rb_cut_tiles(n_rec, op_off, short_max, sched, tiles, &n_long);
-            if (!tiles.empty()) pl->stream_end = (uint32_t)n_long;
-        }
-        pl->n_tiles = (uint32_t)(tiles.size() / 3);
-    }
+    pl->stream_end = o.stream_end;
+    pl->n_tiles = (uint32_t)(o.tiles.size() / 3);
     int rc = RB_OK;
-    std::vector<uint32_t> slot_of(n_rec);
-    for (uint64_t w = 0; w < n_rec; w++) slot_of[sched[w]] = (uint32_t)w;
-    if (!rc) rc = upload_vec(ctx, sched, &pl->sched);
-    if (!rc) rc = upload_vec(ctx, slot_of, &pl->slot_of);
+    if (!rc) rc = upload_vec(ctx, o.sched, &pl->sched);
+    if (!rc) rc = upload_vec(ctx, o.slot_of, &pl->slot_of);
+    if (!rc) rc = upload_vec(ctx, o.slot_of_canon, &pl->slot_of_canon);
     if (!rc) rc = upload_vec(ctx, ident, &pl->ident);
-    if (!rc) rc = upload_vec(ctx, canon_pos, &pl->canon_pos);
+    if (!rc) rc = upload_vec(ctx, o.canon_pos, &pl->canon_pos);
     if (!rc) rc = upload_vec(ctx, g_st, &pl->w_st);
     if (!rc) rc = upload_vec(ctx, g_en, &pl->w_en);
     if (!rc) rc = upload_vec(ctx, g_orig, &pl->w_orig);
@@ -730,7 +762,7 @@
     if (!rc) rc = upload_vec(ctx, o_en, &pl->wo_en);
     if (!rc) rc = upload_vec(ctx, cw_off, &pl->cw_off);
     if (!rc) rc = upload_vec(ctx, mono, &pl->cw_mono);
-    if (!rc && pl->n_tiles) rc = upload_vec(ctx, tiles, &pl->tiles);
+    if (!rc && pl->n_tiles) rc = upload_vec(ctx, o.tiles, &pl->tiles);
     if (!rc && hipStreamSynchronize(ctx->stream) != hipSuccess) rc = fail(ctx, RB_E_HIP, "plan upload: %s", hipGetErrorString(hipGetLastError()));
     if (rc) {
         rb_plan_destroy(pl);
@@ -741,7 +773,7 @@
 }
 extern "C" void rb_plan_destroy(rb_plan *pl) {
     if (!pl) return;
-    void *ptrs[] = {pl->sched, pl->slot_of, pl->ident, pl->canon_pos, pl->w_st, pl->w_en, pl->w_orig, pl->wo_st, pl->wo_en, pl->cw_off, pl->cw_mono, pl->tiles};
+    void *ptrs[] = {pl->sched, pl->slot_of, pl->slot_of_canon, pl->ident, pl->canon_pos, pl->w_st, pl->w_en, pl->w_orig, pl->wo_st, pl->wo_en, pl->cw_off, pl->cw_mono, pl->tiles};
     for (void *q : ptrs)
         if (q) (void)rb_dev_free(pl->ctx, q);
     delete pl;
@@ -900,18 +932,30 @@
         sp.t_st = b->t_st, sp.t_en = b->t_en, sp.q_st = b->q_st, sp.q_en = b->q_en;
         sp.strand = b->strand;
         sp.norm_rows = p.norm_w;
-        HIPCHK(ctx, rb_fill_async(p.pend_count, 0, 8, ctx->stream));
-        HIPCHK(ctx, rb_launch_peek_norm(&sp, ctx->stream));
     }
     p.counters = counters;
     p.policy = policy & 1;
     p.early_exit = (policy & RB_LIFT_EARLY_EXIT) ? 1 : 0;
     p.debug_skip = (policy >> 8) & 0xFFF;
     uint64_t *block_sums = (uint64_t *)(ws + w.block_sums);
-    HIPCHK(ctx, rb_fill_async(counters, 0, sizeof(rb_counters), ctx->stream));
-    HIPCHK(ctx, rb_fill_async(p.copy_count, 0, 8, ctx->stream));
-    HIPCHK(ctx, rb_fill_async(p.arena_cur, 0, (size_t)RB_MAX_ARENA * RB_ARENA_STRIDE * 8, ctx->stream));
+    rb_setup_params su;
+    memset(&su, 0, sizeof su);
+    su.counters = counters;
+    su.pend_count = p.pend_count, su.copy_count = p.copy_count, su.fb_count = p.fb_count, su.arena_cur = p.arena_cur;
+    su.n_zero = sizeof(rb_counters) / 8 + 4 + p.n_arena;
+    su.records = !is_break && b->n_rec != 0;
+    su.fused = p.fused;
+    su.n_rec = b->n_rec;
+    su.ops = b->ops, su.op_off = b->op_off;
+    su.t_st = b->t_st, su.t_en = b->t_en, su.q_st = b->q_st, su.q_en = b->q_en;
+    su.strand = b->strand, su.contig = b->contig;
+    su.norm = p.norm_w;
+    su.slot_of = p.slot_of, su.canon_pos = p.canon_pos;
+    su.w_st = p.w_st, su.w_en = p.w_en, su.cw_off = p.cw_off, su.cw_mono = p.cw_mono, su.n_contig = p.n_contig;
+    su.hit_off = p.hit_off, su.win_lo = p.win_lo, su.jobs = p.jobs;
+    HIPCHK(ctx, rb_launch_lift_setup(&su, ctx->stream));
     if (b->n_rec == 0) return RB_OK;
+    if (is_break && p.fused) HIPCHK(ctx, rb_launch_peek_norm(&sp, ctx->stream));
     const bool one_walk = is_break && (policy & RB_BREAK_ONE_WALK) && !p.desc_mode;
     if (one_walk) {
         p.brk_mode = 1, p.brk_max = max_size;
@@ -934,7 +978,6 @@
         p.wave_end = stream_end;
         HIPCHK(ctx, rb_launch_liftover_stream(&p, ctx->stream));
         if (use_tiles) {
-            HIPCHK(ctx, rb_fill_async(p.fb_count, 0, 8, ctx->stream));
             HIPCHK(ctx, rb_launch_liftover_tiles(&p, ctx->stream));
             HIPCHK(ctx, rb_launch_liftover_stream_list(&p, ctx->stream));
         }
@@ -956,7 +999,7 @@
         bp.fill = 0;
         HIPCHK(ctx, rb_launch_break_list_declined(&p, ctx->stream));
         HIPCHK(ctx, rb_launch_break_pieces(&bp, ctx->stream));
-        HIPCHK(ctx, rb_launch_count_and_scan(&p, block_sums, false, ctx->stream));
+        HIPCHK(ctx, rb_launch_exclusive_scan(p.hit_off, p.n_rec, block_sums, &counters->n_hits, ctx->stream));
         bp.fill = 1;
         HIPCHK(ctx, rb_launch_break_pieces(&bp, ctx->stream));
         HIPCHK(ctx, rb_launch_break_gather(&p, ctx->stream));
@@ -986,19 +1029,18 @@
         HIPCHK(ctx, rb_fill_async(bp.tmp_cursor, 0, (size_t)RB_MAX_ARENA * 128, ctx->stream));
         bp.fill = 2, bp.redo_only = 0;
         HIPCHK(ctx, rb_launch_break_pieces(&bp, ctx->stream));
-        HIPCHK(ctx, rb_launch_count_and_scan(&p, block_sums, false, ctx->stream));
+        HIPCHK(ctx, rb_launch_exclusive_scan(p.hit_off, p.n_rec, block_sums, &counters->n_hits, ctx->stream));
         HIPCHK(ctx, rb_launch_break_place(&bp, ctx->stream));
         bp.fill = 1, bp.redo_only = 1;
         HIPCHK(ctx, rb_launch_break_pieces(&bp, ctx->stream));
         p.x_st = bp.x_st;
         p.x_en = bp.x_en;
     } else {
-        HIPCHK(ctx, rb_launch_count_and_scan(&p, block_sums, true, ctx->stream));
+        HIPCHK(ctx, rb_launch_scan_jobs(&p, plan->slot_of_canon, block_sums, ctx->stream));
     }
     const char *tb = getenv("RB_TILE_BESIDE");
     const bool beside = use_tiles && !is_break && stream_end != 0 && !(tb && atoi(tb) == 0);
-    if (use_tiles && !is_break) HIPCHK(ctx, rb_fill_async(p.fb_count, 0, 8, ctx->stream));
-    HIPCHK(ctx, rb_launch_make_jobs(&p, ctx->stream));
+    if (is_break) HIPCHK(ctx, rb_launch_make_jobs(&p, ctx->stream));
     const size_t slot = (size_t)(ctx->timed_calls % RB_TIMING_RING);
     if (beside) HIPCHK(ctx, hipEventRecord(ctx->ev_fork, ctx->stream));
     if (ctx->timing) HIPCHK(ctx, hipEventRecord(ctx->ev_a[slot], ctx->stream));
@@ -1019,7 +1061,6 @@
     } else {
         HIPCHK(ctx, rb_launch_liftover_stream(&p, ctx->stream));
         if (use_tiles) {
-            if (is_break) HIPCHK(ctx, rb_fill_async(p.fb_count, 0, 8, ctx->stream));
             HIPCHK(ctx, rb_launch_liftover_tiles(&p, ctx->stream));
             HIPCHK(ctx, rb_launch_liftover_stream_list(&p, ctx->stream));
         }
diff --git a/rustybam_amd/csrc/k_liftover.hip b/rustybam_amd/csrc/k_liftover.hip
--- a/rustybam_amd/csrc/k_liftover.hip
+++ b/rustybam_amd/csrc/k_liftover.hip
@@ -2,27 +2,6 @@
 #include "rb_launch.h"
 #include <type_traits>
 #include <algorithm>
-
-__global__ __launch_bounds__(256) void rb_k_count_hits(rb_lift_params p) {
-    const uint64_t r = (uint64_t)blockIdx.x * blockDim.x + threadIdx.x;
-    if (r >= p.n_rec) return;
-    uint64_t cnt = 0;
-    const rb_norm_row *nr = &p.norm[r];
-    const uint32_t c = p.contig[r];
-    if (nr->status == RB_ST_OK && c < p.n_contig) {
-        const uint64_t ws = p.cw_off[c], we = p.cw_off[c + 1];
-        const uint64_t t_st = nr->t_st, t_en = nr->t_en;
-        if (p.cw_mono[c]) {
-            const uint64_t lo = rb_lower_en_gt(p.w_en, ws, we, t_st);
-            const uint64_t hi = rb_lower_st_ge(p.w_st, ws, we, t_en);
-            cnt = hi > lo ? hi - lo : 0;
-            p.win_lo[r] = (uint32_t)lo;
-        } else {
-            for (uint64_t i = ws; i < we; i++) cnt += (t_en > p.w_st[i] && t_st < p.w_en[i]) ? 1 : 0;
-        }
-    }
-    p.hit_off[p.canon_pos[r]] = cnt;
-}
 
 #define RB_SCAN_PER_BLOCK 2048
 __global__ __launch_bounds__(256) void rb_k_scan_partial(const uint64_t *v, uint64_t n, uint64_t *block_sums) {
@@ -93,38 +72,62 @@
         if (total_out) *total_out = total;
     }
 }
+__global__ __launch_bounds__(256) void rb_k_scan_apply_jobs(uint64_t *v, uint64_t n, const uint64_t *block_sums, uint64_t *total_out,
+                                                            const uint32_t *slot_of_canon, rb_job *jobs, uint64_t rows_cap) {
+    __shared__ uint64_t sh[256];
+    __shared__ uint64_t front[4];
+    const uint64_t base = (uint64_t)blockIdx.x * RB_SCAN_PER_BLOCK;
+    uint64_t f = 0;
+    for (uint32_t b = threadIdx.x; b < blockIdx.x; b += 256u) f += block_sums[b];
+    f = rb_wave_sum_u64(f);
+    if ((threadIdx.x & 63) == 0) front[threadIdx.x >> 6] = f;
+    uint64_t x[RB_SCAN_PER_BLOCK / 256];
+    uint64_t s = 0;
+    const uint64_t i0 = base + (uint64_t)threadIdx.x * (RB_SCAN_PER_BLOCK / 256);
+#pragma unroll
+    for (int k = 0; k < RB_SCAN_PER_BLOCK / 256; k++) {
+        x[k] = (i0 + k < n) ? v[i0 + k] : 0;
+        s += x[k];
+    }
+    sh[threadIdx.x] = s;
+    __syncthreads();
+    for (int off = 1; off < 256; off <<= 1) {
+        uint64_t y = threadIdx.x >= (unsigned)off ? sh[threadIdx.x - off] : 0;
+        __syncthreads();
+        sh[threadIdx.x] += y;
+        __syncthreads();
+    }
+    uint64_t run = front[0] + front[1] + front[2] + front[3] + sh[threadIdx.x] - s;
+#pragma unroll
+    for (int k = 0; k < RB_SCAN_PER_BLOCK / 256; k++) {
+        if (i0 + k < n) {
+            v[i0 + k] = run;
+            rb_job *j = &jobs[slot_of_canon[i0 + k]];
+            j->h0 = (uint32_t)run;
+            if (run + x[k] > rows_cap) {
+                const uint32_t fl = j->flags;
+                if (fl & RB_JOB_VALID) j->flags = (fl & ~(uint32_t)RB_JOB_VALID) | RB_JOB_ROWS_OVERFLOW, j->lo = 0u;
+            }
+        }
+        run += x[k];
+    }
+    if (blockIdx.x == gridDim.x - 1 && threadIdx.x == 255) {
+        v[n] = run;
+        if (total_out) *total_out = run;
+    }
+}
 
 __global__ __launch_bounds__(256) void rb_k_make_jobs(rb_lift_params p) {
     const uint64_t r64 = (uint64_t)blockIdx.x * blockDim.x + threadIdx.x;
     if (r64 >= p.n_rec) return;
     const uint32_t r = (uint32_t)r64;
-    const uint64_t w = p.slot_of[r];
-    const rb_norm_row *nr = &p.norm[r];
-    rb_job j;
-    j.r = r;
-    j.n = nr->n_ops;
-    j.rec0 = p.op_off[r] + nr->first_op;
-    j.t_st = nr->t_st, j.t_en = nr->t_en, j.q_st = nr->q_st, j.q_en = nr->q_en;
     const uint64_t k = p.canon_pos[r];
     const bool brk = p.brk_mode != 0;
     const uint64_t h0 = brk ? 0ull : p.hit_off[k], nh = brk ? 1ull : p.hit_off[k + 1] - h0;
     const bool explicit_w = brk || p.x_st != nullptr;
     const uint32_t cg = p.contig[r];
     const bool mono = explicit_w || (cg < p.n_contig && p.cw_mono[cg] != 0);
-    uint32_t f = 0;
-    const bool provisional = (nr->flags & RB_F_PROVISIONAL) != 0;
-    if (nr->status == RB_ST_OK && (nh != 0 || provisional)) {
-        if (h0 + nh > p.rows_cap) f |= RB_JOB_ROWS_OVERFLOW;
-        else f |= RB_JOB_VALID;
-    }
-    if ((nr->flags & RB_F_REGULAR) || (provisional && !(nr->flags & RB_F_ENDS_NOT_MATCH))) f |= RB_JOB_REGULAR;
-    if (p.strand[r] == (uint8_t)'-') f |= RB_JOB_MINUS;
-    if (mono) f |= RB_JOB_MONO;
-    j.flags = f;
-    j.h0 = (uint32_t)h0;
-    j.nh = (uint32_t)nh;
-    j.lo = (explicit_w || !mono || !(f & RB_JOB_VALID) || nh == 0) ? 0u : p.win_lo[r];
-    p.jobs[w] = j;
+    p.jobs[p.slot_of[r]] = rb_make_job(r, p.norm[r], p.op_off[r], p.strand[r] == (uint8_t)'-', mono, explicit_w, h0, nh, &p.win_lo[r], p.rows_cap);
 }
 
 #define RB_RING_BASE 88
@@ -140,10 +143,10 @@
 RB_STREAM_KERNEL(rb_k_liftover_stream, false, false, RB_SPILL_ROOM)
 RB_STREAM_KERNEL(rb_k_liftover_stream_diag, false, true, 5)
 
-__global__ __launch_bounds__(256) void rb_k_copy_clips(rb_lift_params p) {
+__device__ __forceinline__ void rb_copy_clips_loop(const rb_lift_params &p, uint32_t block, uint32_t n_blocks) {
     const uint64_t n_copy = *p.copy_count;
     const int lane = rb_lane();
-    for (uint64_t e = (uint64_t)blockIdx.x * 4u + (threadIdx.x >> 6); e < n_copy; e += (uint64_t)gridDim.x * 4u) {
+    for (uint64_t e = (uint64_t)block * 4u + (threadIdx.x >> 6); e < n_copy; e += (uint64_t)n_blocks * 4u) {
         const uint4 d = p.copy_list[e];
         rb_hit_row *row = &p.rows[d.x];
         const uint32_t rec = row->rec, n = row->out_n;
@@ -173,6 +176,7 @@
         if (lane == 0) row->out_off = off;
     }
 }
+__global__ __launch_bounds__(256) void rb_k_copy_clips(rb_lift_params p) { rb_copy_clips_loop(p, blockIdx.x, gridDim.x); }
 
 struct rb_gwalk {
     const uint32_t *ops;
@@ -457,12 +461,12 @@
 __device__ __forceinline__ uint4 *rb_gen_cp_of(const rb_lift_params &p, uint32_t r, uint32_t first_op) {
     return p.gen_cp + ((p.op_off[r] + first_op) / RB_GCP + r);
 }
-__global__ __launch_bounds__(256) void rb_k_generic_checkpoints(rb_lift_params p) {
+__device__ __forceinline__ void rb_generic_checkpoints_loop(const rb_lift_params &p, uint32_t block, uint32_t n_blocks) {
     static_assert(RB_GCP == 64u, "one 16-byte load per lane covers four checkpoint intervals: lanes 0, 16, 32, 48 stand at their starts");
     const uint32_t wib = threadIdx.x >> 6;
     const int lane = rb_lane();
     const uint64_t n_gen = p.counters->n_generic;
-    for (uint64_t g = (uint64_t)blockIdx.x * 4u + wib; g < n_gen; g += (uint64_t)gridDim.x * 4u) {
+    for (uint64_t g = (uint64_t)block * 4u + wib; g < n_gen; g += (uint64_t)n_blocks * 4u) {
         const uint32_t r = p.rows[p.gen_list[g]].rec;
         if (g > 0 && p.rows[p.gen_list[g - 1]].rec == r) continue;
         const rb_norm_row *nr = &p.norm[r];
@@ -509,6 +513,12 @@
         }
     }
 }
+__global__ __launch_bounds__(256) void rb_k_generic_checkpoints(rb_lift_params p) { rb_generic_checkpoints_loop(p, blockIdx.x, gridDim.x); }
+#define RB_TAIL_HALF 2048u
+__global__ __launch_bounds__(256) void rb_k_copy_and_checkpoints(rb_lift_params p) {
+    if (blockIdx.x < RB_TAIL_HALF) rb_copy_clips_loop(p, blockIdx.x, RB_TAIL_HALF);
+    else rb_generic_checkpoints_loop(p, blockIdx.x - RB_TAIL_HALF, RB_TAIL_HALF);
+}
 __device__ __forceinline__ uint64_t rb_wave_min_u64(uint64_t v) {
 #pragma unroll
     for (int off = 32; off > 0; off >>= 1) {
@@ -566,9 +576,57 @@
         p.gj_c[g] = make_uint2(nr->aln_len, k1);
     }
 }
+__device__ __forceinline__ void rb_finish(const rb_lift_params &p, int lane) {
+    unsigned long long mx = 0, sum = 0;
+    for (uint32_t a = (uint32_t)lane; a < p.n_arena; a += 64) {
+        const unsigned long long c = __hip_atomic_load(&p.arena_cur[(uint64_t)a * RB_ARENA_STRIDE], __ATOMIC_RELAXED, __HIP_MEMORY_SCOPE_AGENT);
+        mx = c > mx ? c : mx;
+        sum += c;
+    }
+    for (int off = 32; off > 0; off >>= 1) {
+        const unsigned long long o = __shfl_xor(mx, off, 64);
+        mx = o > mx ? o : mx;
+        sum += __shfl_xor(sum, off, 64);
+    }
+    if (lane != 0) return;
+    p.counters->out_ops_used = p.arena_origin + sum;
+    p.counters->out_ops_needed = p.needed_base + (mx + 3ull) / 4ull * 4ull * p.n_arena + 1024ull * p.n_arena;
+    if (p.counters->n_hits > p.rows_cap) p.counters->overflow = 1;
+    if (p.n_tiles && !p.debug_skip) {
+        p.counters->phase[3] = p.n_tiles;
+        p.counters->phase[4] = (uint32_t)*p.fb_count;
+    }
+    if (p.brk_mode && p.counters->brk_scratch_short) {
+        p.counters->overflow = 1;
+        const uint64_t have = p.counters->n_hits > p.rows_cap ? p.counters->n_hits : p.rows_cap;
+        p.counters->n_hits = have + have / 4u + 1024u;
+    }
+}
+__device__ __forceinline__ void rb_finish_last(const rb_lift_params &p, uint64_t n_gen, uint32_t *is_last, int lane) {
+    const uint64_t want = (n_gen + 3u) / 4u;
+    const uint32_t busy = want < gridDim.x ? (uint32_t)want : gridDim.x;
+    if (busy == 0u) {
+        if (blockIdx.x == 0u && threadIdx.x < 64u) rb_finish(p, lane);
+        return;
+    }
+    if (blockIdx.x >= busy) return;
+    asm volatile("s_waitcnt vmcnt(0)" ::: "memory");
+    __syncthreads();
+    if (threadIdx.x == 0u) {
+        __threadfence();
+        asm volatile("s_waitcnt vmcnt(0)" ::: "memory");
+        const unsigned long long t = atomicAdd(rb_tail_ticket(p.copy_count), 1ull);
+        *is_last = t + 1ull == (unsigned long long)busy ? 1u : 0u;
+        if (t + 1ull == (unsigned long long)busy) __threadfence();
+    }
+    __syncthreads();
+    if (*is_last != 0u && threadIdx.x < 64u) rb_finish(p, lane);
+}
+
 #define RB_GW_WPE 4
 __global__ __launch_bounds__(256) __attribute__((amdgpu_waves_per_eu(RB_GW_WPE))) void rb_k_liftover_generic_wave(rb_lift_params p) {
     __shared__ uint32_t run_tot_all[4][64], run_opc_all[4][64];
+    __shared__ uint32_t fin_is_last;
     const uint32_t wib = threadIdx.x >> 6;
     uint32_t *run_tot = run_tot_all[wib], *run_opc = run_opc_all[wib];
     const int lane = rb_lane();
@@ -909,33 +967,7 @@
         w.out_off = off;
         if (lane == 0) *row = w;
     }
-}
-
-__global__ __launch_bounds__(64) void rb_k_finish(rb_lift_params p) {
-    unsigned long long mx = 0, sum = 0;
-    for (uint32_t a = threadIdx.x; a < p.n_arena; a += 64) {
-        const unsigned long long c = p.arena_cur[(uint64_t)a * RB_ARENA_STRIDE];
-        mx = c > mx ? c : mx;
-        sum += c;
-    }
-    for (int off = 32; off > 0; off >>= 1) {
-        const unsigned long long o = __shfl_xor(mx, off, 64);
-        mx = o > mx ? o : mx;
-        sum += __shfl_xor(sum, off, 64);
-    }
-    if (threadIdx.x != 0) return;
-    p.counters->out_ops_used = p.arena_origin + sum;
-    p.counters->out_ops_needed = p.needed_base + (mx + 3ull) / 4ull * 4ull * p.n_arena + 1024ull * p.n_arena;
-    if (p.counters->n_hits > p.rows_cap) p.counters->overflow = 1;
-    if (p.n_tiles && !p.debug_skip) {
-        p.counters->phase[3] = p.n_tiles;
-        p.counters->phase[4] = (uint32_t)*p.fb_count;
-    }
-    if (p.brk_mode && p.counters->brk_scratch_short) {
-        p.counters->overflow = 1;
-        const uint64_t have = p.counters->n_hits > p.rows_cap ? p.counters->n_hits : p.rows_cap;
-        p.counters->n_hits = have + have / 4u + 1024u;
-    }
+    rb_finish_last(p, n_gen, &fin_is_last, lane);
 }
 
 __global__ __launch_bounds__(256) void rb_k_break_gather(rb_lift_params p) {
@@ -991,16 +1023,15 @@
     if (p->gen_cp) hipLaunchKernelGGL(rb_k_generic_checkpoints, dim3(2048), dim3(256), 0, stream, *p);
     hipLaunchKernelGGL(rb_k_generic_jobs, dim3(1024), dim3(256), 0, stream, *p);
     hipLaunchKernelGGL(rb_k_liftover_generic_wave, dim3(2048), dim3(256), 0, stream, *p);
-    hipLaunchKernelGGL(rb_k_finish, dim3(1), dim3(64), 0, stream, *p);
     return hipGetLastError();
 }
-extern "C" hipError_t rb_launch_count_and_scan(const rb_lift_params *p, uint64_t *block_sums, bool do_count, hipStream_t stream) {
+extern "C" hipError_t rb_launch_scan_jobs(const rb_lift_params *p, const uint32_t *slot_of_canon, uint64_t *block_sums, hipStream_t stream) {
     if (p->n_rec == 0) return hipSuccess;
-    if (do_count) {
-        const unsigned blocks = (unsigned)((p->n_rec + 255) / 256);
-        hipLaunchKernelGGL(rb_k_count_hits, dim3(blocks), dim3(256), 0, stream, *p);
-    }
-    return rb_launch_exclusive_scan(p->hit_off, p->n_rec, block_sums, &p->counters->n_hits, stream);
+    const uint64_t nb = (p->n_rec + RB_SCAN_PER_BLOCK - 1) / RB_SCAN_PER_BLOCK;
+    hipLaunchKernelGGL(rb_k_scan_partial, dim3((unsigned)nb), dim3(256), 0, stream, (const uint64_t *)p->hit_off, p->n_rec, block_sums);
+    hipLaunchKernelGGL(rb_k_scan_apply_jobs, dim3((unsigned)nb), dim3(256), 0, stream, p->hit_off, p->n_rec, (const uint64_t *)block_sums,
+                       (uint64_t *)&p->counters->n_hits, slot_of_canon, p->jobs, p->rows_cap);
+    return hipGetLastError();
 }
 extern "C" hipError_t rb_launch_exclusive_scan(uint64_t *v, uint64_t n, uint64_t *block_sums, uint64_t *total_out, hipStream_t stream) {
     if (n == 0) return hipSuccess;
@@ -1031,11 +1062,9 @@
 }
 extern "C" hipError_t rb_launch_liftover_tail(const rb_lift_params *p, hipStream_t stream) {
     if (p->n_rec == 0) return hipSuccess;
-    hipLaunchKernelGGL(rb_k_copy_clips, dim3(2048), dim3(256), 0, stream, *p);
-    if (p->gen_cp) hipLaunchKernelGGL(rb_k_generic_checkpoints, dim3(2048), dim3(256), 0, stream, *p);
+    hipLaunchKernelGGL(rb_k_copy_and_checkpoints, dim3(p->gen_cp ? 2u * RB_TAIL_HALF : RB_TAIL_HALF), dim3(256), 0, stream, *p);
     hipLaunchKernelGGL(rb_k_generic_jobs, dim3(1024), dim3(256), 0, stream, *p);
     hipLaunchKernelGGL(rb_k_liftover_generic_wave, dim3(2048), dim3(256), 0, stream, *p);
-    hipLaunchKernelGGL(rb_k_finish, dim3(1), dim3(64), 0, stream, *p);
     return hipGetLastError();
 }
 
diff --git a/rustybam_amd/csrc/k_records.hip b/rustybam_amd/csrc/k_records.hip
--- a/rustybam_amd/csrc/k_records.hip
+++ b/rustybam_amd/csrc/k_records.hip
@@ -1,5 +1,6 @@
 #include "rb_device.h"
 #include "rb_launch.h"
+#include "rb_lift.h"
 #include "rb_ratio.h"
 #include <algorithm>
 #include <type_traits>
@@ -60,10 +61,8 @@
     return o;
 }
 
-__global__ __launch_bounds__(256) void rb_k_peek_norm(rb_scan_params p) {
-    const uint64_t r = (uint64_t)blockIdx.x * blockDim.x + threadIdx.x;
-    if (r >= p.n_rec) return;
-    const uint64_t o0 = p.op_off[r], n = p.op_off[r + 1] - o0;
+__device__ __forceinline__ rb_norm_row rb_peek_row(const uint32_t *ops, const uint64_t o0, const uint64_t n, const uint64_t t_st, const uint64_t t_en,
+                                                   const uint64_t q_st, const uint64_t q_en, const bool minus) {
     rb_norm_row w;
     w.t_st = w.t_en = w.q_st = w.q_en = 0;
     w.first_op = w.n_ops = w.lead_ops = w.trail_ops = w.nmatch = w.aln_len = 0;
@@ -72,8 +71,7 @@
     if (n == 0) {
         st = RB_ST_PANIC_EMPTY_CIGAR;
     } else {
-        const bool minus = p.strand && p.strand[r] == (uint8_t)'-';
-        const rb_strip sp = rb_strip_ends(p.ops + o0, n, p.t_st[r], p.t_en[r], p.q_st[r], p.q_en[r], minus);
+        const rb_strip sp = rb_strip_ends(ops + o0, n, t_st, t_en, q_st, q_en, minus);
         w.lead_ops = sp.lead;
         w.trail_ops = sp.trail;
         if (sp.lead || sp.trail) w.flags |= RB_F_STRIPPED;
@@ -83,13 +81,75 @@
             w.t_st = sp.t_st, w.t_en = sp.t_en, w.q_st = sp.q_st, w.q_en = sp.q_en;
             w.first_op = sp.lead;
             w.n_ops = (uint32_t)(n - sp.lead - sp.trail);
-            const uint32_t fo = rb_opc(p.ops[o0 + sp.lead]), lo_ = rb_opc(p.ops[o0 + n - 1 - sp.trail]);
+            const uint32_t fo = rb_opc(ops[o0 + sp.lead]), lo_ = rb_opc(ops[o0 + n - 1 - sp.trail]);
             if (fo > 8u || lo_ > 8u || !rb_in(RB_MATCH_MASK, fo) || !rb_in(RB_MATCH_MASK, lo_)) w.flags |= RB_F_ENDS_NOT_MATCH;
         }
     }
     if (st != RB_ST_OK) w.flags &= ~(uint32_t)RB_F_PROVISIONAL;
     w.status = st;
-    p.norm_rows[r] = w;
+    return w;
+}
+__global__ __launch_bounds__(256) void rb_k_peek_norm(rb_scan_params p) {
+    const uint64_t r = (uint64_t)blockIdx.x * blockDim.x + threadIdx.x;
+    if (r >= p.n_rec) return;
+    const uint64_t o0 = p.op_off[r];
+    p.norm_rows[r] = rb_peek_row(p.ops, o0, p.op_off[r + 1] - o0, p.t_st[r], p.t_en[r], p.q_st[r], p.q_en[r], p.strand && p.strand[r] == (uint8_t)'-');
+}
+
+__global__ __launch_bounds__(256) void rb_k_lift_setup(rb_setup_params p) {
+    const uint64_t r = (uint64_t)blockIdx.x * blockDim.x + threadIdx.x;
+    if (r < p.n_zero) {
+        constexpr uint64_t NC = sizeof(rb_counters) / 8;
+        static_assert(sizeof(rb_counters) % 8 == 0, "the counters are zeroed as 64-bit words");
+        unsigned long long *z = r < NC       ? (unsigned long long *)p.counters + r
+                                : r == NC     ? p.pend_count
+                                : r == NC + 1 ? p.copy_count
+                                : r == NC + 2 ? rb_tail_ticket(p.copy_count)
+                                : r == NC + 3 ? p.fb_count
+                                              : p.arena_cur + (r - (NC + 4)) * RB_ARENA_STRIDE;
+        *z = 0ull;
+    }
+    if (!p.records || r >= p.n_rec) return;
+    const uint64_t o0 = p.op_off[r];
+    const bool minus = p.strand[r] == (uint8_t)'-';
+    const uint32_t c = p.contig[r];
+    const bool known = c < p.n_contig;
+    const bool mono = known && p.cw_mono[c] != 0;
+    const uint64_t ws = known ? p.cw_off[c] : 0, we = known ? p.cw_off[c + 1] : 0;
+    rb_norm_row w;
+    uint64_t l = 0, h = 0;
+    bool searched = false;
+    if (p.fused) {
+        const uint64_t n = p.op_off[r + 1] - o0, t0 = p.t_st[r], t1 = p.t_en[r];
+        uint32_t e0 = 0, e1 = 0;
+        if (n) e0 = p.ops[o0], e1 = p.ops[o0 + n - 1];
+        if (mono && n) rb_lower_both(p.w_en, p.w_st, ws, we, t0, t1, &l, &h), searched = true;
+        asm volatile("" ::"v"(e0), "v"(e1));
+        w = rb_peek_row(p.ops, o0, n, t0, t1, p.q_st[r], p.q_en[r], minus);
+        if (w.t_st != t0 || w.t_en != t1) searched = false;
+        p.norm[r] = w;
+    } else {
+        w = p.norm[r];
+    }
+    uint64_t cnt = 0;
+    uint32_t lo = 0;
+    if (w.status == RB_ST_OK && known) {
+        if (mono) {
+            if (!searched) rb_lower_both(p.w_en, p.w_st, ws, we, w.t_st, w.t_en, &l, &h);
+            cnt = h > l ? h - l : 0;
+            lo = (uint32_t)l;
+            p.win_lo[r] = lo;
+        } else {
+            for (uint64_t i = ws; i < we; i++) cnt += (w.t_en > p.w_st[i] && w.t_st < p.w_en[i]) ? 1 : 0;
+        }
+    }
+    p.hit_off[p.canon_pos[r]] = cnt;
+    p.jobs[p.slot_of[r]] = rb_make_job((uint32_t)r, w, o0, minus, mono, false, 0ull, cnt, &lo, ~0ull);
+}
+extern "C" hipError_t rb_launch_lift_setup(const rb_setup_params *p, hipStream_t stream) {
+    const uint64_t threads = std::max<uint64_t>(p->records ? p->n_rec : 0, p->n_zero);
+    hipLaunchKernelGGL(rb_k_lift_setup, dim3((unsigned)((threads + 255) / 256)), dim3(256), 0, stream, *p);
+    return hipGetLastError();
 }
 
 __device__ __forceinline__ void rb_scan_finish(const rb_scan_params &p, const uint64_t r, const uint64_t (&L)[9], const uint32_t ins_events,
diff --git a/rustybam_amd/csrc/rb_launch.h b/rustybam_amd/csrc/rb_launch.h
--- a/rustybam_amd/csrc/rb_launch.h
+++ b/rustybam_amd/csrc/rb_launch.h
@@ -23,8 +23,30 @@
 extern "C" hipError_t rb_launch_scan_records(const rb_scan_params *p, hipStream_t stream);
 extern "C" hipError_t rb_launch_scan_rows(const rb_scan_params *p, void *long_buf, hipStream_t stream);
 extern "C" hipError_t rb_launch_peek_norm(const rb_scan_params *p, hipStream_t stream);
-
-extern "C" hipError_t rb_launch_count_and_scan(const rb_lift_params *p, uint64_t *block_sums, bool do_count, hipStream_t stream);
+struct rb_job;
+struct rb_setup_params {
+    rb_counters *counters;
+    unsigned long long *pend_count, *copy_count, *fb_count, *arena_cur;
+    uint64_t n_zero;
+    int records, fused;
+    uint64_t n_rec;
+    const uint32_t *ops;
+    const uint64_t *op_off;
+    const uint64_t *t_st, *t_en, *q_st, *q_en;
+    const uint8_t *strand;
+    const uint32_t *contig;
+    rb_norm_row *norm;
+    const uint32_t *slot_of, *canon_pos;
+    const uint64_t *w_st, *w_en, *cw_off;
+    const uint8_t *cw_mono;
+    uint32_t n_contig;
+    uint64_t *hit_off;
+    uint32_t *win_lo;
+    rb_job *jobs;
+};
+extern "C" hipError_t rb_launch_lift_setup(const rb_setup_params *p, hipStream_t stream);
+
+extern "C" hipError_t rb_launch_scan_jobs(const rb_lift_params *p, const uint32_t *slot_of_canon, uint64_t *block_sums, hipStream_t stream);
 extern "C" hipError_t rb_launch_exclusive_scan(uint64_t *v, uint64_t n, uint64_t *block_sums, uint64_t *total_out, hipStream_t stream);
 extern "C" size_t rb_scan_block_sums_count(uint64_t n_rec);
 extern "C" hipError_t rb_launch_make_jobs(const rb_lift_params *p, hipStream_t stream);
diff --git a/rustybam_amd/csrc/rb_lift.h b/rustybam_amd/csrc/rb_lift.h
--- a/rustybam_amd/csrc/rb_lift.h
+++ b/rustybam_amd/csrc/rb_lift.h
@@ -84,6 +84,32 @@
     unsigned long long *fb_count;
     int op_starts;
 };
+#define RB_TAIL_TICKET_WORD 8
+__host__ __device__ __forceinline__ unsigned long long *rb_tail_ticket(unsigned long long *copy_count) { return copy_count + RB_TAIL_TICKET_WORD; }
+
+__device__ __forceinline__ rb_job rb_make_job(uint32_t r, const rb_norm_row &nr, uint64_t op_off_r, bool minus, bool mono, bool explicit_w, uint64_t h0,
+                                              uint64_t nh, const uint32_t *win_lo, uint64_t rows_cap) {
+    rb_job j;
+    j.r = r;
+    j.n = nr.n_ops;
+    j.rec0 = op_off_r + nr.first_op;
+    j.t_st = nr.t_st, j.t_en = nr.t_en, j.q_st = nr.q_st, j.q_en = nr.q_en;
+    uint32_t f = 0;
+    const bool provisional = (nr.flags & RB_F_PROVISIONAL) != 0;
+    if (nr.status == RB_ST_OK && (nh != 0 || provisional)) {
+        if (h0 + nh > rows_cap) f |= RB_JOB_ROWS_OVERFLOW;
+        else f |= RB_JOB_VALID;
+    }
+    if ((nr.flags & RB_F_REGULAR) || (provisional && !(nr.flags & RB_F_ENDS_NOT_MATCH))) f |= RB_JOB_REGULAR;
+    if (minus) f |= RB_JOB_MINUS;
+    if (mono) f |= RB_JOB_MONO;
+    j.flags = f;
+    j.h0 = (uint32_t)h0;
+    j.nh = (uint32_t)nh;
+    j.lo = (explicit_w || !mono || !(f & RB_JOB_VALID) || nh == 0) ? 0u : *win_lo;
+    return j;
+}
+
 #define RB_GCP 64u
 struct __attribute__((aligned(64))) rb_gja {
     uint64_t ops_off;
@@ -112,6 +138,23 @@
         if (w_st[mid] >= t_en) hi = mid; else lo = mid + 1;
     }
     return lo;
+}
+
+__device__ __forceinline__ void rb_lower_both(const uint64_t *w_en, const uint64_t *w_st, uint64_t ws, uint64_t we, uint64_t t_st, uint64_t t_en,
+                                              uint64_t *first_en_gt, uint64_t *first_st_ge) {
+    uint64_t a = ws, b = we, c = ws, d = we;
+    while (a < b || c < d) {
+        const bool go1 = a < b, go2 = c < d;
+        const uint64_t m1 = go1 ? a + ((b - a) >> 1) : ws, m2 = go2 ? c + ((d - c) >> 1) : ws;
+        const uint64_t x = w_en[m1], y = w_st[m2];
+        if (go1) {
+            if (x > t_st) b = m1; else a = m1 + 1;
+        }
+        if (go2) {
+            if (y >= t_en) d = m2; else c = m2 + 1;
+        }
+    }
+    *first_en_gt = a, *first_st_ge = c;
 }
 
 enum { RB_S_UNRES = 0, RB_S_OK = 1, RB_S_NONE = 2, RB_S_DEFER = 3 };
```
